# g-benton/Volt

Hardware: AMD Instinct MI355X
Metric: mll_grad_steps_per_s (higher is better)
Workload: dtype f32; 1 GPU; MLL+grad step, N=4096, batch=64 series per GPU, Volatility kernel + EWMA(k=25) mean; series_total=64, parallelism=series-sharded x1, collective=none

## Files before the change

### include/volt_hip_tune.h

```cpp
#ifndef VOLT_HIP_TUNE_H
#define VOLT_HIP_TUNE_H

#include <stddef.h>
#include <stdint.h>

#ifdef __cplusplus
extern "C" {
#endif

int volt_profile_step_f32(const float* K, int64_t ldk, int64_t bsk, const float* resid, const float* sigma2,
                          float* out, float* alpha, void* workspace, int* info, int B, int N, int groups, void* stream,
                          float* ms_sum_host , float* ms_union_host , int* launches_host ,
                          float* per_launch_host );

int volt_tune_update_f32(float* A, const float* Winv, int* info, int B, int Np, int k, int var, int reps, void* stream);
int volt_sched_describe(int B, int n, int has_y, int k, int G, int S, float frac, int* items, int max_items, float* loads);
int volt_tune_diag_f32(float* A, float* Winv, int* info, int B, int Np, int k, long long* stamps, void* stream);

int volt_tune_diag_f64(double* A, double* Winv, int* info, int B, int Np, int k, long long* stamps, void* stream);

int volt_tune_small_stamps(long long* stamps);

int volt_long_describe(int n, int first, int emin, int* items, int max_items, int* nslabs, int* ncnt);

int volt_batch_describe(int B, int n, int has_y, int order, int* items, int max_items);
int volt_tune_batch_stamps(long long* stamps);
int volt_batch64_describe(int B, int n, int has_y, int* items, int max_items);
int volt_tune_batch64_stamps(long long* stamps);
int volt_topology_describe(int* out);

#ifdef __cplusplus
}
#endif
#endif
```

### volt_amd/_lib.py

```python
from __future__ import annotations

import ctypes as C
import os

import torch

from .build import LIB, build_lib, source_hash, sources_present

_lib = None
ABI_VERSION = 5
WANT_GRAD, WS_INITIALISED, REFINE_ALPHA = 1, 2, 4

_i32, _i64, _f32, _f64, _ptr, _sz = C.c_int, C.c_int64, C.c_float, C.c_double, C.c_void_p, C.c_size_t

_SIGS = {
    "volt_abi_version": (C.c_int, []),
    "volt_source_hash": (C.c_char_p, []),
    "volt_padded_n": (C.c_int, [_i32]),
    "volt_cumtrapz_f32": (C.c_int, [_ptr, _i64, _ptr, _i64, _ptr, _i32, _i32, _i32, _ptr]),
    "volt_cumtrapz_f64": (C.c_int, [_ptr, _i64, _ptr, _i64, _ptr, _i32, _i32, _i32, _ptr]),
    "volt_fill_f32": (C.c_int, [_ptr, _ptr, _i32, _i32, _i64, _i64, _ptr]),
    "volt_fill_f64": (C.c_int, [_ptr, _ptr, _i32, _i32, _i64, _i64, _ptr]),
    "volt_ewma_f32": (C.c_int, [_ptr, _i64, _ptr, _i32, _ptr, _i32, _i32, _ptr]),
    "volt_prepare_f32": (C.c_int, [_ptr, _i64, _i64, _ptr, _f32, _ptr, _i32, _i32, _ptr]),
    "volt_potrf_f32": (C.c_int, [_ptr, _ptr, _ptr, _i32, _i32, _ptr]),
    "volt_potrf_workspace_bytes": (C.c_size_t, [_i32, _i32]),
    "volt_potrf_workspace_init_f32": (C.c_int, [_ptr, C.c_size_t, _i32, _i32, _ptr]),
    "volt_potrf_ws_f32": (C.c_int, [_ptr, _ptr, _ptr, _i32, _i32, _ptr, C.c_size_t, _i32, _ptr]),
    "volt_potrf_k_f32": (C.c_int, [_ptr, _i64, _i64, _ptr, C.c_float, _ptr, _ptr, _ptr, _i32, _i32, _ptr, C.c_size_t, _i32, _ptr]),
    "volt_prepare_f64": (C.c_int, [_ptr, _i64, _i64, _ptr, _f64, _ptr, _i32, _i32, _ptr]),
    "volt_potrf_f64": (C.c_int, [_ptr, _ptr, _ptr, _i32, _i32, _ptr]),
    "volt_potrf_workspace_bytes_f64": (C.c_size_t, [_i32, _i32]),
    "volt_potrf_ws_f64": (C.c_int, [_ptr, _ptr, _ptr, _i32, _i32, _ptr, C.c_size_t, _ptr]),
    "volt_potrf_k_f64": (C.c_int, [_ptr, _i64, _i64, _ptr, C.c_double, _ptr, _ptr, _ptr, _i32, _i32, _ptr, C.c_size_t, _ptr]),
    "volt_trsv_lower_f64": (C.c_int, [_ptr, _ptr, _ptr, _ptr, _ptr, _i32, _i32, _ptr]),
    "volt_trsv_lower_t_f64": (C.c_int, [_ptr, _ptr, _ptr, _ptr, _ptr, _i32, _i32, _ptr]),
    "volt_trsv_lower_f32": (C.c_int, [_ptr, _ptr, _ptr, _ptr, _ptr, _i32, _i32, _ptr]),
    "volt_trsv_lower_t_f32": (C.c_int, [_ptr, _ptr, _ptr, _ptr, _ptr, _i32, _i32, _ptr]),
    "volt_trtri_f32": (C.c_int, [_ptr, _ptr, _ptr, _i32, _i32, _ptr]),
    "volt_trtri_f64": (C.c_int, [_ptr, _ptr, _ptr, _i32, _i32, _ptr]),
    "volt_trtri_workspace_bytes_f64": (C.c_size_t, [_i32, _i32]),
    "volt_trtri_ws_f64": (C.c_int, [_ptr, _ptr, _ptr, _i32, _i32, _ptr, C.c_size_t, _ptr]),
    "volt_mll_workspace_bytes_f64": (_sz, [_i32, _i32, _i32]),
    "volt_mll_step_f64": (C.c_int, [_ptr, _i64, _i64, _ptr, _ptr, _f64, _ptr, _ptr, _ptr, _ptr, _i32, _i32, _i32, _ptr]),
    "volt_rollout_scratch_bytes": (_sz, [_i32, _i32, _i32]),
    "volt_rollout_bordered_f32": (C.c_int, [_ptr] * 16 + [_i32] * 6 + [_f32] * 3 + [_ptr]),
    "volt_adam_step_f32": (C.c_int, [_ptr, _i32, C.c_longlong, _ptr, C.c_float, C.c_float, C.c_float, C.c_float, _ptr, _ptr]),
    "volt_mll_workspace_bytes": (_sz, [_i32, _i32, _i32]),
    "volt_mll_workspace_init_f32": (C.c_int, [_ptr, _i32, _i32, _i32, _ptr]),
    "volt_mll_step_f32": (C.c_int, [_ptr, _i64, _i64, _ptr, _ptr, _f32, _ptr, _ptr, _ptr, _ptr, _i32, _i32, _i32, _ptr]),
    "volt_mll_grad_k_f32": (C.c_int, [_ptr, _ptr, _ptr, _ptr, _i32, _i32, _ptr]),
    "volt_rollout_shared_f32": (C.c_int, [_ptr] * 8 + [_i32] * 5 + [_f32, _ptr]),
    "volt_gemm_nt_f32": (C.c_int, [_ptr, _i64, _i64, _i32, _ptr, _i64, _i64, _i32, _ptr, _i64, _i64, _i32, _f32, _f32,
                                   _i32, _i32, _i32, _i32, _ptr]),
    "volt_gpcv_workspace_bytes": (_sz, [_i32, _i32, _i32]),
    "volt_gpcv_step_f32": (C.c_int, [_ptr, _i64, _i64, _f32] + [_ptr] * 6 + [_i32, _f32, _f32, _f32, _f32] + [_ptr] * 7
                           + [_i32, _i32, _i32, _ptr]),
    "volt_gpcv_cv_workspace_bytes": (_sz, [_i32, _i32, _i32, _i32]),
    "volt_gpcv_cv_step_f32": (C.c_int, [_ptr, _i64, _i64, _f32] + [_ptr] * 5 + [_i32, _ptr, _ptr, _i32, _f32, _f32, _f32, _f32]
                              + [_ptr] * 8 + [_i32, _i32, _i32, _ptr]),
    "volt_gpcv_mt_workspace_bytes": (_sz, [_i32, _i32, _i32]),
    "volt_gpcv_mt_step_f32": (C.c_int, [_ptr, _i64, _f32] + [_ptr] * 9 + [_i32, _f32, _f32, _f32, _f32] + [_ptr] * 10
                              + [_i32, _i32, _i32, _ptr]),
    "volt_syev_small_f64": (C.c_int, [_ptr, _i64, _ptr, _ptr, _ptr, _i32, _i32, _ptr]),
    "volt_kron_state_bytes": (_sz, [_i32]),
    "volt_kron_prologue_f32": (C.c_int, [_ptr] * 7 + [_i64] + [_ptr] * 4 + [_i32, _i32, _ptr]),
    "volt_kron_prologue_f64": (C.c_int, [_ptr] * 7 + [_i64] + [_ptr] * 4 + [_i32, _i32, _ptr]),
    "volt_kron_epilogue_f32": (C.c_int, [_ptr] * 11 + [_i32, _i32, _ptr]),
    "volt_kron_epilogue_f64": (C.c_int, [_ptr] * 11 + [_i32, _i32, _ptr]),
}

_TUNE_SIGS = {
    "volt_profile_step_f32": (C.c_int, [_ptr, _i64, _i64, _ptr, _ptr, _ptr, _ptr, _ptr, _ptr, _i32, _i32, _i32, _ptr, _ptr, _ptr,
                                        _ptr, _ptr]),
    "volt_tune_update_f32": (C.c_int, [_ptr, _ptr, _ptr, _i32, _i32, _i32, _i32, _i32, _ptr]),
    "volt_sched_describe": (C.c_int, [_i32, _i32, _i32, _i32, _i32, _i32, C.c_float, _ptr, _i32, _ptr]),
    "volt_tune_diag_f32": (C.c_int, [_ptr, _ptr, _ptr, _i32, _i32, _i32, _ptr, _ptr]),
    "volt_tune_diag_f64": (C.c_int, [_ptr, _ptr, _ptr, _i32, _i32, _i32, _ptr, _ptr]),
    "volt_tune_small_stamps": (C.c_int, [_ptr]),
    "volt_long_describe": (C.c_int, [_i32, _i32, _i32, _ptr, _i32, _ptr, _ptr]),
    "volt_batch_describe": (C.c_int, [_i32, _i32, _i32, _i32, _ptr, _i32]),
    "volt_tune_batch_stamps": (C.c_int, [_ptr]),
    "volt_batch64_describe": (C.c_int, [_i32, _i32, _i32, _ptr, _i32]),
    "volt_tune_batch64_stamps": (C.c_int, [_ptr]),
    "volt_topology_describe": (C.c_int, [_ptr]),
}

EXPORTS = tuple(_SIGS)
TUNE_EXPORTS = tuple(_TUNE_SIGS)


class VoltHipError(RuntimeError):
    pass


class VoltHipWarning(RuntimeWarning):
    """The library recovered from an internal condition (e.g. re-ran a step on the launch-per-column schedule)."""


INFO_INTERNAL_MAX = -(2 ** 31) + 255


def _embedded_hash(path):
    handle = C.CDLL(path)
    fn = handle.volt_source_hash
    fn.restype = C.c_char_p
    return handle, fn().decode()


def lib() -> C.CDLL:
    global _lib
    if _lib is None:
        handle = None
        if os.path.exists(LIB):
            try:
                handle, built = _embedded_hash(LIB)
            except (OSError, AttributeError):
                handle = None
            if handle is not None and sources_present() and built != source_hash():
                import _ctypes
                _ctypes.dlclose(handle._handle)
                handle = None
        if handle is None:
            try:
                build_lib(force=os.path.exists(LIB), verbose=False)
            except Exception as e:
                raise VoltHipError(
                    f"{LIB} is missing or stale and could not be built ({e}): run `python -m volt_amd.build` "
                    "(hipcc, gfx950). volt_amd has no CPU fallback.") from e
            handle, built = _embedded_hash(LIB)
            if built != source_hash():
                raise VoltHipError(f"{LIB} was built from other sources ({built} != {source_hash()}): "
                                   "run `python -m volt_amd.build --force`")
        for name, (res, args) in {**_SIGS, **_TUNE_SIGS}.items():
            fn = getattr(handle, name)
            fn.restype, fn.argtypes = res, args
        if handle.volt_abi_version() != ABI_VERSION:
            raise VoltHipError("libvolt_hip.so ABI version mismatch: rebuild")
        _lib = handle
    return _lib


def check(rc: int, what: str) -> None:
    if rc == 0:
        return
    if rc < 0:
        raise VoltHipError(f"{what}: invalid argument #{-rc}")
    raise VoltHipError(f"{what}: HIP error {rc}")


def stream_ptr() -> int:
    return torch.cuda.current_stream().cuda_stream
```

### volt_amd/csrc/batch_step.hip

```cpp
#include "common.h"
#include "tiles.h"
#include "host.h"
#include "batch_sched.h"
#include "../../include/volt_hip.h"
#include "../../include/volt_hip_tune.h"
#include <algorithm>
#include <array>
#include <map>
#include <mutex>
#include <string.h>
#include <vector>

namespace volt {

__global__ void batch_begin_kernel(float* __restrict__ Winv, int nflags, int* __restrict__ info, int ninfo,
                                   int* __restrict__ prog, int nprog) {
    const int i = blockIdx.x * blockDim.x + threadIdx.x;
    if (i < nflags) reinterpret_cast<int*>(Winv)[(int64_t)i * TS * TS] = 0;
    if (i < ninfo) info[i] = 0;
    for (int c = i; c < nprog; c += gridDim.x * blockDim.x) prog[c] = 0;
}

constexpr int AUX_WT = AUX_SC1;

__device__ __forceinline__ void diag0_image(const KSource& src, int b, float* smem) {
    const float add = (src.sigma2 ? src.sigma2[b] : 0.f) + src.jitter;
    const float* Kb = src.K + (int64_t)b * src.bsk;
    const int N = src.N;
#pragma unroll 1
    for (int e0 = threadIdx.x; e0 < TS * TS; e0 += 16 * NT) {
        float v[16];
#pragma unroll
        for (int u = 0; u < 16; ++u) {
            const int e = e0 + u * NT, r = e >> 7, c = e & 127;
            v[u] = Kb[(int64_t)(r < N ? r : N - 1) * src.ldk + (c < N ? c : N - 1)];
        }
#pragma unroll
        for (int u = 0; u < 16; ++u) {
            const int e = e0 + u * NT, r = e >> 7, c = e & 127;
            float x = (r < N && c < N) ? v[u] : 0.f;
            if (r == c) x = (r < N) ? x + add : 1.f;
            smem[r * DT + c] = (c <= r) ? x : 0.f;
        }
    }
}

__device__ __forceinline__ void alpha_item(const float* __restrict__ Y, const TriReduce& red, float* __restrict__ z,
                                           float* __restrict__ apart, int Np, int b, int c, int chunk) {
    const int n = Np / TS, lane = threadIdx.x & 63, wave = threadIdx.x >> 6, l31 = lane & 31, h = lane >> 5;
    f32x4 zc = {0.f, 0.f, 0.f, 0.f};
    {
        const float* zp = red.zpart + (int64_t)b * n * Np + c * TS + 4 * l31;
        int jb = 0;
        for (; jb + 8 <= c + 1; jb += 8) {
            f32x4 v[8];
#pragma unroll
            for (int u = 0; u < 8; ++u) v[u] = *reinterpret_cast<const f32x4*>(zp + (int64_t)(jb + u) * Np);
#pragma unroll
            for (int u = 0; u < 8; ++u)
#pragma unroll
                for (int e = 0; e < 4; ++e) zc[e] += v[u][e];
        }
        for (; jb <= c; ++jb) {
            const f32x4 v = *reinterpret_cast<const f32x4*>(zp + (int64_t)jb * Np);
#pragma unroll
            for (int e = 0; e < 4; ++e) zc[e] += v[e];
        }
    }
    if (chunk == 0 && wave == 0 && h == 0) *reinterpret_cast<f32x4*>(z + (int64_t)b * Np + c * TS + 4 * l31) = zc;
    const float* Yc = Y + (int64_t)b * Np * Np + c * TS + 4 * l31 + (int64_t)h * Np;
    float* dst = apart + ((int64_t)b * n + c) * Np;
    const int r0 = chunk * BATCH_ALPHA_ROWS;
    const int r1 = (r0 + BATCH_ALPHA_ROWS < (c + 1) * TS) ? r0 + BATCH_ALPHA_ROWS : (c + 1) * TS;
    for (int r = r0 + 32 * wave; r < r1; r += 128) {
        f32x4 y[16];
#pragma unroll
        for (int u = 0; u < 16; ++u) y[u] = *reinterpret_cast<const f32x4*>(Yc + (int64_t)(r + 2 * u) * Np);
#pragma unroll
        for (int u = 0; u < 16; ++u) {
            float lo, hi;
            rowpair_dot(y[u], zc, lo, hi);
            if (lane == 0) {
                dst[r + 2 * u] = lo;
                dst[r + 2 * u + 1] = hi;
            }
        }
    }
}

static long long* g_batch_stamps = nullptr;

struct BatchArgs {
    float* A; float* Winv; float* Y; int* info;
    int Np, B;
    KSource src;
    TriReduce red;
    const int4* tab;
    int* prog;
    int pstride;
    float* zvec; float* apart;
    long long* stamps;
};

static __shared__ __attribute__((aligned(16))) float g_smem[2 * STAGE_FLOATS];
static __shared__ float g_srv[TS];
static __shared__ int g_piece;
static __shared__ int g_ahead[2];
static __shared__ int4 g_desc;

template <bool FROMK, bool LOCAL>
__device__ __forceinline__ void batch_piece(const BatchArgs a, const int w, const bool ahead, const int par, BatchPull& pull,
                                            int* qw, int per_queue) {
    float* const smem = g_smem;
    float* const srv = g_srv;
    float* const A = a.A; float* const Winv = a.Winv; float* const Y = a.Y; int* const info = a.info;
    const int Np = a.Np;
    const KSource& src = a.src;
    const TriReduce& red = a.red;
    long long* const stamps = a.stamps;
    const int n = Np / TS;
    int4 d = ahead ? g_desc : a.tab[BATCH_HDR + w];
    d.x = __builtin_amdgcn_readfirstlane(d.x);
    d.y = __builtin_amdgcn_readfirstlane(d.y);
    d.z = __builtin_amdgcn_readfirstlane(d.z);
    if (stamps && threadIdx.x == 0) stamps[(int64_t)w * 8 + 5] = __builtin_amdgcn_s_memrealtime();
    const int kind = d.x & 7, b = d.x >> 3;
    int* rowp = a.prog + (int64_t)b * a.pstride;
    int* tcol = rowp + n;
    int* la = tcol + n;
    int* info_b = info + b;
    const bool usek = FROMK && src.K != nullptr;

    if (kind == BK_DIAG) {
        const int k = d.y;
        __builtin_amdgcn_s_setprio(3);
        if (k == 0) {
            if (usek) {
                diag0_image(src, b, smem);
                diag_body<false, false, LOCAL>(A, Winv, info, Np, 0, b, smem, nullptr, true);
            } else {
                diag_body<false, false, LOCAL>(A, Winv, info, Np, 0, b, smem, nullptr, false);
            }
            return;
        }
        batch_wait<LOCAL>(rowp + k, k, k >= 2 ? la + k : nullptr, 1, info_b);
        if (stamps && threadIdx.x == 0) stamps[(int64_t)w * 8 + 3] = __builtin_amdgcn_s_memrealtime();
        if (k >= 2) update_body<FROMK>(A, Np, k, k, k - 1, k, false, b, src, smem, true);
        else update_body<FROMK>(A, Np, 1, 1, 0, 1, true, b, src, smem, true);
        if (stamps && threadIdx.x == 0) stamps[(int64_t)w * 8 + 4] = __builtin_amdgcn_s_memrealtime();
        diag_body<false, false, LOCAL>(A, Winv, info, Np, k, b, smem, nullptr, true);
        return;
    }
    if (kind == BK_LOOKAHEAD) {
        const int k = d.y;
        Chase ch;
        ch.p0 = ch.p1 = rowp + k + 1;
        bool ok = true;
        update_body<FROMK, 0, true, LOCAL>(A, Np, k + 1, k + 1, 0, k, true, b, src, smem, false, &ch, &ok);
        if (!ok && (threadIdx.x & 63) == 0) report_timeout(info_b);
        publish_release<LOCAL>(la + k + 1, 1);
        return;
    }
    if (kind == BK_TRTRI_DIAG) {
        const int i = d.y;
        batch_wait<LOCAL>(reinterpret_cast<const int*>(Winv + ((int64_t)b * n + i) * TS * TS), 1, nullptr, 0, info_b);
        trtri_diag_body(Winv, Y, Np, i, b, red, smem);
        publish_release<LOCAL>(tcol + i, 1);
        return;
    }
    if (kind == BK_ALPHA) {
        const int c = d.y;
        if (threadIdx.x < 64) {
            bool ok = true;
            for (int j = 0; j <= c; ++j) ok = wait_word<AtLeast>(tcol + j, c - j + 1) && ok;
            if (!ok && threadIdx.x == 0) report_timeout(info_b);
            acquire_unless_local<LOCAL>();
        }
        __syncthreads();
        alpha_item(Y, red, a.zvec, a.apart, Np, b, c, d.z);
        return;
    }
    TriJob jb;
    int* word;
    int val;
    if (kind == BK_PANEL) {
        const int i = d.y, k = d.z;
        jb = panel_job<FROMK>(A, Winv, Np, i, k, b, src);
        jb.t.ch.p0 = rowp + k;
        jb.t.ch.p1 = rowp + i;
        word = rowp + i;
        val = k + 1;
    } else {
        const int i = d.y, j = d.z;
        jb = trtri_job(A, Winv, Y, Np, i, j, b);
        if (red.rpad && threadIdx.x < TS) srv[threadIdx.x] = red.rpad[(int64_t)b * Np + j * TS + threadIdx.x];
        jb.t.flag = reinterpret_cast<const int*>(jb.t.W);
        jb.t.ch.p0 = rowp + i;
        jb.t.ch.base0 = j;
        jb.t.ch.p1 = tcol + j;
        word = tcol + j;
        val = i - j + 1;
    }
    f32x16 T[4], O[4];
    ChasePre pre = {0, 0};
    if (jb.t.n1 > 0) pre = chase_issue(jb.t.ch);
    job_t0(jb, T);
    if (stamps && threadIdx.x == 0) stamps[(int64_t)w * 8 + 3] = __builtin_amdgcn_s_memrealtime();
    const bool ok = tri_tile_run<true, LOCAL>(jb.t, T, O, smem, &pre);
#ifndef VOLT_NO_EPILOGUE_PRIO
    __builtin_amdgcn_s_setprio(3);
#endif
    if (stamps && threadIdx.x == 0) stamps[(int64_t)w * 8 + 4] = __builtin_amdgcn_s_memrealtime();
    if (!ok && (threadIdx.x & 63) == 0) report_timeout(info_b);
    int t_next = -1;
    if (threadIdx.x == 0 && pull.q >= 0) t_next = __hip_atomic_fetch_add(qw + 32 * pull.q, 1, __ATOMIC_RELAXED, __HIP_MEMORY_SCOPE_AGENT);
    if (jb.i >= 0 && red.rpad) trtri_reduce<!LOCAL>(O, Np, jb.i, jb.j, jb.b, red, smem + TS * WLD, srv);
    if (stamps && threadIdx.x == 0) stamps[(int64_t)w * 8 + 6] = __builtin_amdgcn_s_memrealtime();
    tri_store_lds<LOCAL ? 0 : AUX_WT>(O, jb.out, Np, smem);
    if (stamps && threadIdx.x == 0) stamps[(int64_t)w * 8 + 7] = __builtin_amdgcn_s_memrealtime();
    int4 d_next = {0, 0, 0, 0};
    int w_next = -1;
    if (threadIdx.x == 0 && pull.q >= 0) {
        if (t_next < per_queue) {
            w_next = LOCAL ? 8 * t_next + pull.q : t_next;
            d_next = a.tab[BATCH_HDR + w_next];
        } else {
            pull.q = -1;
        }
    }
    publish_wt<LOCAL>(word, val);
    if (threadIdx.x == 0 && w_next >= 0) {
        g_ahead[par ^ 1] = 1;
        g_piece = w_next;
        g_desc = d_next;
    }
}

template <bool FROMK, bool LOCAL>
__global__ __launch_bounds__(256, 2) void batch_step_kernel(BatchArgs a, int check, int npieces, int xskew, int xdrop) {
    {
        const int4 h0 = a.tab[0];
        if (h0.x != BATCH_MAGIC || h0.y != a.B || h0.z != a.Np / TS || h0.w != check) {
            if (blockIdx.x == 0)
                for (int b = threadIdx.x; b < a.B; b += NT) a.info[b] = INFO_BAD_WORKSPACE;
            return;
        }
    }
    int* const qw = a.prog + (int64_t)a.B * a.pstride;
    const int hw = hw_xcc_id();
    if (LOCAL && ((xdrop >> hw) & 1)) return;
    const int xcc = (hw + xskew) & 7;
    const int per_queue = LOCAL ? npieces / 8 : npieces;
    BatchPull pull;
    int w, ahead = 0, par = -1;
    if (xdrop & 0x40000000) {
        w = xskew | (int)0x80000000;
        goto piece;
    }
pull_next:
    __syncthreads();
    if (threadIdx.x == 0 && !(par >= 0 && g_ahead[par])) g_piece = batch_next_piece<LOCAL>(pull, qw, xcc, per_queue);
    __syncthreads();
    w = g_piece;
    ahead = par >= 0 ? g_ahead[par] : 0;
    par = par < 0 ? 0 : par;
    if (threadIdx.x == 0) g_ahead[par ^ 1] = 0;
piece:
    w = __builtin_amdgcn_readfirstlane(w);
    if (w < 0) return;
    __builtin_amdgcn_s_setprio(0);
    if (a.stamps && threadIdx.x == 0) {
        a.stamps[(int64_t)w * 8] = __builtin_amdgcn_s_memrealtime();
        a.stamps[(int64_t)w * 8 + 2] = ((long long)hw << 32) | (unsigned)__builtin_amdgcn_s_getreg((16 - 1) << 11 | 0 << 6 | 4);
    }
    par = __builtin_amdgcn_readfirstlane(par < 0 ? 0 : par);
    batch_piece<FROMK, LOCAL>(a, w, __builtin_amdgcn_readfirstlane(ahead) != 0, par, pull, qw, per_queue);
    par ^= 1;
    if (a.stamps && threadIdx.x == 0) a.stamps[(int64_t)w * 8 + 1] = __builtin_amdgcn_s_memrealtime();
    goto pull_next;
}

}

using namespace volt;

bool volt_internal_batch_applies(int B, int n, int has_y) {
    const Tunables& tn = tunables();
    if (tn.batch <= 0 || B < 1 || n < 2 || B > 65535) return false;
    if (tn.batch >= 2) return true;
    if (has_y) {
        if (n >= 20) return B >= 2;
        if (n >= 16) return B >= 4;
        if (n >= 10) return B >= 6;
        if (n >= 8) return B >= 20;
        return false;
    }
    if (n >= 28) return B >= 2;
    if (n >= 20) return B >= 3;
    if (n >= 10) return B >= 8;
    if (n >= 8) return B >= 24;
    return false;
}

bool volt_internal_batch_first() { return tunables().batch >= 3; }

static int batch_lad(int B) {
    int lad = tunables().batch_lad;
    while (lad > 0 && 2 * lad * B > 128) --lad;
    return lad;
}

static size_t batch_table_bytes(int B, int n, bool has_y) {
    return al256((size_t)(BATCH_HDR + batch_count(B, n, has_y)) * sizeof(BatchItem));
}
static size_t batch_prog_bytes(int B, int n) {
    return al256(((size_t)B * batch_pstride(n) + BATCH_QWORDS) * sizeof(int));
}

size_t volt_internal_batch_bytes(int B, int n, int has_y) {
    if (!volt_internal_batch_applies(B, n, has_y)) return 0;
    return batch_table_bytes(B, n, has_y != 0) + batch_prog_bytes(B, n);
}

static int batch_order_for(int B, int n) {
    const int forced = tunables().batch_order;
    if (forced >= 0) return forced;
    return (B >= 48 && n >= 28 && (B & 7) == 0) ? 54 : 0;
}

static int batch_check_word(int B, int n, bool has_y) {
    const uint32_t w = (uint32_t)BATCH_MAGIC ^ ((uint32_t)B * 0x01000193u) ^ ((uint32_t)n << 20) ^ (has_y ? 0x40000000u : 0u) ^
                       ((uint32_t)batch_order_for(B, n) * 2654435761u) ^ ((uint32_t)batch_lad(B) << 16);
    return (int)w;
}

struct BatchTable {
    int4* items = nullptr;
    size_t bytes = 0;
};
static const BatchTable* get_batch_table(int B, int n, bool has_y) {
    static std::mutex mu;
    static std::map<std::array<int, 4>, BatchTable*> cache;
    const int order = batch_order_for(B, n);
    const std::array<int, 4> key{B, n, has_y ? 1 : 0, order * 16 + batch_lad(B)};
    std::lock_guard<std::mutex> lock(mu);
    auto it = cache.find(key);
    if (it != cache.end()) return it->second;
    std::vector<BatchItem> items;
    batch_build(B, n, has_y, order, items, batch_lad(B));
    BatchTable* bt = new BatchTable;
    static_assert(sizeof(BatchItem) == sizeof(int4), "items are read as int4");
    bt->bytes = (BATCH_HDR + items.size()) * sizeof(BatchItem);
    if ((int64_t)items.size() != batch_count(B, n, has_y) ||
        hipHostMalloc((void**)&bt->items, bt->bytes, hipHostMallocDefault) != hipSuccess) {
        (void)hipGetLastError();
        delete bt;
        bt = nullptr;
    } else {
        memset(bt->items, 0, BATCH_HDR * sizeof(BatchItem));
        bt->items[0] = int4{BATCH_MAGIC, B, n, batch_check_word(B, n, has_y)};
        for (BatchItem& it : items) it.pad = batch_check_word(B, n, has_y);
        memcpy(bt->items + BATCH_HDR, items.data(), items.size() * sizeof(BatchItem));
    }
    cache[key] = bt;
    return bt;
}

int volt_internal_batch_install(Region state, int B, int n, int has_y, void* stream) {
    if (!state.p || state.bytes < volt_internal_batch_bytes(B, n, has_y) || !volt_internal_batch_applies(B, n, has_y)) return 0;
    const BatchTable* bt = get_batch_table(B, n, has_y != 0);
    if (!bt) return (int)hipErrorOutOfMemory;
    hipError_t e = hipMemcpyAsync(state.p, bt->items, bt->bytes, hipMemcpyHostToDevice, (hipStream_t)stream);
    return e != hipSuccess ? (int)e : 0;
}

int volt_internal_batch_step(const StepMats& m, const KSource& src, const TriReduce& red_in, const StepTail& t, Region state,
                             hipEvent_t e0, hipEvent_t e1) {
    const int B = m.B, Np = volt_padded_n(m.N), n = Np / TS;
    const bool has_y = m.Y != nullptr;
    if (!state.p || !volt_internal_batch_applies(B, n, has_y) || state.bytes < volt_internal_batch_bytes(B, n, has_y)) return 0;
    if (has_y && (!t.z || !t.apart)) return 0;
    hipStream_t s = m.stream;
    const int4* tab = reinterpret_cast<const int4*>(state.p);
    int* prog = reinterpret_cast<int*>(reinterpret_cast<char*>(state.p) + batch_table_bytes(B, n, has_y));
    const int pstride = batch_pstride(n), nprog = B * pstride + BATCH_QWORDS, nflags = B * n;
    hipLaunchKernelGGL(batch_begin_kernel, dim3(begin_grid(std::max(nflags, B), nprog)), dim3(256), 0, s, m.Winv, nflags, m.info, B, prog, nprog);
    const int check = batch_check_word(B, n, has_y);
    const bool local = batch_local_handoffs(B);
    const TriReduce red{has_y ? red_in.rpad : nullptr, red_in.zpart, red_in.frob, m.N};
    const int64_t npieces = batch_count(B, n, has_y);
    const int spread = tunables().batch_spread + (n < 32 ? 9 * (32 - n) * tunables().cus / 256 : 0);
    const unsigned pad = (int64_t)B * (n + 1) <= spread ? 16 * 1024 : 0;
    const int64_t slots = (int64_t)tunables().cus * (pad ? 1 : 2) * std::max(1, tunables().batch_pullers);
    const unsigned grid = (unsigned)std::min<int64_t>(npieces, tunables().batch_pullers > 0 ? slots : npieces);
    const BatchArgs args{m.A, m.Winv, m.Y, m.info, Np, B, src, red, tab, prog, pstride, t.z, t.apart, g_batch_stamps};
    const int xskew = tunables().batch_xskew, xdrop = tunables().batch_xdrop;
    if (e0 && hipEventRecord(e0, s) != hipSuccess) return (int)hipGetLastError();
#define VOLT_BATCH_LAUNCH(FK, LC) \
    hipLaunchKernelGGL((batch_step_kernel<FK, LC>), dim3(grid), dim3(256), pad, s, args, check, (int)npieces, xskew, xdrop)
    if (src.K && local) VOLT_BATCH_LAUNCH(true, true);
    else if (src.K) VOLT_BATCH_LAUNCH(true, false);
    else if (local) VOLT_BATCH_LAUNCH(false, true);
    else VOLT_BATCH_LAUNCH(false, false);
#undef VOLT_BATCH_LAUNCH
    if (e1 && hipEventRecord(e1, s) != hipSuccess) return (int)hipGetLastError();
    hipError_t e = hipGetLastError();
    return e != hipSuccess ? (int)e : 1;
}

extern "C" {

int volt_topology_describe(int* out) {
    if (!out) return -1;
    const Tunables& tn = tunables();
    out[0] = tn.cus;
    out[1] = tn.xccs;
    out[2] = tn.sched_g;
    out[3] = tn.plain_spread;
    out[4] = tn.split_spread;
    out[5] = tn.group_gate;
    out[6] = (tn.small_nmax > 0 ? 1 : 0) | (tn.long_on ? 2 : 0) | (tn.batch > 0 ? 4 : 0);
    return 0;
}

int volt_tune_batch_stamps(long long* stamps) {
    g_batch_stamps = stamps;
    return 0;
}

int volt_batch_describe(int B, int n, int has_y, int order, int* items, int max_items) {
    if (order == -1) order = 1000 + batch_order_for(B, n);
    if (B < 1 || n < 1 || order < 0 || (order > 15 && order < 1000) || order > 1255) return -1;
    std::vector<BatchItem> it;
    if (order >= 1000) batch_build(B, n, has_y != 0, order - 1000, it, 0);
    else batch_build(B, n, has_y != 0, order & 1, it, order >> 1);
    if ((int64_t)it.size() != batch_count(B, n, has_y != 0)) return -1;
    if (items) {
        if ((int)it.size() > max_items) return -2;
        memcpy(items, it.data(), it.size() * sizeof(BatchItem));
    }
    return (int)it.size();
}

}
```

### volt_amd/csrc/chol.hip

```cpp
#include "common.h"
#include "tiles.h"
#include "host.h"
#include "sched.h"
#include "long_sched.h"
#include "../../include/volt_hip.h"
#include "../../include/volt_hip_tune.h"
#include <algorithm>
#include <array>
#include <map>
#include <mutex>
#include <stdlib.h>
#include <string.h>
#include <utility>
#include <vector>

namespace volt {

__global__ __launch_bounds__(256) void prepare_kernel(const float* __restrict__ K, int64_t ldk, int64_t bsk,
                                                      const float* __restrict__ sigma2, float jitter,
                                                      float* __restrict__ A, int N, int Np, int col0_only) {
    int t = blockIdx.x;
    int ti, tj;
    if (col0_only) {
        ti = t;
        tj = 0;
    } else {
        ti = (int)((sqrtf(8.f * (float)t + 1.f) - 1.f) * 0.5f);
        while ((ti + 1) * (ti + 2) / 2 <= t) ++ti;
        while (ti * (ti + 1) / 2 > t) --ti;
        tj = t - ti * (ti + 1) / 2;
    }
    const int b = blockIdx.y;
    const float add = (sigma2 ? sigma2[b] : 0.f) + jitter;
    const float* Kb = K + (int64_t)b * bsk;
    float* Ab = A + (int64_t)b * Np * Np;
    const int cq = (threadIdx.x & 31) * 4;
    const int r0 = threadIdx.x >> 5;
    const bool vec_ok = ((ldk & 3) == 0) && ((bsk & 3) == 0) && (((uintptr_t)K & 15) == 0);
#pragma unroll 4
    for (int rr = r0; rr < TS; rr += 8) {
        const int i = ti * TS + rr;
        const int j = tj * TS + cq;
        f32x4 v;
        if (i < N && j + 3 < N && vec_ok) {
            v = *reinterpret_cast<const f32x4*>(Kb + (int64_t)i * ldk + j);
        } else {
#pragma unroll
            for (int c = 0; c < 4; ++c) v[c] = (i < N && j + c < N) ? Kb[(int64_t)i * ldk + j + c] : 0.f;
        }
#pragma unroll
        for (int c = 0; c < 4; ++c)
            if (i == j + c) v[c] = (i < N) ? v[c] + add : 1.f;
        *reinterpret_cast<f32x4*>(Ab + (int64_t)i * Np + j) = v;
    }
}

template <bool FROMK>
__global__ __launch_bounds__(256, 2) void factor_step_kernel(float* __restrict__ A, float* __restrict__ Winv,
                                                            float* __restrict__ Y, int* __restrict__ info, int Np,
                                                            int k_upd, int i_tri, int B, KSource src, TriReduce red) {
    __shared__ __attribute__((aligned(16))) float smem[2 * STAGE_FLOATS];
    static_assert(DIAG_LDS_FLOATS <= 2 * STAGE_FLOATS, "diag block must fit the staging area");
    static_assert(TS * WLD + TS <= 2 * STAGE_FLOATS, "W image + reduction scratch must fit");
    const int n = Np / TS;
    int w = blockIdx.x;
    TriJob jb;
    bool have = false;
    if (k_upd >= 0) {
        const int k = k_upd;
        if (w < B) {
            if (k >= 2) update_body<FROMK>(A, Np, k, k, k - 1, k, false, w, src, smem, true);
            else if (k == 1) update_body<FROMK>(A, Np, 1, 1, 0, 1, true, w, src, smem, true);
            diag_body(A, Winv, info, Np, k, w, smem, nullptr, k > 0);
            return;
        }
        w -= B;
        const int npre = (k >= 1 && k + 1 < n) ? B : 0;
        if (w < npre) {
            update_body<FROMK>(A, Np, k + 1, k + 1, 0, k, true, w, src, smem);
            return;
        }
        w -= npre;
        const int npan = (n - k - 1) * B;
        if (w < npan) {
            int t, b;
            decode_tile_batch(w, n - k - 1, B, t, b);
            jb = panel_job<FROMK>(A, Winv, Np, k + 1 + t, k, b, src);
            have = true;
        }
        w -= npan;
    }
    if (!have) {
        int j, b;
        decode_tile_batch(w, i_tri + 1, B, j, b);
        if (j == i_tri) {
            trtri_diag_body(Winv, Y, Np, i_tri, b, red, smem);
            return;
        }
        jb = trtri_job(A, Winv, Y, Np, i_tri, j, b);
    }
    f32x16 T[4], O[4];
    if (jb.c0 && jb.row_ok && jb.vec_ok) {
#pragma unroll
        for (int tm = 0; tm < 4; ++tm)
#pragma unroll
            for (int g = 0; g < 4; ++g) {
                const f32x4 v = *reinterpret_cast<const f32x4*>(jb.c0 + 32 * tm + 8 * g);
#pragma unroll
                for (int e = 0; e < 4; ++e) T[tm][4 * g + e] = -v[e];
            }
    } else if (jb.c0 && jb.row_ok) {
#pragma unroll
        for (int tm = 0; tm < 4; ++tm)
#pragma unroll
            for (int q = 0; q < 16; ++q) T[tm][q] = -jb.c0[32 * tm + 8 * (q >> 2) + (q & 3)];
    } else {
        zero_acc(T);
    }
    const bool ok = tri_tile_run(jb.t, T, O, smem);
    if (threadIdx.x == 0 && !ok) report_timeout(info + jb.b);
    tri_store(O, jb.out, Np);
    if (jb.i >= 0 && red.rpad) trtri_reduce(O, Np, jb.i, jb.j, jb.b, red, smem);
}

constexpr int VOLT_SPLITK_SLABS = 64;
struct SplitK {
    float* slab;
    int* count;
    int S;
    int L;
    int cap;
    int4* tab = nullptr;
    size_t tab_bytes = 0;
};

__device__ __forceinline__ void slab_sum(f32x16 (&acc)[4], const float* __restrict__ slabs, int nsl) {
    zero_acc(acc);
    for (int sidx = 0; sidx < nsl; ++sidx) {
        const f32x4* in = reinterpret_cast<const f32x4*>(slabs + (int64_t)sidx * TS * TS);
#pragma unroll
        for (int t4 = 0; t4 < 4; ++t4)
#pragma unroll
            for (int g = 0; g < 4; ++g) {
                const f32x4 v = in[(t4 * 4 + g) * NT + threadIdx.x];
#pragma unroll
                for (int e = 0; e < 4; ++e) acc[t4][4 * g + e] += v[e];
            }
    }
}
__device__ __forceinline__ bool splitk_arrive(int* counter, int nsl) {
    __shared__ int s_last;
    asm volatile("s_waitcnt vmcnt(0)" ::: "memory");
    __syncthreads();
    if (threadIdx.x == 0) {
        const int old = __hip_atomic_fetch_add(counter, 1, __ATOMIC_RELAXED, __HIP_MEMORY_SCOPE_AGENT);
        s_last = (old == nsl - 1);
        if (s_last) __builtin_amdgcn_fence(__ATOMIC_ACQUIRE, "agent");
    }
    __syncthreads();
    return s_last != 0;
}

template <bool FROMK>
__device__ __forceinline__ void lookahead_slice(float* __restrict__ A, int Np, int k, int b, int sl, int nsl, int b0, int b1,
                                                const KSource& src, float* __restrict__ slabs, int* __restrict__ counter,
                                                float* smem) {
    float* Ab = A + (int64_t)b * Np * Np;
    const int lane = threadIdx.x & 63, wave = threadIdx.x >> 6, wr = wave >> 1, wc = wave & 1;
    f32x16 acc[4];
    zero_acc(acc);
    gemm_nt_128<0>(Ab + (int64_t)(k + 1) * TS * Np + (int64_t)b0 * TS, Np, Ab + (int64_t)(k + 1) * TS * Np + (int64_t)b0 * TS, Np,
                   (b1 - b0) * (TS / BK), acc, smem);
    if (nsl > 1) {
        slab_dump(acc, slabs + (int64_t)sl * TS * TS);
        if (!splitk_arrive(counter, nsl)) return;
        slab_sum(acc, slabs, nsl);
    }
    const bool usek = FROMK && src.K != nullptr;
    const float add = usek ? ((src.sigma2 ? src.sigma2[b] : 0.f) + src.jitter) : 0.f;
    const float* Kb = usek ? src.K + (int64_t)b * src.bsk : nullptr;
    float* C = Ab + (int64_t)(k + 1) * TS * Np + (int64_t)(k + 1) * TS;
#pragma unroll
    for (int tm = 0; tm < 2; ++tm)
#pragma unroll
        for (int tn = 0; tn < 2; ++tn)
#pragma unroll
            for (int q = 0; q < 16; ++q) {
                const int r = wr * 64 + tm * 32 + accrow(q, lane);
                const int c = wc * 64 + tn * 32 + (lane & 31);
                C[(int64_t)r * Np + c] = input_elem(src, Kb, add, Ab, Np, usek, (k + 1) * TS + r, (k + 1) * TS + c)
                                         - acc[tm * 2 + tn][q];
            }
}

template <bool FUSE>
__device__ __forceinline__ void tri_slice(TriJob& jb, int sl, int nsl, int b0, int b1, float* __restrict__ slabs,
                                          int* __restrict__ counter, int* __restrict__ info, const TriReduce& red, int Np,
                                          float* smem) {
    f32x16 T[4], O[4];
    if (sl == 0 && jb.c0 && jb.row_ok && jb.vec_ok) {
#pragma unroll
        for (int tm = 0; tm < 4; ++tm)
#pragma unroll
            for (int g = 0; g < 4; ++g) {
                const f32x4 v = *reinterpret_cast<const f32x4*>(jb.c0 + 32 * tm + 8 * g);
#pragma unroll
                for (int e = 0; e < 4; ++e) T[tm][4 * g + e] = -v[e];
            }
    } else if (sl == 0 && jb.c0 && jb.row_ok) {
#pragma unroll
        for (int tm = 0; tm < 4; ++tm)
#pragma unroll
            for (int q = 0; q < 16; ++q) T[tm][q] = -jb.c0[32 * tm + 8 * (q >> 2) + (q & 3)];
    } else {
        zero_acc(T);
    }
    if (!FUSE || nsl > 1) {
        gemm_nt_128<1>(jb.t.X + (int64_t)b0 * TS, jb.t.ldx, jb.t.Z + (int64_t)b0 * TS, jb.t.ldz, (b1 - b0) * (TS / BK), T, smem);
        if (nsl > 1) {
            slab_dump(T, slabs + (int64_t)sl * TS * TS);
            if (!splitk_arrive(counter, nsl)) return;
            slab_sum(T, slabs, nsl);
        }
        jb.t.n1 = 0;
    }
    const bool ok = tri_tile_run(jb.t, T, O, smem);
    if (threadIdx.x == 0 && !ok) report_timeout(info + jb.b);
    tri_store(O, jb.out, Np);
    if (jb.i >= 0 && red.rpad) trtri_reduce(O, Np, jb.i, jb.j, jb.b, red, smem);
}

template <bool FROMK>
__global__ __launch_bounds__(256, 2) void factor_step_split_kernel(float* __restrict__ A, float* __restrict__ Winv,
                                                                  float* __restrict__ Y, int* __restrict__ info, int Np,
                                                                  int k_upd, int i_tri, int B, KSource src, TriReduce red,
                                                                  SplitK sk) {
    __shared__ __attribute__((aligned(16))) float smem[2 * STAGE_FLOATS];
    const int n = Np / TS, S = sk.S;
    int w = blockIdx.x;
    const int k = k_upd;
    if (k < n && w < B) {
        if (k >= 2) update_body<FROMK>(A, Np, k, k, k - 1, k, false, w, src, smem, true);
        else if (k == 1) update_body<FROMK>(A, Np, 1, 1, 0, 1, true, w, src, smem, true);
        diag_body(A, Winv, info, Np, k, w, smem, nullptr, k > 0);
        return;
    }
    if (k < n) w -= B;
    int* count = sk.count + (int64_t)k * B * (n + 1);
    const int npre = (k >= 1 && k + 1 < n) ? B : 0;
    if (w < npre * S) {
        const int b = w / S, sl = w % S;
        const int kb = k;
        int nsl = (kb + sk.L - 1) / sk.L;
        nsl = nsl < 1 ? 1 : (nsl > S ? S : nsl);
        if (sl >= nsl) return;
        lookahead_slice<FROMK>(A, Np, k, b, sl, nsl, sl * kb / nsl, (sl + 1) * kb / nsl, src,
                               sk.slab + (int64_t)b * S * TS * TS, count + b, smem);
        return;
    }
    w -= npre * S;
    TriJob jb;
    int tile, kb;
    const int npan = (k < n) ? (n - k - 1) * B : 0;
    const int sl = w % S;
    int wt = w / S;
    if (wt < npan) {
        int t, b;
        decode_tile_batch(wt, n - k - 1, B, t, b);
        jb = panel_job<FROMK>(A, Winv, Np, k + 1 + t, k, b, src);
        tile = B + wt;
        kb = k;
    } else {
        wt -= npan;
        int j, b;
        decode_tile_batch(wt, i_tri + 1, B, j, b);
        if (j == i_tri) {
            if (sl == 0) trtri_diag_body(Winv, Y, Np, i_tri, b, red, smem);
            return;
        }
        jb = trtri_job(A, Winv, Y, Np, i_tri, j, b);
        tile = B + npan + wt;
        kb = i_tri - j;
    }
    int nsl = (kb + sk.L - 1) / sk.L;
    nsl = nsl < 1 ? 1 : (nsl > S ? S : nsl);
    if (sl >= nsl) return;
    tri_slice<false>(jb, sl, nsl, sl * kb / nsl, (sl + 1) * kb / nsl, sk.slab + (int64_t)tile * S * TS * TS, count + tile,
                     info, red, Np, smem);
}

template <bool FROMK>
__global__ __launch_bounds__(256, 1) void factor_step_sched_kernel(float* __restrict__ A, float* __restrict__ Winv,
                                                                  float* __restrict__ Y, int* __restrict__ info, int Np,
                                                                  int k, int i_tri, int B, KSource src, TriReduce red,
                                                                  SplitK sk, const int4* __restrict__ items, int4 key0,
                                                                  int4 key1) {
    __shared__ __attribute__((aligned(16))) float smem[2 * STAGE_FLOATS];
    const int n = Np / TS, S = sk.S;
    {
        const int4 h0 = sk.tab[0], h1 = sk.tab[1];
        if (h0.x != key0.x || h0.y != key0.y || h0.z != key0.z || h0.w != key0.w || h1.x != key1.x || h1.y != key1.y ||
            h1.z != key1.z || h1.w != key1.w) {
            if (blockIdx.x == 0)
                for (int b = threadIdx.x; b < B; b += NT) info[b] = INFO_BAD_WORKSPACE;
            return;
        }
    }
    int* count = sk.count + (int64_t)k * B * (n + 1);
    const int4 d = items[blockIdx.x];
    const int kind = d.x & 7, b = d.x >> 3;
    const int sl = d.z & 255, nsl = (d.z >> 8) & 255, tile = d.z >> 16;
    const int b0 = d.w & 0xffff, b1 = d.w >> 16;
    float* slabs = sk.slab + (int64_t)tile * S * TS * TS;
    if (kind == 0) {
        if (k >= 2) update_body<FROMK>(A, Np, k, k, k - 1, k, false, b, src, smem, true);
        else if (k == 1) update_body<FROMK>(A, Np, 1, 1, 0, 1, true, b, src, smem, true);
        diag_body(A, Winv, info, Np, k, b, smem, nullptr, k > 0);
    } else if (kind == 4) {
        trtri_diag_body(Winv, Y, Np, i_tri, b, red, smem);
    } else if (kind == 1) {
        lookahead_slice<FROMK>(A, Np, k, b, sl, nsl, b0, b1, src, slabs, count + tile, smem);
    } else {
        TriJob jb = kind == 2 ? panel_job<FROMK>(A, Winv, Np, d.y, k, b, src) : trtri_job(A, Winv, Y, Np, i_tri, d.y, b);
        tri_slice<true>(jb, sl, nsl, b0, b1, slabs, count + tile, info, red, Np, smem);
    }
}

__global__ __launch_bounds__(256, 2) void tune_diag_kernel(float* __restrict__ A, float* __restrict__ Winv,
                                                          int* __restrict__ info, int Np, int k, long long* stamps) {
    __shared__ __attribute__((aligned(16))) float smem[2 * STAGE_FLOATS];
    diag_body<true>(A, Winv, info, Np, k, blockIdx.x, smem, stamps + 32 * blockIdx.x);
}

__global__ void begin_factor_kernel(float* __restrict__ Winv, int nflags, int* __restrict__ info, int ninfo,
                                    int* __restrict__ count, int ncount) {
    const int i = blockIdx.x * blockDim.x + threadIdx.x;
    if (i < nflags) reinterpret_cast<int*>(Winv)[(int64_t)i * TS * TS] = 0;
    if (i < ninfo) info[i] = 0;
    for (int c = i; c < ncount; c += gridDim.x * blockDim.x) count[c] = 0;
}

__global__ __launch_bounds__(256, 2) void tune_update_kernel(float* __restrict__ A, const float* __restrict__ Winv,
                                                            int* __restrict__ info, int Np, int k, int B, KSource src) {
    __shared__ __attribute__((aligned(16))) float smem[2 * STAGE_FLOATS];
    int t, b;
    decode_tile_batch(Np / TS - k - 1, B, t, b);
    const TriJob jb = panel_job<false>(A, Winv, Np, k + 1 + t, k, b, src);
    f32x16 T[4], O[4];
#pragma unroll
    for (int tm = 0; tm < 4; ++tm)
#pragma unroll
        for (int g = 0; g < 4; ++g) {
            const f32x4 v = *reinterpret_cast<const f32x4*>(jb.c0 + 32 * tm + 8 * g);
#pragma unroll
            for (int e = 0; e < 4; ++e) T[tm][4 * g + e] = -v[e];
        }
    const bool ok = tri_tile_run(jb.t, T, O, smem);
    if (threadIdx.x == 0 && !ok) report_timeout(info + jb.b);
    tri_store(O, jb.out, Np);
}
template <int ABL>
__global__ __launch_bounds__(256, 2) void tune_update_sq_kernel(float* __restrict__ A, int Np, int k, int B, KSource src) {
    __shared__ __attribute__((aligned(16))) float smem[2 * STAGE_FLOATS];
    int t, b;
    decode_tile_batch(Np / TS - k - 1, B, t, b);
    update_body<false, ABL>(A, Np, k + 1 + t, k, 0, k, true, b, src, smem);
}
__global__ void tune_empty_kernel(float* A) { if (A == nullptr) A[0] = 0.f; }

}

using namespace volt;

static Tunables read_env(Tunables t) {
    auto geti = [](const char* name, int& v) { if (const char* e = getenv(name)) v = atoi(e); };
        geti("VOLT_GROUPS", t.groups);
        geti("VOLT_SPLITK_TARGET", t.splitk_target);
        geti("VOLT_SPLITK_MINL", t.splitk_minl);
        geti("VOLT_SPLITK_MAXS", t.splitk_maxs);
        geti("VOLT_SPLITK_GROUPS", t.splitk_groups);
        geti("VOLT_SPLITK_MAXB", t.splitk_maxb);
        geti("VOLT_SCHED", t.sched);
        geti("VOLT_SCHED_MINB", t.sched_minb);
        geti("VOLT_SCHED_MAXB", t.sched_maxb);
        geti("VOLT_SCHED_MAXB_POTRF", t.sched_maxb_potrf);
        geti("VOLT_SCHED_G", t.sched_g);
        geti("VOLT_SCHED_S", t.sched_s);
        geti("VOLT_SCHED_GROUPS", t.sched_groups);
        geti("VOLT_SCHED_KMIN", t.sched_kmin);
        geti("VOLT_SMALL_NMAX", t.small_nmax);
        geti("VOLT_SMALL_MAXWG", t.small_maxwg);
        geti("VOLT_SMALL_PAD_MAXB", t.small_pad_maxb);
        geti("VOLT_SMALL_MAXB", t.small_maxb);
        geti("VOLT_SMALL_MAXB2", t.small_maxb2);
        geti("VOLT_LONG", t.long_on);
        geti("VOLT_LONG_FIRST", t.long_first);
        geti("VOLT_LONG_EMIN", t.long_emin);
        geti("VOLT_LONG_PAD", t.long_pad);
        geti("VOLT_LONG_NMIN", t.long_nmin);
        geti("VOLT_LONG_XCD", t.long_xcd);
        geti("VOLT_LONG_SPLIT", t.long_split);
        geti("VOLT_PLAIN_SPREAD", t.plain_spread);
        geti("VOLT_SPLIT_SPREAD", t.split_spread);
        geti("VOLT_BATCH", t.batch);
        geti("VOLT_BATCH_ORDER", t.batch_order);
        geti("VOLT_BATCH_LOCAL", t.batch_local);
        geti("VOLT_BATCH_SPREAD", t.batch_spread);
        geti("VOLT_BATCH_LAD", t.batch_lad);
        geti("VOLT_BATCH_PULLERS", t.batch_pullers);
        geti("VOLT_ROLLOUT_LANE", t.rollout_lane);
        geti("VOLT_LONG_PULLERS", t.long_pullers);
        geti("VOLT_BATCH_XSKEW", t.batch_xskew);
        geti("VOLT_BATCH_XDROP", t.batch_xdrop);
        geti("VOLT_BATCH64", t.batch64);
        geti("VOLT_BATCH64_MAX", t.batch64_max);
        geti("VOLT_BATCH64_MAX_STEP", t.batch64_max_step);
        geti("VOLT_F64_LOOKAHEAD", t.f64_lookahead);
        geti("VOLT_F64_TRTRI_LOOKAHEAD", t.f64_trtri_lookahead);
        geti("VOLT_F64_SPREAD", t.f64_spread);
        geti("VOLT_F64_SPLIT_TARGET", t.f64_split_target);
        if (const char* e = getenv("VOLT_SCHED_FRAC")) t.sched_frac = (float)atof(e);
        geti("VOLT_FAKE_CUS", t.cus);
        geti("VOLT_FAKE_XCCS", t.xccs);
    return t;
}

static void apply_topology(Tunables& t, bool faked) {
    if (!faked) {
        int dev = 0, cus = 0, xccs = 0;
        if (hipGetDevice(&dev) == hipSuccess &&
            hipDeviceGetAttribute(&cus, hipDeviceAttributeMultiprocessorCount, dev) == hipSuccess && cus > 0) {
            t.cus = cus;
            if (hipDeviceGetAttribute(&xccs, hipDeviceAttributeNumberOfXccs, dev) == hipSuccess && xccs > 0) t.xccs = xccs;
        } else {
            (void)hipGetLastError();
        }
    }
    if (t.cus == 256 && t.xccs == 8) return;
    const double f = t.cus / 256.0;
    auto scale = [f](int v, int lo) { const int r = (int)(v * f + 0.5); return r < lo ? lo : r; };
    t.sched_g = scale(t.sched_g, 8);
    t.plain_spread = scale(t.plain_spread, 8);
    t.split_spread = scale(t.split_spread, 16);
    t.splitk_target = scale(t.splitk_target, 16);
    t.group_gate = scale(t.group_gate, 16);
    t.batch_spread = scale(t.batch_spread, 8);
    t.small_nmax = 0;
    t.long_on = 0;
    t.batch = 0;
    t.batch64 = 0;
}

const Tunables& tunables() {
    static const Tunables tn = [] {
        const char* tune0 = getenv("VOLT_TUNE");
        const bool tuning = tune0 && atoi(tune0) != 0;
        const bool faked = tuning && (getenv("VOLT_FAKE_CUS") || getenv("VOLT_FAKE_XCCS"));
        Tunables t = [&] {
            Tunables t;
            if (!tuning) return t;
            return read_env(t);
        }();
        apply_topology(t, faked);
        return t;
    }();
    return tn;
}
struct LaunchTimer {
    hipEvent_t base = nullptr;
    std::vector<hipEvent_t> ev;
    std::vector<int> cls;
    hipError_t err = hipSuccess;
    void note(hipError_t e) { if (err == hipSuccess && e != hipSuccess) err = e; }
    void start(hipStream_t s) {
        note(hipEventCreate(&base));
        note(hipEventRecord(base, s));
    }
    void begin(int c, hipStream_t s) {
        hipEvent_t e = nullptr;
        note(hipEventCreate(&e));
        note(hipEventRecord(e, s));
        ev.push_back(e);
        cls.push_back(c);
    }
    void end(hipStream_t s) {
        hipEvent_t e = nullptr;
        note(hipEventCreate(&e));
        note(hipEventRecord(e, s));
        ev.push_back(e);
    }
    void collect(float* ms_sum, float* ms_union, int* n_by_class, int nclass, float* per_launch = nullptr) {
        std::vector<std::vector<std::pair<float, float>>> iv(nclass);
        for (int c = 0; c < nclass; ++c) { ms_sum[c] = ms_union[c] = 0.f; n_by_class[c] = 0; }
        for (size_t i = 0; i < cls.size(); ++i) {
            float t0 = 0.f, t1 = 0.f;
            note(hipEventElapsedTime(&t0, base, ev[2 * i]));
            note(hipEventElapsedTime(&t1, base, ev[2 * i + 1]));
            ms_sum[cls[i]] += t1 - t0;
            n_by_class[cls[i]] += 1;
            if (per_launch) per_launch[i] = t1 - t0;
            iv[cls[i]].push_back({t0, t1});
        }
        for (int c = 0; c < nclass; ++c) {
            std::sort(iv[c].begin(), iv[c].end());
            float lo = 0.f, hi = -1.f;
            for (auto& x : iv[c]) {
                if (hi < lo || x.first > hi) {
                    if (hi >= lo) ms_union[c] += hi - lo;
                    lo = x.first;
                    hi = x.second;
                } else if (x.second > hi) {
                    hi = x.second;
                }
            }
            if (hi >= lo) ms_union[c] += hi - lo;
        }
        for (auto e : ev) (void)hipEventDestroy(e);
        if (base) (void)hipEventDestroy(base);
        ev.clear();
        cls.clear();
    }
};

struct FactorOpts {
    KSource src;
    float* Y;
    TriReduce red;
    SplitK sk;
    const struct SchedDev* sched = nullptr;
};

constexpr int SCHED_HDR = 16;
struct SchedDev {
    int4* items = nullptr;
    size_t bytes = 0;
    int4 key[2];
    std::vector<int> item_off;
    int S = 0;
    int pad_lds = 0;
    int kmin = 0;
};

static const SchedDev* get_sched(int B, int n, bool has_y, const SchedParams& p, hipStream_t s) {
    static std::mutex mu;
    static std::map<std::array<int, 8>, SchedDev*> cache;
    int dev = 0;
    if (hipGetDevice(&dev) != hipSuccess) return nullptr;
    const std::array<int, 8> key{dev, B, n, has_y ? 1 : 0, p.G, p.S, (int)(p.frac * 1000.f), p.min_len};
    std::lock_guard<std::mutex> lock(mu);
    auto it = cache.find(key);
    if (it != cache.end()) return it->second;
    hipStreamCaptureStatus cap = hipStreamCaptureStatusNone;
    if (hipStreamIsCapturing(s, &cap) != hipSuccess || cap != hipStreamCaptureStatusNone) return nullptr;
    std::vector<SchedItem> items;
    SchedDev* sd = new SchedDev;
    sd->S = p.S;
    sd->pad_lds = 16 * 1024;
    const int kmin_env = tunables().sched_kmin;
    sd->kmin = kmin_env >= 0 ? kmin_env : !has_y ? (B * (256 / p.G) >= 48 ? 20 : 12) : (p.G < 256 ? 16 : B <= 4 ? 12 : B <= 7 ? 16 : 20);
    const int launches = has_y ? n + 1 : n;
    for (int k = 0; k < launches; ++k) {
        sd->item_off.push_back((int)items.size());
        sched_build_launch(B, n, has_y, k, p, items);
    }
    sd->item_off.push_back((int)items.size());
    static_assert(sizeof(SchedItem) == sizeof(int4), "items are read as int4");
    sd->bytes = (SCHED_HDR + items.size()) * sizeof(SchedItem);
    sd->key[0] = int4{0x564f4c54, B, n, has_y ? 1 : 0};
    sd->key[1] = int4{p.G, p.S, (int)(p.frac * 1000.f), p.min_len};
    if (hipHostMalloc((void**)&sd->items, sd->bytes, hipHostMallocDefault) != hipSuccess) {
        (void)hipGetLastError();
        delete sd;
        sd = nullptr;
    } else {
        memset(sd->items, 0, SCHED_HDR * sizeof(SchedItem));
        sd->items[0] = sd->key[0];
        sd->items[1] = sd->key[1];
        memcpy(sd->items + SCHED_HDR, items.data(), items.size() * sizeof(SchedItem));
    }
    cache[key] = sd;
    return sd;
}

static bool sched_choice(int B, int n, bool has_y, int cap, int& Gs, SchedParams& sp) {
    const Tunables& tn = tunables();
    if (!tn.sched || cap < 1 || B < tn.sched_minb || B > (has_y ? tn.sched_maxb : tn.sched_maxb_potrf)) return false;
    Gs = (tn.sched_groups > 1 && B >= 10 && B % tn.sched_groups == 0) ? tn.sched_groups : 1;
    sp = SchedParams();
    sp.G = tn.sched_g / Gs;
    sp.S = std::max(1, std::min(tn.sched_s, cap / B));
    sp.frac = tn.sched_frac;
    (void)n;
    return true;
}

static int sched_install(void* tab, size_t tab_bytes, int B, int n, bool has_y, int cap, hipStream_t s) {
    int Gs = 1;
    SchedParams sp;
    if (!tab || !sched_choice(B, n, has_y, cap, Gs, sp)) return 0;
    const SchedDev* sd = get_sched(B / Gs, n, has_y, sp, s);
    if (!sd || sd->bytes > tab_bytes) return 0;
    hipError_t e = hipMemcpyAsync(tab, sd->items, sd->bytes, hipMemcpyHostToDevice, s);
    return e != hipSuccess ? (int)e : 0;
}

struct Group {
    float* A;
    float* Winv;
    int* info;
    FactorOpts o;
    int B;
    hipStream_t s;
};

static void enqueue_step(const Group& g, int Np, int k, LaunchTimer* tm) {
    const int n = Np / TS, B = g.B;
    const TriReduce nored{nullptr, nullptr, nullptr, 0};
    const int itri = (g.o.Y && k > 0) ? k - 1 : -1;
    const int npre = (k >= 1 && k + 1 < n) ? B : 0;
    const int grid = B + npre + (n - k - 1) * B + (itri >= 0 ? (itri + 1) * B : 0);
    if (g.o.sched && k >= g.o.sched->kmin) {
        const SchedDev& sd = *g.o.sched;
        SplitK sk = g.o.sk;
        sk.S = sd.S;
        sk.L = 1;
        for (int kk = k; kk <= (k + 1 == n && g.o.Y ? n : k); ++kk) {
            const int it = kk < n ? itri : n - 1;
            if (tm) tm->begin(kk < n ? 0 : 1, g.s);
            const int cnt = sd.item_off[kk + 1] - sd.item_off[kk];
            if (g.o.src.K && kk < n)
                hipLaunchKernelGGL(factor_step_sched_kernel<true>, dim3(cnt), dim3(256), sd.pad_lds, g.s, g.A, g.Winv, g.o.Y,
                                   g.info, Np, kk, it, B, g.o.src, g.o.Y ? g.o.red : nored, sk, g.o.sk.tab + SCHED_HDR + sd.item_off[kk], sd.key[0],
                                   sd.key[1]);
            else
                hipLaunchKernelGGL(factor_step_sched_kernel<false>, dim3(cnt), dim3(256), sd.pad_lds, g.s, g.A, g.Winv, g.o.Y,
                                   g.info, Np, kk, it, B, g.o.src, g.o.Y ? g.o.red : nored, sk, g.o.sk.tab + SCHED_HDR + sd.item_off[kk], sd.key[0],
                                   sd.key[1]);
            if (tm) tm->end(g.s);
        }
        return;
    }
    if (!g.o.sched && g.o.sk.slab && g.o.sk.S > 1) {
        const int kk = k < n ? k : n - 1;
        const double blocks = (double)B * ((double)(n - kk - 1) * kk + 0.5 * kk * (kk - 1) + kk);
        int L = (int)(blocks / (double)g.o.sk.S + 0.999);
        const int minl = tunables().splitk_minl;
        if (L < minl) L = minl;
        int S = (kk + L - 1) / L;
        if (S < 1) S = 1;
        const int maxs = tunables().splitk_maxs;
        if (S > maxs) S = maxs;
        if (S * B > g.o.sk.cap) S = g.o.sk.cap / B;
        if (S < 1) S = 1;
        SplitK sk = g.o.sk;
        sk.S = S;
        sk.L = L;
        const int gs = B + S * (npre + (n - k - 1) * B + (itri >= 0 ? (itri + 1) * B : 0));
        if (tm) tm->begin(0, g.s);
        const int split_spread = tunables().split_spread;
        const unsigned spad = gs <= split_spread ? 16 * 1024 : 0;
        if (g.o.src.K)
            hipLaunchKernelGGL(factor_step_split_kernel<true>, dim3(gs), dim3(256), spad, g.s, g.A, g.Winv, g.o.Y, g.info, Np,
                               k, itri, B, g.o.src, g.o.Y ? g.o.red : nored, sk);
        else
            hipLaunchKernelGGL(factor_step_split_kernel<false>, dim3(gs), dim3(256), spad, g.s, g.A, g.Winv, g.o.Y, g.info, Np,
                               k, itri, B, g.o.src, g.o.Y ? g.o.red : nored, sk);
        if (tm) tm->end(g.s);
        if (k + 1 == n && g.o.Y) {
            if (tm) tm->begin(1, g.s);
            hipLaunchKernelGGL(factor_step_split_kernel<false>, dim3(S * n * B), dim3(256), S * n * B <= split_spread ? 16 * 1024 : 0, g.s, g.A, g.Winv, g.o.Y,
                               g.info, Np, n, n - 1, B, g.o.src, g.o.red, sk);
            if (tm) tm->end(g.s);
        }
        return;
    }
    if (tm) tm->begin(0, g.s);
    const unsigned pad = grid <= tunables().plain_spread ? 16 * 1024 : 0;
    if (g.o.src.K)
        hipLaunchKernelGGL(factor_step_kernel<true>, dim3(grid), dim3(256), pad, g.s, g.A, g.Winv, g.o.Y, g.info, Np, k,
                           itri, B, g.o.src, g.o.Y ? g.o.red : nored);
    else
        hipLaunchKernelGGL(factor_step_kernel<false>, dim3(grid), dim3(256), pad, g.s, g.A, g.Winv, g.o.Y, g.info, Np, k,
                           itri, B, g.o.src, g.o.Y ? g.o.red : nored);
    if (tm) tm->end(g.s);
    if (k + 1 == n && g.o.Y) {
        if (tm) tm->begin(1, g.s);
        hipLaunchKernelGGL(factor_step_kernel<false>, dim3(n * B), dim3(256), 0, g.s, g.A, g.Winv, g.o.Y, g.info, Np,
                           -1, n - 1, B, g.o.src, g.o.red);
        if (tm) tm->end(g.s);
    }
}

static int begin_factor(float* Winv, int* info, int B, int n, hipStream_t s, int* sk_count = nullptr) {
    const int nflags = B * n, ncount = sk_count ? (n + 1) * (n + 1) * B : 0;
    hipLaunchKernelGGL(begin_factor_kernel, dim3(begin_grid(std::max(nflags, B), ncount)), dim3(256), 0, s, Winv, nflags, info, B, sk_count, ncount);
    return 0;
}

constexpr int MAX_GROUPS = 8;
struct StreamPool {
    hipStream_t aux[MAX_GROUPS - 1];
    hipEvent_t fork, join[MAX_GROUPS - 1], extra[5];
    std::mutex mu;
    int want_groups = 2;
    bool ok = false;
};
static StreamPool* stream_pool() {
    static StreamPool pools[16];
    static std::once_flag once[16];
    int dev = 0;
    if (hipGetDevice(&dev) != hipSuccess || dev < 0 || dev >= 16) return nullptr;
    std::call_once(once[dev], [dev]() {
        StreamPool& p = pools[dev];
        bool ok = hipEventCreateWithFlags(&p.fork, hipEventDisableTiming) == hipSuccess;
        for (int i = 0; i < MAX_GROUPS - 1; ++i) {
            ok = ok && hipStreamCreateWithFlags(&p.aux[i], hipStreamNonBlocking) == hipSuccess;
            ok = ok && hipEventCreateWithFlags(&p.join[i], hipEventDisableTiming) == hipSuccess;
        }
        for (int i = 0; i < 5; ++i) ok = ok && hipEventCreateWithFlags(&p.extra[i], hipEventDisableTiming) == hipSuccess;
        p.want_groups = tunables().groups;
        if (p.want_groups < 1) p.want_groups = 1;
        if (p.want_groups > MAX_GROUPS) p.want_groups = MAX_GROUPS;
        p.ok = ok;
    });
    return pools[dev].ok ? &pools[dev] : nullptr;
}

bool volt_internal_aux(VoltAux* out) {
    StreamPool* p = stream_pool();
    if (!p) return false;
    *out = VoltAux{p->aux[0], p->aux[1], p->aux[2], p->aux[3], p->fork,
                   {p->join[0], p->join[1], p->join[2], p->join[3], p->join[4], p->join[5], p->join[6], p->extra[0],
                    p->extra[1], p->extra[2], p->extra[3], p->extra[4]}, &p->mu};
    return true;
}

static int pick_groups(const StreamPool* pool, int B, int force) {
    int want = force > 0 ? force : (pool ? pool->want_groups : 1);
    if (want > MAX_GROUPS) want = MAX_GROUPS;
    while (want > 1 && (B % want != 0 || B / want < 8)) want >>= 1;
    return want;
}

#define VOLT_TRY(call)                              \
    do {                                            \
        hipError_t e__ = (call);                    \
        if (e__ != hipSuccess) return (int)e__;     \
    } while (0)

static int run_factor_groups(float* A, float* Winv, int* info, int B, int Np, hipStream_t s, const FactorOpts& o,
                             volt_group_post_fn post = nullptr, void* post_ctx = nullptr, LaunchTimer* tm = nullptr,
                             int force_groups = 0) {
    const int n = Np / TS;
    StreamPool* pool = stream_pool();
    int G = pool ? pick_groups(pool, B, force_groups) : 1;
    if (force_groups == 0 && (int64_t)B * (n + 1) < tunables().group_gate) G = 1;
    hipStreamCaptureStatus cap_status = hipStreamCaptureStatusNone;
    const bool capturing = hipStreamIsCapturing(s, &cap_status) == hipSuccess && cap_status != hipStreamCaptureStatusNone;
    if (capturing && force_groups == 0) G = 1;
    const Tunables& tn = tunables();
    const int target = tn.splitk_target, split_groups = tn.splitk_groups, split_maxb = tn.splitk_maxb;
    const bool can_split = o.sk.slab && o.sk.count && force_groups == 0 && target > 1;
    FactorOpts o1 = o;
    o1.sk.S = 1;
    if (can_split && B < 8) {
        G = 1;
        o1.sk.S = target;
    }
    if (can_split && !capturing && B >= 10 && B < split_maxb && pool && split_groups > 1 && B % split_groups == 0) {
        G = split_groups;
        o1.sk.S = target / G;
    }
    if (can_split) {
        int Gs = 1;
        SchedParams sp;
        const SchedDev* sd = nullptr;
        if (o.sk.tab && sched_choice(B, n, o.Y != nullptr, o.sk.cap, Gs, sp) && (Gs == 1 || (pool && !capturing)))
            sd = get_sched(B / Gs, n, o.Y != nullptr, sp, s);
        if (sd && sd->bytes <= o.sk.tab_bytes && n > sd->kmin + (B < 8 ? 7 : 1)) {
            G = Gs;
            o1.sk.S = 2;
            o1.sched = sd;
        }
    }
    int rc = begin_factor(Winv, info, B, n, s, o1.sk.S > 1 ? o1.sk.count : nullptr);
    if (rc) return rc;
    std::unique_lock<std::mutex> lock;
    if (pool && G > 1) lock = std::unique_lock<std::mutex>(pool->mu);
    if (pool && G > 1) VOLT_TRY(hipEventRecord(pool->fork, s));
    if (tm) tm->start(s);
    if (G == 1) {
        const Group g{A, Winv, info, o1, B, s};
        for (int k = 0; k < n; ++k) enqueue_step(g, Np, k, tm);
        if (post) post(post_ctx, 0, B, s);
        VOLT_LAUNCH_CHECK();
        return tm && tm->err != hipSuccess ? (int)tm->err : 0;
    }
    const int Bg = B / G;
    const int64_t mat = (int64_t)Np * Np;
    Group grp[MAX_GROUPS];
    for (int g = 0; g < G; ++g) {
        FactorOpts og = o1;
        const int b0 = g * Bg;
        if (og.sk.S > 1) {
            og.sk.slab += (int64_t)g * (o.sk.cap / G) * (n + 1) * TS * TS;
            og.sk.count += (int64_t)g * (n + 1) * (n + 1) * Bg;
            og.sk.cap = o.sk.cap / G;
        }
        if (og.src.K) {
            og.src.K += (int64_t)b0 * og.src.bsk;
            if (og.src.sigma2) og.src.sigma2 += b0;
        }
        if (og.Y) og.Y += b0 * mat;
        if (og.red.rpad) {
            og.red.rpad += (int64_t)b0 * Np;
            og.red.zpart += (int64_t)b0 * n * Np;
            og.red.frob += (int64_t)b0 * (n * (n + 1) / 2);
        }
        grp[g] = Group{A + b0 * mat, Winv + (int64_t)b0 * n * TS * TS, info + b0, og, Bg, g == 0 ? s : pool->aux[g - 1]};
        if (g > 0) VOLT_TRY(hipStreamWaitEvent(grp[g].s, pool->fork, 0));
    }
    for (int k = 0; k < n; ++k)
        for (int g = 0; g < G; ++g) enqueue_step(grp[g], Np, k, tm);
    if (post)
        for (int g = 0; g < G; ++g) post(post_ctx, g * Bg, Bg, grp[g].s);
    int first_err = 0;
    for (int g = 1; g < G; ++g) {
        hipError_t e = hipEventRecord(pool->join[g - 1], grp[g].s);
        if (e == hipSuccess) e = hipStreamWaitEvent(s, pool->join[g - 1], 0);
        if (e != hipSuccess) {
            (void)hipStreamSynchronize(grp[g].s);
            if (!first_err) first_err = (int)e;
        }
    }
    if (first_err) return first_err;
    VOLT_LAUNCH_CHECK();
    return tm && tm->err != hipSuccess ? (int)tm->err : 0;
}

static int run_trtri(const float* A, const float* Winv, float* Y, int B, int Np, hipStream_t s, LaunchTimer* tm) {
    const int n = Np / TS;
    const TriReduce nored{nullptr, nullptr, nullptr, 0};
    for (int i = 0; i < n; ++i) {
        if (tm) tm->begin(1, s);
        hipLaunchKernelGGL(factor_step_kernel<false>, dim3((i + 1) * B), dim3(256), 0, s, const_cast<float*>(A),
                           const_cast<float*>(Winv), Y, nullptr, Np, -1, i, B, KSource{nullptr, 0, 0, nullptr, 0.f, 0},
                           nored);
        if (tm) tm->end(s);
    }
    VOLT_LAUNCH_CHECK();
    return 0;
}

size_t volt_internal_sched_bytes(int B, int n) {
    if (B < 3 || B > 64 || n < 8) return 0;
    return al256(((size_t)(n + 1) * B * (1 + 4 * (size_t)(n + 1)) + SCHED_HDR) * sizeof(SchedItem));
}

int volt_internal_sched_install(Region tab, int B, int n, int has_y, int cap, void* stream) {
    return sched_install(tab.p, tab.bytes, B, n, has_y != 0, cap, (hipStream_t)stream);
}

static FactorOpts factor_from_k(const StepMats& m, const KSource& src, const TriReduce& red, const SplitScratch& sk) {
    const int Np = volt_padded_n(m.N);
    hipLaunchKernelGGL(prepare_kernel, dim3(Np / TS, m.B), dim3(256), 0, m.stream, src.K, src.ldk, src.bsk, src.sigma2, src.jitter,
                       m.A, m.N, Np, 1);
    return FactorOpts{src, m.Y, red, SplitK{sk.slab, sk.count, 1, 1, sk.rows, (int4*)sk.tab.p, sk.tab.bytes}};
}

int volt_internal_factor(const StepMats& m, const KSource& src, const TriReduce& red, const SplitScratch& sk,
                         volt_group_post_fn post, void* post_ctx) {
    const FactorOpts o = factor_from_k(m, src, red, sk);
    return run_factor_groups(m.A, m.Winv, m.info, m.B, volt_padded_n(m.N), m.stream, o, post, post_ctx);
}

int volt_internal_profile(const StepMats& m, const KSource& src, const TriReduce& red, const SplitScratch& sk, int groups,
                          volt_group_post_fn post, void* post_ctx, const ProfileOut& out) {
    if (groups < 0 || groups > MAX_GROUPS) return -11;
    const FactorOpts o = factor_from_k(m, src, red, sk);
    LaunchTimer tm;
    const int rc = run_factor_groups(m.A, m.Winv, m.info, m.B, volt_padded_n(m.N), m.stream, o, post, post_ctx, &tm, groups);
    hipError_t e = hipStreamSynchronize(m.stream);
    tm.collect(out.ms_sum, out.ms_union, out.launches, 2, out.per_launch);
    if (rc) return rc;
    if (e != hipSuccess) return (int)e;
    return tm.err != hipSuccess ? (int)tm.err : 0;
}

extern "C" {

int volt_prepare_f32(const float* K, int64_t ldk, int64_t bsk, const float* sigma2, float jitter, float* A, int B,
                     int N, void* stream) {
    if (!K) return -1;
    if (ldk < N) return -2;
    if (!A) return -6;
    if (B < 0 || B > 65535) return -7;
    if (N < 1) return -8;
    if (B == 0) return 0;
    const int Np = volt_padded_n(N), n = Np / TS;
    hipLaunchKernelGGL(prepare_kernel, dim3(n * (n + 1) / 2, B), dim3(256), 0, (hipStream_t)stream, K, ldk, bsk,
                       sigma2, jitter, A, N, Np, 0);
    VOLT_LAUNCH_CHECK();
    return 0;
}

int volt_tune_update_f32(float* A, const float* Winv, int* info, int B, int Np, int k, int var, int reps, void* stream) {
    if (!A) return -1;
    if (!Winv) return -2;
    if (!info) return -3;
    if (B < 1) return -4;
    if (Np < TS || Np % TS) return -5;
    const int n = Np / TS;
    if (k < 1 || k + 1 >= n) return -6;
    if (var < 0 || var > 5) return -7;
    hipStream_t s = (hipStream_t)stream;
    const KSource none{nullptr, 0, 0, nullptr, 0.f, 0};
    for (int r = 0; r < reps; ++r) {
        if (var == 0) hipLaunchKernelGGL(tune_update_kernel, dim3((n - k - 1) * B), dim3(256), 0, s, A, Winv, info, Np, k, B, none);
        else if (var == 1) hipLaunchKernelGGL(tune_update_sq_kernel<0>, dim3((n - k - 1) * B), dim3(256), 0, s, A, Np, k, B, none);
        else if (var == 2) hipLaunchKernelGGL(tune_update_sq_kernel<1>, dim3((n - k - 1) * B), dim3(256), 0, s, A, Np, k, B, none);
        else if (var == 3) hipLaunchKernelGGL(tune_update_sq_kernel<2>, dim3((n - k - 1) * B), dim3(256), 0, s, A, Np, k, B, none);
        else if (var == 4) hipLaunchKernelGGL(tune_update_sq_kernel<3>, dim3((n - k - 1) * B), dim3(256), 0, s, A, Np, k, B, none);
        else hipLaunchKernelGGL(tune_empty_kernel, dim3((n - k - 1) * B), dim3(256), 0, s, A);
    }
    VOLT_LAUNCH_CHECK();
    return 0;
}

int volt_sched_describe(int B, int n, int has_y, int k, int G, int S, float frac, int* items, int max_items, float* loads) {
    if (B < 1 || n < 1 || k < 0 || k > n || (k == n && !has_y) || G < 1 || S < 1) return -1;
    SchedParams p;
    p.G = G;
    p.S = S;
    if (frac > 0.f) p.frac = frac;
    std::vector<SchedItem> it;
    std::vector<float> ld;
    sched_build_launch(B, n, has_y != 0, k, p, it, &ld);
    if ((int)it.size() > max_items) return -2;
    if (items) memcpy(items, it.data(), it.size() * sizeof(SchedItem));
    if (loads) memcpy(loads, ld.data(), ld.size() * sizeof(float));
    return (int)it.size();
}



int volt_tune_diag_f32(float* A, float* Winv, int* info, int B, int Np, int k, long long* stamps, void* stream) {
    if (!A) return -1;
    if (!Winv) return -2;
    if (!info) return -3;
    if (B < 1) return -4;
    if (Np < TS || Np % TS) return -5;
    if (k < 0 || k >= Np / TS) return -6;
    if (!stamps) return -7;
    hipLaunchKernelGGL(tune_diag_kernel, dim3(B), dim3(256), 0, (hipStream_t)stream, A, Winv, info, Np, k, stamps);
    VOLT_LAUNCH_CHECK();
    return 0;
}

static int potrf_ws_rows(int B) { return B < 32 ? VOLT_SPLITK_SLABS : (B <= 64 ? 2 * VOLT_SPLITK_SLABS : 0); }

struct PotrfWs {
    SplitScratch sk;
    Region batch;
    size_t bytes;
};
static PotrfWs carve_potrf(void* ws, int B, int Np) {
    const size_t n = (size_t)Np / TS;
    size_t off = 0;
    auto take = [&](size_t bytes) {
        void* p = ws && bytes ? reinterpret_cast<char*>(ws) + off : nullptr;
        off += bytes;
        return Region{p, bytes};
    };
    PotrfWs w;
    w.sk.rows = n < 3 ? 0 : potrf_ws_rows(B);
    w.sk.slab = reinterpret_cast<float*>(take(w.sk.rows ? al256((size_t)w.sk.rows * (n + 1) * TS * TS * sizeof(float)) : 0).p);
    w.sk.count = reinterpret_cast<int*>(take(w.sk.rows ? al256((n + 1) * (n + 1) * B * sizeof(int)) : 0).p);
    w.sk.tab = take(w.sk.rows ? volt_internal_sched_bytes(B, (int)n) : 0);
    w.batch = take(volt_internal_batch_bytes(B, (int)n, 0));
    w.bytes = off;
    return w;
}

size_t volt_potrf_workspace_bytes(int B, int Np) {
    if (B < 1 || Np < TS || Np % TS) return 0;
    return carve_potrf(nullptr, B, Np).bytes;
}

int volt_potrf_workspace_init_f32(void* ws, size_t ws_bytes, int B, int Np, void* stream) {
    if (B < 1) return -3;
    if (Np < TS || Np % TS) return -4;
    if (!volt_potrf_workspace_bytes(B, Np)) return 0;
    if (!ws || ((uintptr_t)ws & 255)) return -1;
    const PotrfWs w = carve_potrf(ws, B, Np);
    if (ws_bytes < w.bytes) return -2;
    if (w.batch.p) {
        const int rc = volt_internal_batch_install(w.batch, B, Np / TS, 0, stream);
        if (rc) return rc;
    }
    if (!w.sk.tab.p) return 0;
    return sched_install(w.sk.tab.p, w.sk.tab.bytes, B, Np / TS, false, w.sk.rows, (hipStream_t)stream);
}

static int potrf_with_scratch(const KSource& src, const StepMats& m, void* ws, size_t ws_bytes, int ws_flags, int err) {
    const int Np = volt_padded_n(m.N);
    const bool ready = (ws_flags & VOLT_WS_INITIALISED) != 0;
    SplitScratch sk{nullptr, nullptr, 0, {}};
    if (ws) {
        if (((uintptr_t)ws & 255) != 0) return err;
        const PotrfWs w = carve_potrf(ws, m.B, Np);
        if (ws_bytes < w.bytes) return err - 1;
        if (w.batch.p && ready) {
            KSource bsrc = src;
            bsrc.N = m.N;
            const int rc = volt_internal_batch_step(m, bsrc, TriReduce{nullptr, nullptr, nullptr, 0}, StepTail{}, w.batch);
            if (rc == 1) return 0;
            if (rc) return rc > 0 ? rc : err - 2;
        }
        sk = w.sk;
        if (!ready) sk.tab.p = nullptr;
    }
    if (src.K) return volt_internal_factor(m, src, TriReduce{nullptr, nullptr, nullptr, 0}, sk, nullptr, nullptr);
    const FactorOpts o{src, nullptr, TriReduce{nullptr, nullptr, nullptr, 0}, SplitK{sk.slab, sk.count, 1, 1, sk.rows, (int4*)sk.tab.p, sk.tab.bytes}};
    return run_factor_groups(m.A, m.Winv, m.info, m.B, Np, m.stream, o);
}

int volt_potrf_ws_f32(float* A, float* Winv, int* info, int B, int Np, void* ws, size_t ws_bytes, int ws_flags, void* stream) {
    if (!A) return -1;
    if (!Winv) return -2;
    if (!info) return -3;
    if (B < 0) return -4;
    if (Np < TS || Np % TS) return -5;
    if (B == 0) return 0;
    return potrf_with_scratch(KSource{nullptr, 0, 0, nullptr, 0.f, 0}, StepMats{A, Winv, nullptr, info, B, Np, (hipStream_t)stream}, ws,
                              ws_bytes, ws_flags, -6);
}

int volt_potrf_f32(float* A, float* Winv, int* info, int B, int Np, void* stream) {
    return volt_potrf_ws_f32(A, Winv, info, B, Np, nullptr, 0, 0, stream);
}

int volt_potrf_k_f32(const float* K, int64_t ldk, int64_t bsk, const float* sigma2, float jitter, float* A, float* Winv,
                     int* info, int B, int N, void* ws, size_t ws_bytes, int ws_flags, void* stream) {
    if (!K) return -1;
    if (ldk < N) return -2;
    if (!A) return -6;
    if (!Winv) return -7;
    if (!info) return -8;
    if (B < 0 || B > 65535) return -9;
    if (N < 1) return -10;
    if (B == 0) return 0;
    return potrf_with_scratch(KSource{K, ldk, bsk, sigma2, jitter, N}, StepMats{A, Winv, nullptr, info, B, N, (hipStream_t)stream}, ws,
                              ws_bytes, ws_flags, -11);
}

int volt_trtri_f32(const float* A, const float* Winv, float* Y, int B, int Np, void* stream) {
    if (!A) return -1;
    if (!Winv) return -2;
    if (!Y) return -3;
    if (B < 0) return -4;
    if (Np < TS || Np % TS) return -5;
    if (B == 0) return 0;
    return run_trtri(A, Winv, Y, B, Np, (hipStream_t)stream, nullptr);
}

}
```

### volt_amd/csrc/common.h

```cpp
#pragma once
#include <hip/hip_runtime.h>
#include <stdint.h>
#include "handoff.h"

#define VOLT_ABI_VERSION 5

namespace volt {

constexpr int TS = 128;
constexpr int BK = 32;
constexpr int SLD = BK + 4;
constexpr int NT = 256;
constexpr int STAGE_FLOATS = 2 * TS * SLD;
constexpr int GEMM_LDS_BYTES = 2 * STAGE_FLOATS * 4;

typedef float f32x4 __attribute__((ext_vector_type(4)));
typedef float f32x16 __attribute__((ext_vector_type(16)));

#define VOLT_LAUNCH_CHECK()                                   \
    do {                                                      \
        hipError_t e__ = hipGetLastError();                   \
        if (e__ != hipSuccess) return (int)e__;               \
    } while (0)

__device__ __forceinline__ int accrow(int q, int lane) { return (q & 3) + 8 * (q >> 2) + 4 * (lane >> 5); }

__device__ __forceinline__ void decode_tile_batch(int w, int ntiles, int nbatch, int& tile, int& batch) {
    if ((nbatch & 7) == 0) {
        const int xcd = w & 7, slot = w >> 3;
        batch = (slot / ntiles) * 8 + xcd;
        tile = slot % ntiles;
    } else {
        batch = w / ntiles;
        tile = w % ntiles;
    }
}

__device__ __forceinline__ void decode_tile_batch(int ntiles, int nbatch, int& tile, int& batch) {
    decode_tile_batch((int)blockIdx.x, ntiles, nbatch, tile, batch);
}

struct StageRegs {
    f32x4 a[4], b[4];
};

__device__ __forceinline__ void stage_load(StageRegs& s, const float* __restrict__ A, int64_t lda,
                                           const float* __restrict__ B, int64_t ldb, int k0) {
    const int t = threadIdx.x;
    const int row = t >> 3, cq = (t & 7) * 4;
#pragma unroll
    for (int p = 0; p < 4; ++p) {
        s.a[p] = *reinterpret_cast<const f32x4*>(A + (int64_t)(row + 32 * p) * lda + k0 + cq);
        s.b[p] = *reinterpret_cast<const f32x4*>(B + (int64_t)(row + 32 * p) * ldb + k0 + cq);
    }
}

__device__ __forceinline__ void stage_store(const StageRegs& s, float* __restrict__ buf) {
    const int t = threadIdx.x;
    const int row = t >> 3, cq = (t & 7) * 4;
    float* sA = buf;
    float* sB = buf + TS * SLD;
#pragma unroll
    for (int p = 0; p < 4; ++p) {
        *reinterpret_cast<f32x4*>(sA + (row + 32 * p) * SLD + cq) = s.a[p];
        *reinterpret_cast<f32x4*>(sB + (row + 32 * p) * SLD + cq) = s.b[p];
    }
}

struct StageAddr {
    __amdgpu_buffer_rsrc_t ra, rb;
    int va[4], vb[4];
};

__device__ __forceinline__ StageAddr stage_addr(const float* A, int64_t lda, const float* B, int64_t ldb) {
    StageAddr sa;
    sa.ra = __builtin_amdgcn_make_buffer_rsrc((void*)A, 0, 0x7fffffff, 0x00020000);
    sa.rb = __builtin_amdgcn_make_buffer_rsrc((void*)B, 0, 0x7fffffff, 0x00020000);
    const int t = threadIdx.x;
    const int row = t >> 3, cq = (t & 7) * 4;
#pragma unroll
    for (int p = 0; p < 4; ++p) {
        sa.va[p] = (int)(((int64_t)(row + 32 * p) * lda + cq) * 4);
        sa.vb[p] = (int)(((int64_t)(row + 32 * p) * ldb + cq) * 4);
    }
    return sa;
}

__device__ __forceinline__ void stage_load_buf(StageRegs& s, const StageAddr& sa, int k0) {
    const int so = __builtin_amdgcn_readfirstlane(k0 * 4);
#pragma unroll
    for (int p = 0; p < 4; ++p) {
        s.a[p] = __builtin_bit_cast(f32x4, __builtin_amdgcn_raw_buffer_load_b128(sa.ra, sa.va[p], so, 0));
        s.b[p] = __builtin_bit_cast(f32x4, __builtin_amdgcn_raw_buffer_load_b128(sa.rb, sa.vb[p], so, 0));
    }
}

__device__ __forceinline__ void zero_acc(f32x16 (&acc)[4]) {
#pragma unroll
    for (int i = 0; i < 4; ++i)
#pragma unroll
        for (int q = 0; q < 16; ++q) acc[i][q] = 0.f;
}

template <int WL> struct Frag;
template <> struct Frag<0> { f32x4 a0, a1, b0, b1; };
template <> struct Frag<1> { f32x4 a[4], b0; };

template <int WL>
__device__ __forceinline__ void frag_load(Frag<WL>& f, const float* __restrict__ buf, int kk) {
    const int lane = threadIdx.x & 63, wave = threadIdx.x >> 6;
    const int l31 = lane & 31, lh = lane >> 5;
    const float* sA = buf;
    const float* sB = buf + TS * SLD;
    const int ko = kk * 8 + 4 * lh;
    if constexpr (WL == 0) {
        const int wr = wave >> 1, wc = wave & 1;
        f.a0 = *reinterpret_cast<const f32x4*>(sA + (wr * 64 + l31) * SLD + ko);
        f.b0 = *reinterpret_cast<const f32x4*>(sB + (wc * 64 + l31) * SLD + ko);
        f.b1 = *reinterpret_cast<const f32x4*>(sB + (wc * 64 + 32 + l31) * SLD + ko);
        f.a1 = *reinterpret_cast<const f32x4*>(sA + (wr * 64 + 32 + l31) * SLD + ko);
    } else {
        f.b0 = *reinterpret_cast<const f32x4*>(sB + (wave * 32 + l31) * SLD + ko);
#pragma unroll
        for (int tm = 0; tm < 4; ++tm) f.a[tm] = *reinterpret_cast<const f32x4*>(sA + (tm * 32 + l31) * SLD + ko);
    }
}

template <int WL>
__device__ __forceinline__ void frag_mma_m(const Frag<WL>& f, int m, f32x16 (&acc)[4]) {
    if constexpr (WL == 0) {
        acc[0] = __builtin_amdgcn_mfma_f32_32x32x2f32(f.a0[m], f.b0[m], acc[0], 0, 0, 0);
        acc[1] = __builtin_amdgcn_mfma_f32_32x32x2f32(f.a0[m], f.b1[m], acc[1], 0, 0, 0);
        acc[2] = __builtin_amdgcn_mfma_f32_32x32x2f32(f.a1[m], f.b0[m], acc[2], 0, 0, 0);
        acc[3] = __builtin_amdgcn_mfma_f32_32x32x2f32(f.a1[m], f.b1[m], acc[3], 0, 0, 0);
    } else {
#pragma unroll
        for (int tm = 0; tm < 4; ++tm)
            acc[tm] = __builtin_amdgcn_mfma_f32_32x32x2f32(f.a[tm][m], f.b0[m], acc[tm], 0, 0, 0);
    }
}
template <int WL>
__device__ __forceinline__ void frag_mma(const Frag<WL>& f, f32x16 (&acc)[4]) {
#pragma unroll
    for (int m = 0; m < 4; ++m) frag_mma_m<WL>(f, m, acc);
}

constexpr int SEG_CHUNKS = 4;
__device__ __forceinline__ f32x16 zero16c() {
    f32x16 z;
#pragma unroll
    for (int q = 0; q < 16; ++q) z[q] = 0.f;
    return z;
}
#define VOLT_SB() __builtin_amdgcn_sched_barrier(0)
template <int WL>
__device__ __forceinline__ f32x16 frag_mma_one(const Frag<WL>& f, int m, int t, const f32x16& c) {
    if constexpr (WL == 0) {
        const float a = (t & 2) ? f.a1[m] : f.a0[m], b = (t & 1) ? f.b1[m] : f.b0[m];
        return __builtin_amdgcn_mfma_f32_32x32x2f32(a, b, c, 0, 0, 0);
    } else {
        return __builtin_amdgcn_mfma_f32_32x32x2f32(f.a[t][m], f.b0[m], c, 0, 0, 0);
    }
}
template <int WL>
__device__ __forceinline__ void seg_first_group(const Frag<WL>& f, f32x16 (&P)[4], f32x16 (&T)[4]) {
    const f32x16 z = zero16c();
    P[0] = frag_mma_one<WL>(f, 0, 0, z);
    VOLT_SB();
    T[3] += P[3];
    VOLT_SB();
    P[1] = frag_mma_one<WL>(f, 0, 1, z);
    P[2] = frag_mma_one<WL>(f, 0, 2, z);
    P[3] = frag_mma_one<WL>(f, 0, 3, z);
#pragma unroll
    for (int m = 1; m < 4; ++m) frag_mma_m<WL>(f, m, P);
}
template <int WL>
__device__ __forceinline__ void seg_last_group(const Frag<WL>& f, f32x16 (&P)[4], f32x16 (&T)[4]) {
#pragma unroll
    for (int m = 0; m < 3; ++m) frag_mma_m<WL>(f, m, P);
    P[0] = frag_mma_one<WL>(f, 3, 0, P[0]);
    P[1] = frag_mma_one<WL>(f, 3, 1, P[1]);
    VOLT_SB();
    T[0] += P[0];
    VOLT_SB();
    P[2] = frag_mma_one<WL>(f, 3, 2, P[2]);
    VOLT_SB();
    T[1] += P[1];
    VOLT_SB();
    P[3] = frag_mma_one<WL>(f, 3, 3, P[3]);
    VOLT_SB();
    T[2] += P[2];
    VOLT_SB();
}
enum SegRole { SEG_MID = 0, SEG_FIRST = 1, SEG_LAST = 2 };


__device__ __forceinline__ void stage_store_piece(const StageRegs& s, float* __restrict__ buf, int p) {
    const int t = threadIdx.x;
    const int row = t >> 3, cq = (t & 7) * 4;
    *reinterpret_cast<f32x4*>(buf + (row + 32 * p) * SLD + cq) = s.a[p];
    *reinterpret_cast<f32x4*>(buf + TS * SLD + (row + 32 * p) * SLD + cq) = s.b[p];
}
__device__ __forceinline__ void stage_load_piece(StageRegs& s, const StageAddr& sa, int so, int p) {
    s.a[p] = __builtin_bit_cast(f32x4, __builtin_amdgcn_raw_buffer_load_b128(sa.ra, sa.va[p], so, 0));
    s.b[p] = __builtin_bit_cast(f32x4, __builtin_amdgcn_raw_buffer_load_b128(sa.rb, sa.vb[p], so, 0));
}

template <int WL, bool MORE, bool ST, bool LD, int ROLE = SEG_MID>
__device__ __forceinline__ void chunk_run(const float* cur, float* nxt, Frag<WL>& F0, Frag<WL>& F1, f32x16 (&acc)[4],
                                         f32x16 (&run)[4], StageRegs& s, const StageAddr& sa, int k_ld) {
    frag_load<WL>(F1, cur, 1);
    VOLT_SB();
    if constexpr (ROLE == SEG_FIRST) seg_first_group<WL>(F0, acc, run);
    else frag_mma<WL>(F0, acc);
    VOLT_SB();
    frag_load<WL>(F0, cur, 2);
    VOLT_SB();
#pragma unroll
    for (int m = 0; m < 4; ++m) {
        frag_mma_m<WL>(F1, m, acc);
        if constexpr (ST) stage_store_piece(s, nxt, m);
        VOLT_SB();
    }
    frag_load<WL>(F1, cur, 3);
    VOLT_SB();
    const int so = __builtin_amdgcn_readfirstlane(k_ld * 4);
#pragma unroll
    for (int m = 0; m < 4; ++m) {
        frag_mma_m<WL>(F0, m, acc);
        if constexpr (LD) stage_load_piece(s, sa, so, m);
        VOLT_SB();
    }
    __syncthreads();
    if constexpr (MORE) frag_load<WL>(F0, nxt, 0);
    VOLT_SB();
    if constexpr (ROLE == SEG_LAST) seg_last_group<WL>(F1, acc, run);
    else frag_mma<WL>(F1, acc);
    VOLT_SB();
}

template <int WL, bool CHASE = false, bool LOCALP = false>
__device__ __forceinline__ void gemm_nt_128(const float* __restrict__ A, int64_t lda, const float* __restrict__ B,
                                               int64_t ldb, int nchunks, f32x16 (&acc)[4], float* smem,
                                               const Chase* ch = nullptr, bool* ch_ok = nullptr) {
    if (nchunks <= 0) return;
    int ready = 0;
    if constexpr (CHASE) ready = chase_wait<LOCALP>(*ch, 1, *ch_ok);
    StageRegs s0, s1;
    const StageAddr sa = stage_addr(A, lda, B, ldb);
    stage_load_buf(s0, sa, 0);
    stage_store(s0, smem);
    stage_load_buf(s0, sa, BK);
    stage_load_buf(s1, sa, 2 * BK);
    __syncthreads();
    Frag<WL> F0, F1;
    frag_load<WL>(F0, smem, 0);
    float* b0 = smem;
    float* b1 = smem + STAGE_FLOATS;
    f32x16 P[4];
    P[3] = zero16c();
    int c = 0;
    for (; c + SEG_CHUNKS < nchunks; c += SEG_CHUNKS) {
        if constexpr (CHASE) {
            const int need = (c >> 2) + 2;
            if (ready < need) ready = chase_wait<LOCALP>(*ch, need, *ch_ok);
        }
        chunk_run<WL, true, true, true, SEG_FIRST>(b0, b1, F0, F1, P, acc, s0, sa, (c + 3) * BK);
        chunk_run<WL, true, true, true>(b1, b0, F0, F1, P, acc, s1, sa, (c + 4) * BK);
        chunk_run<WL, true, true, true>(b0, b1, F0, F1, P, acc, s0, sa, (c + 5) * BK);
        chunk_run<WL, true, true, true, SEG_LAST>(b1, b0, F0, F1, P, acc, s1, sa, (c + 6) * BK);
    }
    chunk_run<WL, true, true, true, SEG_FIRST>(b0, b1, F0, F1, P, acc, s0, sa, (c + 3) * BK);
    chunk_run<WL, true, true, false>(b1, b0, F0, F1, P, acc, s1, sa, 0);
    chunk_run<WL, true, true, false>(b0, b1, F0, F1, P, acc, s0, sa, 0);
    chunk_run<WL, false, false, false, SEG_LAST>(b1, b0, F0, F1, P, acc, s1, sa, 0);
    acc[3] += P[3];
    __syncthreads();
}

struct TriTile {
    const float* X;  int64_t ldx;
    const float* Z;  int64_t ldz;
    int n1;
    const float* W;
    const int* flag;
    int want;
    Chase ch;
};

#ifndef VOLT_Z_AUX
#define VOLT_Z_AUX 2
#endif
struct TriSrc {
    __amdgpu_buffer_rsrc_t ra, rb, rw;
    int va, vb, vw;
    int pa, pb;
    int n1, nall;
};

template <int KIND = -1>
__device__ __forceinline__ void tri_load_piece(StageRegs& s, const TriSrc& ts, int c, int p) {
    if constexpr (KIND == 0) return;
    if (KIND == 1 || (KIND < 0 && c < ts.n1)) {
        const int sa = __builtin_amdgcn_readfirstlane(c * BK * 4 + p * ts.pa);
        const int sb = __builtin_amdgcn_readfirstlane(c * BK * 4 + p * ts.pb);
        s.a[p] = __builtin_bit_cast(f32x4, __builtin_amdgcn_raw_buffer_load_b128(ts.ra, ts.va, sa, 0));
        s.b[p] = __builtin_bit_cast(f32x4, __builtin_amdgcn_raw_buffer_load_b128(ts.rb, ts.vb, sb, VOLT_Z_AUX));
    } else {
        const int so = __builtin_amdgcn_readfirstlane((c - ts.n1) * BK * 4 + p * (32 * TS * 4));
        s.b[p] = __builtin_bit_cast(f32x4, __builtin_amdgcn_raw_buffer_load_b128(ts.rw, ts.vw, so, 0));
    }
}
template <int KIND = -1>
__device__ __forceinline__ void tri_store_piece(const StageRegs& s, float* __restrict__ buf, const TriSrc& ts, int c, int p) {
    if constexpr (KIND == 0) return;
    const int t = threadIdx.x;
    const int row = t >> 3, cq = (t & 7) * 4;
    if (KIND == 1 || (KIND < 0 && c < ts.n1)) *reinterpret_cast<f32x4*>(buf + (row + 32 * p) * SLD + cq) = s.a[p];
    *reinterpret_cast<f32x4*>(buf + TS * SLD + (row + 32 * p) * SLD + cq) = s.b[p];
}

template <bool MORE, int STK, int LDK, int ROLE = SEG_MID>
__device__ __forceinline__ void tri_chunk_p1(const float* cur, float* nxt, int c, Frag<1>& F0, Frag<1>& F1,
                                             f32x16 (&P)[4], f32x16 (&T)[4], StageRegs& s, const TriSrc& ts) {
    frag_load<1>(F1, cur, 1);
    VOLT_SB();
    if constexpr (ROLE == SEG_FIRST) seg_first_group<1>(F0, P, T);
    else frag_mma<1>(F0, P);
    VOLT_SB();
    frag_load<1>(F0, cur, 2);
    VOLT_SB();
#pragma unroll
    for (int m = 0; m < 4; ++m) {
        frag_mma_m<1>(F1, m, P);
        tri_store_piece<STK>(s, nxt, ts, c + 1, m);
        VOLT_SB();
    }
    frag_load<1>(F1, cur, 3);
    VOLT_SB();
#pragma unroll
    for (int m = 0; m < 4; ++m) {
        frag_mma_m<1>(F0, m, P);
        tri_load_piece<LDK>(s, ts, c + 3, m);
        VOLT_SB();
    }
    __syncthreads();
    if constexpr (MORE) frag_load<1>(F0, nxt, 0);
    VOLT_SB();
    if constexpr (ROLE == SEG_LAST) seg_last_group<1>(F1, P, T);
    else frag_mma<1>(F1, P);
    VOLT_SB();
}

struct FragW { f32x4 w[4]; };
__device__ __forceinline__ void fragw_load(FragW& f, const float* __restrict__ buf, int tp, int g) {
    const int lane = threadIdx.x & 63, l31 = lane & 31, lh = lane >> 5;
    const float* sB = buf + TS * SLD;
#pragma unroll
    for (int rb = 0; rb < 4; ++rb)
        if (rb >= tp) f.w[rb] = *reinterpret_cast<const f32x4*>(sB + (rb * 32 + l31) * SLD + 8 * g + 4 * lh);
}
__device__ __forceinline__ void fragw_mma_m(const FragW& f, const f32x16& Ttp, int tp, int g, int m, f32x16 (&O)[4]) {
    const float a = Ttp[4 * g + m];
#pragma unroll
    for (int rb = 0; rb < 4; ++rb)
        if (rb >= tp) O[rb] = __builtin_amdgcn_mfma_f32_32x32x2f32(a, f.w[rb][m], O[rb], 0, 0, 0);
}

template <int TP>
__device__ __forceinline__ void tri_chunk_p2(const float* cur, float* nxt, f32x16 (&T)[4], f32x16 (&O)[4],
                                             StageRegs& s, const TriSrc& ts) {
    const int c = ts.n1 + TP;
    FragW G0, G1;
    fragw_load(G0, cur, TP, 0);
    fragw_load(G1, cur, TP, 1);
    VOLT_SB();
#pragma unroll
    for (int m = 0; m < 4; ++m) fragw_mma_m(G0, T[TP], TP, 0, m, O);
    VOLT_SB();
    fragw_load(G0, cur, TP, 2);
    VOLT_SB();
#pragma unroll
    for (int m = 0; m < 4; ++m) {
        fragw_mma_m(G1, T[TP], TP, 1, m, O);
        if (TP < 3) tri_store_piece<2>(s, nxt, ts, c + 1, m);
        VOLT_SB();
    }
    fragw_load(G1, cur, TP, 3);
    VOLT_SB();
#pragma unroll
    for (int m = 0; m < 4; ++m) {
        fragw_mma_m(G0, T[TP], TP, 2, m, O);
        if (TP == 0) tri_load_piece<2>(s, ts, c + 3, m);
        VOLT_SB();
    }
    __syncthreads();
#pragma unroll
    for (int m = 0; m < 4; ++m) fragw_mma_m(G1, T[TP], TP, 3, m, O);
    VOLT_SB();
}

template <bool CHASE = false, bool LOCALP = false>
__device__ __forceinline__ bool tri_tile_run(const TriTile& t, f32x16 (&T)[4], f32x16 (&O)[4], float* smem,
                                             const ChasePre* pre = nullptr) {
    const int tid = threadIdx.x;
    const int srow = tid >> 3, scq = (tid & 7) * 4;
    TriSrc ts;
    ts.ra = __builtin_amdgcn_make_buffer_rsrc((void*)t.X, 0, 0x7fffffff, 0x00020000);
    ts.rb = __builtin_amdgcn_make_buffer_rsrc((void*)t.Z, 0, 0x7fffffff, 0x00020000);
    ts.rw = __builtin_amdgcn_make_buffer_rsrc((void*)t.W, 0, TS * TS * 4, 0x00020000);
    ts.va = (int)(((int64_t)srow * t.ldx + scq) * 4);
    ts.vb = (int)(((int64_t)srow * t.ldz + scq) * 4);
    ts.vw = (srow * TS + scq) * 4;
    ts.pa = (int)(32 * t.ldx * 4);
    ts.pb = (int)(32 * t.ldz * 4);
    ts.n1 = t.n1;
    ts.nall = t.n1 + 4;
    bool ok = true;
    int ready = 0;
    if constexpr (CHASE) {
        if (t.n1 > 0) ready = pre ? chase_wait_pre<LOCALP>(t.ch, *pre, 1, ok) : chase_wait<LOCALP>(t.ch, 1, ok);
    }
    if (t.flag && t.n1 == 0) {
        ok = flag_wait_one_lane<LOCALP>(t.flag, t.want);
        __syncthreads();
    }
    StageRegs s0, s1;
    float* b0 = smem;
    float* b1 = smem + STAGE_FLOATS;
#pragma unroll
    for (int p = 0; p < 4; ++p) tri_load_piece(s0, ts, 0, p);
#pragma unroll
    for (int p = 0; p < 4; ++p) tri_store_piece(s0, b0, ts, 0, p);
#pragma unroll
    for (int p = 0; p < 4; ++p) tri_load_piece(s0, ts, 1, p);
#pragma unroll
    for (int p = 0; p < 4; ++p) tri_load_piece(s1, ts, 2, p);
    __syncthreads();
    int c = 0;
    if (t.n1 > 0) {
        Frag<1> F0, F1;
        frag_load<1>(F0, b0, 0);
        O[3] = zero16c();
        for (; c + SEG_CHUNKS < t.n1; c += SEG_CHUNKS) {
            if constexpr (CHASE) {
                const int need = (c >> 2) + 2;
                if (ready < need) ready = chase_wait<LOCALP>(t.ch, need, ok);
            }
            tri_chunk_p1<true, 1, 1, SEG_FIRST>(b0, b1, c, F0, F1, O, T, s0, ts);
            tri_chunk_p1<true, 1, 1>(b1, b0, c + 1, F0, F1, O, T, s1, ts);
            tri_chunk_p1<true, 1, 1>(b0, b1, c + 2, F0, F1, O, T, s0, ts);
            tri_chunk_p1<true, 1, 1, SEG_LAST>(b1, b0, c + 3, F0, F1, O, T, s1, ts);
        }
        if (t.flag) ok = flag_wait_one_lane<LOCALP>(t.flag, t.want) && ok;
        tri_chunk_p1<true, 1, 1, SEG_FIRST>(b0, b1, c, F0, F1, O, T, s0, ts);
        tri_chunk_p1<true, 1, 2>(b1, b0, c + 1, F0, F1, O, T, s1, ts);
        tri_chunk_p1<true, 1, 2>(b0, b1, c + 2, F0, F1, O, T, s0, ts);
        tri_chunk_p1<false, 2, 2, SEG_LAST>(b1, b0, c + 3, F0, F1, O, T, s1, ts);
        c += SEG_CHUNKS;
        T[3] += O[3];
    }
    zero_acc(O);
    tri_chunk_p2<0>(b0, b1, T, O, s0, ts);
    tri_chunk_p2<1>(b1, b0, T, O, s1, ts);
    tri_chunk_p2<2>(b0, b1, T, O, s0, ts);
    tri_chunk_p2<3>(b1, b0, T, O, s1, ts);
    __syncthreads();
    return ok;
}

__device__ __forceinline__ void tri_phase1_only(const TriTile& t, f32x16 (&T)[4], float* smem) {
    const int tid = threadIdx.x;
    const int srow = tid >> 3, scq = (tid & 7) * 4;
    TriSrc ts;
    ts.ra = __builtin_amdgcn_make_buffer_rsrc((void*)t.X, 0, 0x7fffffff, 0x00020000);
    ts.rb = __builtin_amdgcn_make_buffer_rsrc((void*)t.Z, 0, 0x7fffffff, 0x00020000);
    ts.rw = ts.ra;
    ts.va = (int)(((int64_t)srow * t.ldx + scq) * 4);
    ts.vb = (int)(((int64_t)srow * t.ldz + scq) * 4);
    ts.vw = 0;
    ts.pa = (int)(32 * t.ldx * 4);
    ts.pb = (int)(32 * t.ldz * 4);
    ts.n1 = t.n1;
    ts.nall = t.n1;
    StageRegs s0, s1;
    float* b0 = smem;
    float* b1 = smem + STAGE_FLOATS;
#pragma unroll
    for (int p = 0; p < 4; ++p) tri_load_piece(s0, ts, 0, p);
#pragma unroll
    for (int p = 0; p < 4; ++p) tri_store_piece(s0, b0, ts, 0, p);
#pragma unroll
    for (int p = 0; p < 4; ++p) tri_load_piece(s0, ts, 1, p);
#pragma unroll
    for (int p = 0; p < 4; ++p) tri_load_piece(s1, ts, 2, p);
    __syncthreads();
    Frag<1> F0, F1;
    frag_load<1>(F0, b0, 0);
    int c = 0;
    f32x16 P[4];
    P[3] = zero16c();
    for (; c + SEG_CHUNKS < t.n1; c += SEG_CHUNKS) {
        tri_chunk_p1<true, 1, 1, SEG_FIRST>(b0, b1, c, F0, F1, P, T, s0, ts);
        tri_chunk_p1<true, 1, 1>(b1, b0, c + 1, F0, F1, P, T, s1, ts);
        tri_chunk_p1<true, 1, 1>(b0, b1, c + 2, F0, F1, P, T, s0, ts);
        tri_chunk_p1<true, 1, 1, SEG_LAST>(b1, b0, c + 3, F0, F1, P, T, s1, ts);
    }
    tri_chunk_p1<true, 1, 1, SEG_FIRST>(b0, b1, c, F0, F1, P, T, s0, ts);
    tri_chunk_p1<true, 1, 0>(b1, b0, c + 1, F0, F1, P, T, s1, ts);
    tri_chunk_p1<true, 1, 0>(b0, b1, c + 2, F0, F1, P, T, s0, ts);
    tri_chunk_p1<false, 0, 0, SEG_LAST>(b1, b0, c + 3, F0, F1, P, T, s1, ts);
    T[3] += P[3];
    __syncthreads();
}

template <int CTRL>
__device__ __forceinline__ float dpp_add(float x) {
    return x + __int_as_float(__builtin_amdgcn_update_dpp(0, __float_as_int(x), CTRL, 0xf, 0xf, true));
}
__device__ __forceinline__ float wave_sum_f(float x) {
    x = dpp_add<0xB1>(x);
    x = dpp_add<0x4E>(x);
    x = dpp_add<0x141>(x);
    x = dpp_add<0x140>(x);
    const int xi = __float_as_int(x);
    const float r0 = __int_as_float(__builtin_amdgcn_readlane(xi, 0));
    const float r1 = __int_as_float(__builtin_amdgcn_readlane(xi, 16));
    const float r2 = __int_as_float(__builtin_amdgcn_readlane(xi, 32));
    const float r3 = __int_as_float(__builtin_amdgcn_readlane(xi, 48));
    return (r0 + r1) + (r2 + r3);
}

__device__ __forceinline__ void rowpair_dot(const f32x4& y, const f32x4& z, float& lo, float& hi) {
    float p = __builtin_fmaf(y[0], z[0], y[1] * z[1]) + __builtin_fmaf(y[2], z[2], y[3] * z[3]);
    p = dpp_add<0xB1>(p);
    p = dpp_add<0x4E>(p);
    p = dpp_add<0x141>(p);
    p = dpp_add<0x140>(p);
    const int pi = __float_as_int(p);
    lo = __int_as_float(__builtin_amdgcn_readlane(pi, 0)) + __int_as_float(__builtin_amdgcn_readlane(pi, 16));
    hi = __int_as_float(__builtin_amdgcn_readlane(pi, 32)) + __int_as_float(__builtin_amdgcn_readlane(pi, 48));
}

__device__ __forceinline__ double log_pivot_product(const float (&dg)[16], int nvalid_mask) {
    double prod = 1.0;
    bool ok = true;
#pragma unroll
    for (int u = 0; u < 16; ++u)
        if ((nvalid_mask >> u) & 1) {
            ok = ok && (dg[u] > 0.f);
            prod *= (double)dg[u];
        }
    if (!ok) return __builtin_nan("");
    if (prod > 1e-280 && prod < 1e280) return log(prod);
    double s = 0.0;
#pragma unroll 1
    for (int u = 0; u < 16; ++u)
        if ((nvalid_mask >> u) & 1) s += log((double)dg[u]);
    return s;
}

}
```

### volt_amd/csrc/host.h

```cpp
#pragma once
#include <hip/hip_runtime.h>
#include <stddef.h>
#include <stdint.h>
#include <mutex>

struct Tunables {
    int groups = 2;
    int splitk_target = 512, splitk_minl = 2, splitk_maxs = 8, splitk_groups = 2, splitk_maxb = 22;
    int sched = 1, sched_minb = 3, sched_maxb = 31, sched_maxb_potrf = 64;
    int sched_g = 256, sched_s = 4, sched_groups = 2, sched_kmin = -1;
    float sched_frac = 0.6f;
    int small_nmax = 8, small_maxwg = 1150;
    int plain_spread = 320, split_spread = 700;
    int long_split = 1;
    int long_xcd = 0;
    int long_on = 1, long_first = 0, long_emin = 1, long_pad = 1, long_nmin = 2;
    int small_maxb = 40, small_maxb2 = 64;
    int small_pad_maxb = 40;
    int cus = 256, xccs = 8;
    int group_gate = 700;
    int batch = 1;
    int batch_order = -1;
    int batch_lad = 0;
    int batch_spread = 400;
    int batch64 = 1;
    int batch64_max = 3300;
    int batch64_max_step = 2500;
    int batch_local = 1;
    int batch_pullers = 1;
    int long_pullers = 1;
    int rollout_lane = 1;
    int batch_xskew = 0, batch_xdrop = 0;
    int f64_lookahead = -1;
    int f64_trtri_lookahead = -1;
    int f64_spread = 512;
    int f64_split_target = 512;
};
const Tunables& tunables();

namespace volt {

inline size_t al256(size_t x) { return (x + 255) & ~(size_t)255; }

struct KSource {
    const float* K;
    int64_t ldk, bsk;
    const float* sigma2;
    float jitter;
    int N;
};
struct KSource64 {
    const double* K;
    int64_t ldk, bsk;
    const double* sigma2;
    double jitter;
    int N;
};
struct TriReduce {
    const float* rpad;
    float* zpart;
    float* frob;
    int N;
};

struct StepMats {
    float *A, *Winv, *Y;
    int* info;
    int B, N;
    hipStream_t stream;
};
struct StepMats64 {
    double *A, *Winv, *Y;
    int* info;
    int B, Np;
    hipStream_t stream;
};
struct StepTail {
    const float* resid;
    float *rpad, *z, *apad, *apart, *out, *alpha;
};
struct Region {
    void* p = nullptr;
    size_t bytes = 0;
};
struct SplitScratch {
    float* slab;
    int* count;
    int rows;
    Region tab;
};
struct ProfileOut {
    float *ms_sum, *ms_union;
    int* launches;
    float* per_launch;
};

inline bool batch_local_handoffs(int B) { return (B & 7) == 0 && tunables().batch_local != 0 && tunables().xccs == 8; }
inline int begin_grid(int direct, int strided) {
    int blocks = ((direct > strided ? direct : strided) + 255) / 256;
    if (blocks > 256) blocks = 256;
    if (blocks * 256 < direct) blocks = (direct + 255) / 256;
    return blocks;
}

}

typedef void (*volt_group_post_fn)(void* ctx, int b0, int Bg, hipStream_t s);
struct VoltAux {
    hipStream_t aux, aux2, aux3, aux4;
    hipEvent_t fork, ev[12];
    std::mutex* mu;
};
bool volt_internal_aux(VoltAux* out);
size_t volt_internal_sched_bytes(int B, int n);
int volt_internal_sched_install(volt::Region tab, int B, int n, int has_y, int cap, void* stream);
int volt_internal_factor(const volt::StepMats& m, const volt::KSource& src, const volt::TriReduce& red, const volt::SplitScratch& sk,
                         volt_group_post_fn post, void* post_ctx);
int volt_internal_profile(const volt::StepMats& m, const volt::KSource& src, const volt::TriReduce& red, const volt::SplitScratch& sk,
                          int groups, volt_group_post_fn post, void* post_ctx, const volt::ProfileOut& out);
size_t volt_internal_small_bytes(int B, int n);
int volt_internal_small_install(volt::Region state, int B, int n, void* stream);
int volt_internal_small_step(const volt::StepMats& m, const volt::KSource& src, const volt::TriReduce& red, const volt::StepTail& t,
                             volt::Region state);
size_t volt_internal_long_bytes(int B, int n);
size_t volt_internal_long_slab_floats(int B, int n);
int volt_internal_long_install(volt::Region state, int B, int n, void* stream);
int volt_internal_long_step(const volt::StepMats& m, const volt::KSource& src, const volt::TriReduce& red, const volt::StepTail& t,
                            float* eslab, volt::Region state);
bool volt_internal_batch_applies(int B, int n, int has_y);
size_t volt_internal_batch_bytes(int B, int n, int has_y);
bool volt_internal_batch_first();
int volt_internal_batch_install(volt::Region state, int B, int n, int has_y, void* stream);
int volt_internal_batch_step(const volt::StepMats& m, const volt::KSource& src, const volt::TriReduce& red, const volt::StepTail& t,
                             volt::Region state, hipEvent_t e0 = nullptr, hipEvent_t e1 = nullptr);
int volt_internal_factor_f64(const volt::StepMats64& m, volt::Region state = {});
bool volt_internal_batch64_applies(int B, int n, int has_y);
size_t volt_internal_batch64_bytes(int B, int n, int has_y);
int volt_internal_batch64_step(const volt::StepMats64& m, volt::Region state, const volt::KSource64* ksrc = nullptr);
size_t volt_internal_batch64_trtri_bytes(int B, int n);
int volt_internal_batch64_trtri(const double* A, const double* Winv, double* Y, int B, int Np, volt::Region state, void* stream);
const float* volt_internal_mll_y(void* workspace, int B, int N);
```

### volt_amd/csrc/mll.hip

```cpp
#include "common.h"
#include "host.h"
#include "../../include/volt_hip.h"
#include "../../include/volt_hip_tune.h"
#include <math.h>

namespace volt {

__global__ void pad_resid_kernel(const float* __restrict__ resid, float* __restrict__ rpad, int N, int Np) {
    const int b = blockIdx.y;
    const int i = blockIdx.x * blockDim.x + threadIdx.x;
    if (i < Np) rpad[(int64_t)b * Np + i] = (i < N) ? resid[(int64_t)b * N + i] : 0.f;
}

__global__ void sum_zpart_kernel(const float* __restrict__ zpart, float* __restrict__ z, int Np) {
    const int n = Np / TS;
    const int b = blockIdx.y;
    const int c = blockIdx.x * blockDim.x + threadIdx.x;
    if (c >= Np) return;
    const int cb = c / TS;
    float a = 0.f;
    for (int jb = 0; jb <= cb; ++jb) a += zpart[((int64_t)b * n + jb) * Np + c];
    z[(int64_t)b * Np + c] = a;
}

__global__ __launch_bounds__(256) void y_times_z_kernel(const float* __restrict__ Y, const float* __restrict__ z,
                                                        float* __restrict__ alpha, int Np, int B) {
    int rb, b;
    decode_tile_batch(Np / 16, B, rb, b);
    const int lane = threadIdx.x & 63, wave = threadIdx.x >> 6, l31 = lane & 31, h = lane >> 5;
    const int j0 = rb * 16 + wave * 4;
    const float* Yb = Y + (int64_t)b * Np * Np;
    const float* zb = z + (int64_t)b * Np;
    const int n = Np / TS;
    float acc[4] = {0.f, 0.f, 0.f, 0.f};
    const float* y0 = Yb + (int64_t)(j0 + h) * Np + 4 * l31;
    const float* y1 = Yb + (int64_t)(j0 + 2 + h) * Np + 4 * l31;
    for (int c = j0 / TS; c < n; ++c) {
        const f32x4 zv = *reinterpret_cast<const f32x4*>(zb + c * TS + 4 * l31);
        const f32x4 ya = *reinterpret_cast<const f32x4*>(y0 + c * TS);
        const f32x4 yb = *reinterpret_cast<const f32x4*>(y1 + c * TS);
        float lo, hi;
        rowpair_dot(ya, zv, lo, hi);
        acc[0] += lo;
        acc[1] += hi;
        rowpair_dot(yb, zv, lo, hi);
        acc[2] += lo;
        acc[3] += hi;
    }
    if (lane == 0) {
#pragma unroll
        for (int r = 0; r < 4; ++r) alpha[(int64_t)b * Np + j0 + r] = acc[r];
    }
}

__global__ __launch_bounds__(256) void alpha_sum_kernel(const float* __restrict__ apart, float* __restrict__ alpha_pad, int N,
                                                        int Np) {
    const int n = Np / TS, b = blockIdx.y;
    const int i = blockIdx.x * 256 + threadIdx.x;
    if (i >= Np) return;
    float al = 0.f;
    if (i < N)
        for (int c = i / TS; c < n; ++c) al += apart[((int64_t)b * n + c) * Np + i];
    alpha_pad[(int64_t)b * Np + i] = al;
}

__global__ __launch_bounds__(256) void mll_scalars_kernel(const float* __restrict__ A, const float* __restrict__ z,
                                                          const float* __restrict__ alpha_pad,
                                                          const float* __restrict__ frob, const float* __restrict__ sigma2,
                                                          float jitter, float* __restrict__ out,
                                                          float* __restrict__ alpha_out, int N, int Np, int want_grad) {
    __shared__ double red[256];
    const int b = blockIdx.x, tid = threadIdx.x;
    const int n = Np / TS;
    const float* Ab = A + (int64_t)b * Np * Np;
    auto block_sum = [&](double v) -> double {
        red[tid] = v;
        __syncthreads();
        for (int s = 128; s > 0; s >>= 1) {
            if (tid < s) red[tid] += red[tid + s];
            __syncthreads();
        }
        const double r = red[0];
        __syncthreads();
        return r;
    };
    double q = 0, ld = 0, aa = 0, tr = 0;
    constexpr int CPT = 16;
    for (int c0 = tid; c0 < Np; c0 += CPT * 256) {
        float al[CPT], dg[CPT], zz[CPT];
#pragma unroll
        for (int u = 0; u < CPT; ++u) {
            const int c = c0 + u * 256, cc = c < N ? c : N - 1;
            dg[u] = Ab[(int64_t)cc * Np + cc];
            zz[u] = z[(int64_t)b * Np + cc];
            al[u] = 0.f;
            if (want_grad) al[u] = alpha_pad[(int64_t)b * Np + cc];
        }
        int valid = 0;
#pragma unroll
        for (int u = 0; u < CPT; ++u) {
            const int c = c0 + u * 256;
            if (c < N) {
                const double zi = zz[u];
                q += zi * zi;
                valid |= 1 << u;
                if (want_grad) {
                    aa += (double)al[u] * al[u];
                    alpha_out[(int64_t)b * N + c] = al[u];
                }
            }
        }
        ld += log_pivot_product(dg, valid);
    }
    if (want_grad) {
        const int nt = n * (n + 1) / 2;
        for (int i = tid; i < nt; i += 256) tr += frob[(int64_t)b * nt + i];
    }
    q = block_sum(q);
    ld = 2.0 * block_sum(ld);
    aa = block_sum(aa);
    tr = block_sum(tr);
    if (tid == 0) {
        const double LOG_2PI = 1.8378770664093453;
        float* o = out + (int64_t)b * 8;
        o[0] = (float)(-0.5 * (q + ld + N * LOG_2PI) / N);
        o[2] = (float)q;
        o[3] = (float)ld;
        o[6] = (sigma2 ? sigma2[b] : 0.f) + jitter;
        o[7] = 0.f;
        if (want_grad) {
            o[1] = (float)(0.5 * (aa - tr) / N);
            o[4] = (float)tr;
            o[5] = (float)aa;
        }
    }
}

__device__ __forceinline__ double wave_sum_d(double x) {
#pragma unroll
    for (int o = 32; o > 0; o >>= 1) x += __shfl_xor(x, o);
    return x;
}
__global__ __launch_bounds__(256) void refine_resid_kernel(const float* __restrict__ K, int64_t ldk, int64_t bsk,
                                                           const float* __restrict__ resid, const float* __restrict__ alpha,
                                                           const float* __restrict__ sigma2, float jitter,
                                                           float* __restrict__ r1pad, int N, int Np) {
    const int b = blockIdx.y;
    const int lane = threadIdx.x & 63, wave = threadIdx.x >> 6;
    const int i = blockIdx.x * 4 + wave;
    if (i >= Np) return;
    if (i >= N) {
        if (lane == 0) r1pad[(int64_t)b * Np + i] = 0.f;
        return;
    }
    const float* Ki = K + (int64_t)b * bsk + (int64_t)i * ldk;
    const float* ab = alpha + (int64_t)b * N;
    double acc = 0.0;
    const bool vec = ((ldk & 3) == 0) && ((bsk & 3) == 0) && (((uintptr_t)K & 15) == 0) && ((N & 3) == 0) && (((uintptr_t)alpha & 15) == 0);
    if (vec) {
        for (int j = lane * 4; j < N; j += 256) {
            const f32x4 kv = *reinterpret_cast<const f32x4*>(Ki + j);
            const f32x4 av = *reinterpret_cast<const f32x4*>(ab + j);
            acc += ((double)kv[0] * av[0] + (double)kv[1] * av[1]) + ((double)kv[2] * av[2] + (double)kv[3] * av[3]);
        }
    } else {
        for (int j = lane; j < N; j += 64) acc += (double)Ki[j] * ab[j];
    }
    acc = wave_sum_d(acc);
    if (lane == 0) {
        const double s = (double)(sigma2 ? sigma2[b] : 0.f) + (double)jitter;
        r1pad[(int64_t)b * Np + i] = (float)((double)resid[(int64_t)b * N + i] - acc - s * (double)ab[i]);
    }
}
__global__ __launch_bounds__(256) void refine_finish_kernel(const float* __restrict__ delta_pad, const float* __restrict__ resid,
                                                            float* __restrict__ alpha, float* __restrict__ out, int N, int Np) {
    __shared__ double red[2][256];
    const int b = blockIdx.x, tid = threadIdx.x;
    double q = 0, aa = 0;
    for (int i = tid; i < N; i += 256) {
        const float an = alpha[(int64_t)b * N + i] + delta_pad[(int64_t)b * Np + i];
        alpha[(int64_t)b * N + i] = an;
        q += (double)resid[(int64_t)b * N + i] * an;
        aa += (double)an * an;
    }
    red[0][tid] = q;
    red[1][tid] = aa;
    __syncthreads();
    for (int s = 128; s > 0; s >>= 1) {
        if (tid < s) { red[0][tid] += red[0][tid + s]; red[1][tid] += red[1][tid + s]; }
        __syncthreads();
    }
    if (tid == 0) {
        const double LOG_2PI = 1.8378770664093453;
        float* o = out + (int64_t)b * 8;
        o[0] = (float)(-0.5 * (red[0][0] + (double)o[3] + N * LOG_2PI) / N);
        o[1] = (float)(0.5 * (red[1][0] - (double)o[4]) / N);
        o[2] = (float)red[0][0];
        o[5] = (float)red[1][0];
        o[7] = 1.f;
    }
}

struct MllWs {
    float *A, *Winv, *Y, *rpad, *z, *scratch, *apad, *zpart, *frob, *apart;
    SplitScratch sk;
    Region small;
    Region lng;
    float* eslab;
    Region batch;
    size_t bytes;
};

static MllWs carve(void* base, int B, int N, int want_grad) {
    const size_t Np = (size_t)volt_padded_n(N), n = Np / TS;
    size_t off = 0;
    auto take = [&](size_t floats) {
        float* p = base ? reinterpret_cast<float*>(reinterpret_cast<char*>(base) + off) : nullptr;
        off += al256(floats * sizeof(float));
        return p;
    };
    MllWs w;
    w.A = take((size_t)B * Np * Np);
    w.Winv = take((size_t)B * n * TS * TS);
    w.rpad = take((size_t)B * Np);
    w.z = take((size_t)B * Np);
    w.scratch = take((size_t)B * Np);
    w.apad = take((size_t)B * Np);
    if (want_grad) {
        w.Y = take((size_t)B * Np * Np);
        w.zpart = take((size_t)B * n * Np);
        w.frob = take((size_t)B * (n * (n + 1) / 2));
    } else {
        w.Y = w.zpart = w.frob = nullptr;
    }
    w.sk.rows = B < 32 ? 64 : (!want_grad && B <= 64 ? 128 : 0);
    w.sk.slab = w.sk.rows ? take((size_t)w.sk.rows * (n + 1) * TS * TS) : nullptr;
    w.sk.count = w.sk.rows ? reinterpret_cast<int*>(take((size_t)(n + 1) * (n + 1) * B)) : nullptr;
    auto region = [&](size_t bytes) { return Region{bytes ? take(bytes / sizeof(float)) : nullptr, bytes}; };
    w.sk.tab = region(w.sk.rows ? volt_internal_sched_bytes(B, (int)n) : 0);
    w.small = region(want_grad ? volt_internal_small_bytes(B, (int)n) : 0);
    w.lng = region(want_grad ? volt_internal_long_bytes(B, (int)n) : 0);
    w.eslab = w.lng.bytes ? take(volt_internal_long_slab_floats(B, (int)n)) : nullptr;
    const size_t batch_bytes = volt_internal_batch_bytes(B, (int)n, want_grad);
    w.apart = (w.small.bytes || w.lng.bytes || (want_grad && batch_bytes)) ? take((size_t)B * n * Np) : nullptr;
    w.batch = region(batch_bytes);
    w.bytes = off;
    return w;
}

}

using namespace volt;

namespace {
struct TailCtx {
    volt::MllWs w;
    const float* sigma2;
    float jitter;
    float* out;
    float* alpha;
    int N, Np, want_grad;
};

void mll_tail(void* vctx, int b0, int Bg, hipStream_t s) {
    const TailCtx& c = *static_cast<const TailCtx*>(vctx);
    const int Np = c.Np, n = Np / TS;
    const int64_t mat = (int64_t)Np * Np;
    float* z = c.w.z + (int64_t)b0 * Np;
    float* apad = c.w.apad + (int64_t)b0 * Np;
    const float* A = c.w.A + b0 * mat;
    if (c.want_grad) {
        const float* Y = c.w.Y + b0 * mat;
        hipLaunchKernelGGL(sum_zpart_kernel, dim3((Np + 255) / 256, Bg), dim3(256), 0, s,
                           c.w.zpart + (int64_t)b0 * n * Np, z, Np);
        hipLaunchKernelGGL(y_times_z_kernel, dim3((Np / 16) * Bg), dim3(256), 0, s, Y, z, apad, Np, Bg);
    } else {
        (void)volt_trsv_lower_f32(A, c.w.Winv + (int64_t)b0 * n * TS * TS, c.w.rpad + (int64_t)b0 * Np, z,
                                  c.w.scratch + (int64_t)b0 * Np, Bg, Np, (void*)s);
    }
    hipLaunchKernelGGL(mll_scalars_kernel, dim3(Bg), dim3(256), 0, s, A, z, apad,
                       c.want_grad ? c.w.frob + (int64_t)b0 * (n * (n + 1) / 2) : nullptr,
                       c.sigma2 ? c.sigma2 + b0 : nullptr, c.jitter, c.out + (int64_t)b0 * 8,
                       c.alpha ? c.alpha + (int64_t)b0 * c.N : nullptr, c.N, Np, c.want_grad);
}
void batch_tail(TailCtx& c, int B, hipStream_t s) {
    if (!c.want_grad) {
        mll_tail(&c, 0, B, s);
        return;
    }
    hipLaunchKernelGGL(alpha_sum_kernel, dim3((c.Np + 255) / 256, B), dim3(256), 0, s, c.w.apart, c.w.apad, c.N, c.Np);
    hipLaunchKernelGGL(mll_scalars_kernel, dim3(B), dim3(256), 0, s, c.w.A, c.w.z, c.w.apad, c.w.frob, c.sigma2, c.jitter, c.out,
                       c.alpha, c.N, c.Np, 1);
}

struct StepArgs {
    StepMats m;
    KSource src;
    TriReduce red;
    StepTail t;
};
StepArgs step_args(const TailCtx& c, const float* K, int64_t ldk, int64_t bsk, const float* resid, int* info, int B, hipStream_t s) {
    const volt::MllWs& w = c.w;
    return {StepMats{w.A, w.Winv, w.Y, info, B, c.N, s}, KSource{K, ldk, bsk, c.sigma2, c.jitter, c.N},
            TriReduce{w.rpad, w.zpart, w.frob, c.N}, StepTail{resid, w.rpad, w.z, w.apad, w.apart, c.out, c.alpha}};
}
void pad_resid(const StepArgs& a, const TailCtx& c) {
    hipLaunchKernelGGL(pad_resid_kernel, dim3((c.Np + 255) / 256, a.m.B), dim3(256), 0, a.m.stream, a.t.resid, a.t.rpad, c.N, c.Np);
}
int try_batch_step(const StepArgs& a, TailCtx& c, hipEvent_t e0 = nullptr, hipEvent_t e1 = nullptr) {
    pad_resid(a, c);
    const int rc = volt_internal_batch_step(a.m, a.src, a.red, a.t, c.w.batch, e0, e1);
    if (rc == 1) batch_tail(c, a.m.B, a.m.stream);
    return rc;
}
}

const float* volt_internal_mll_y(void* workspace, int B, int N) { return carve(workspace, B, N, 1).Y; }

extern "C" {

size_t volt_mll_workspace_bytes(int B, int N, int want_grad) {
    if (B <= 0 || N <= 0) return 0;
    return carve(nullptr, B, N, want_grad).bytes;
}

int volt_mll_workspace_init_f32(void* workspace, int B, int N, int want_grad, void* stream) {
    if (!workspace || ((uintptr_t)workspace & 255)) return -1;
    if (B < 1 || B > 65535) return -2;
    if (N < 1) return -3;
    MllWs w = carve(workspace, B, N, want_grad);
    const int n = volt_padded_n(N) / TS;
    int rc;
    if (w.small.p && (rc = volt_internal_small_install(w.small, B, n, stream))) return rc;
    if (w.lng.p && (rc = volt_internal_long_install(w.lng, B, n, stream))) return rc;
    if (w.batch.p && (rc = volt_internal_batch_install(w.batch, B, n, want_grad, stream))) return rc;
    if (!w.sk.tab.p) return 0;
    return volt_internal_sched_install(w.sk.tab, B, n, want_grad, w.sk.rows, stream);
}

int volt_mll_step_f32(const float* K, int64_t ldk, int64_t bsk, const float* resid, const float* sigma2, float jitter,
                      float* out, float* alpha, int* info, void* workspace, int B, int N, int flags,
                      void* stream) {
    const int want_grad = flags & VOLT_WANT_GRAD;
    const bool ready = (flags & VOLT_WS_INITIALISED) != 0;
    if (!K) return -1;
    if (ldk < N) return -2;
    if (!resid) return -4;
    if (!out) return -7;
    if (want_grad && !alpha) return -8;
    if (!info) return -9;
    if (!workspace || ((uintptr_t)workspace & 255)) return -10;
    if (B < 0 || B > 65535) return -11;
    if (N < 1) return -12;
    if (B == 0) return 0;
    hipStream_t s = (hipStream_t)stream;
    const int Np = volt_padded_n(N);
    TailCtx ctx{carve(workspace, B, N, want_grad), sigma2, jitter, out, alpha, N, Np, want_grad};
    const MllWs& w = ctx.w;
    const StepArgs a = step_args(ctx, K, ldk, bsk, resid, info, B, s);
    int rc = 0;
    if (ready && w.batch.p && volt_internal_batch_first()) rc = try_batch_step(a, ctx);
    if (rc == 0 && ready && want_grad && w.lng.p && w.apart && w.eslab)
        rc = volt_internal_long_step(a.m, a.src, a.red, a.t, w.eslab, w.lng);
    if (rc == 0 && ready && want_grad && w.small.p && w.apart)
        rc = volt_internal_small_step(a.m, a.src, a.red, a.t, w.small);
    if (rc == 0 && ready && w.batch.p) rc = try_batch_step(a, ctx);
    if (rc == 0) {
        pad_resid(a, ctx);
        TriReduce red = a.red;
        if (!want_grad) red.rpad = nullptr;
        SplitScratch sk = w.sk;
        if (!ready) sk.tab.p = nullptr;
        rc = volt_internal_factor(a.m, a.src, red, sk, mll_tail, &ctx);
    } else if (rc == 1) {
        rc = 0;
    }
    if (rc) return rc > 0 ? rc : -1;
    if (want_grad && (flags & VOLT_REFINE_ALPHA)) {
        hipLaunchKernelGGL(refine_resid_kernel, dim3((Np + 3) / 4, B), dim3(256), 0, s, K, ldk, bsk, resid, alpha, sigma2, jitter,
                           w.rpad, N, Np);
        if ((rc = volt_trsv_lower_f32(w.A, w.Winv, w.rpad, w.z, w.scratch, B, Np, stream))) return rc > 0 ? rc : -1;
        if ((rc = volt_trsv_lower_t_f32(w.A, w.Winv, w.z, w.apad, w.scratch, B, Np, stream))) return rc > 0 ? rc : -1;
        hipLaunchKernelGGL(refine_finish_kernel, dim3(B), dim3(256), 0, s, w.apad, resid, alpha, out, N, Np);
    }
    VOLT_LAUNCH_CHECK();
    return 0;
}

int volt_profile_step_f32(const float* K, int64_t ldk, int64_t bsk, const float* resid, const float* sigma2,
                          float* out, float* alpha, void* workspace, int* info, int B, int N, int groups, void* stream,
                          float* ms_sum_host, float* ms_union_host, int* launches_host, float* per_launch_host) {
    if (!K) return -1;
    if (ldk < N) return -2;
    if (!resid) return -4;
    if (!out) return -6;
    if (!alpha) return -7;
    if (!workspace || ((uintptr_t)workspace & 255)) return -8;
    if (!info) return -9;
    if (B < 1 || B > 65535) return -10;
    if (N < 1) return -11;
    if (!ms_sum_host) return -14;
    if (!ms_union_host) return -15;
    if (!launches_host) return -16;
    TailCtx ctx{carve(workspace, B, N, 1), sigma2, 0.f, out, alpha, N, volt_padded_n(N), 1};
    const StepArgs a = step_args(ctx, K, ldk, bsk, resid, info, B, (hipStream_t)stream);
    if (groups == 0 && ctx.w.batch.p) {
        hipEvent_t e0 = nullptr, e1 = nullptr;
        if (hipEventCreate(&e0) != hipSuccess || hipEventCreate(&e1) != hipSuccess) return (int)hipGetLastError();
        int rc = try_batch_step(a, ctx, e0, e1);
        if (rc == 1) {
            hipError_t e = hipStreamSynchronize((hipStream_t)stream);
            float ms = 0.f;
            if (e == hipSuccess) e = hipEventElapsedTime(&ms, e0, e1);
            ms_sum_host[0] = ms_union_host[0] = ms;
            ms_sum_host[1] = ms_union_host[1] = 0.f;
            launches_host[0] = 1;
            launches_host[1] = 0;
            if (per_launch_host) per_launch_host[0] = ms;
            rc = e != hipSuccess ? (int)e : 0;
        } else if (rc == 0) {
            rc = -8;
        }
        (void)hipEventDestroy(e0);
        (void)hipEventDestroy(e1);
        return rc;
    }
    pad_resid(a, ctx);
    return volt_internal_profile(a.m, a.src, a.red, ctx.w.sk, groups, mll_tail, &ctx,
                                 ProfileOut{ms_sum_host, ms_union_host, launches_host, per_launch_host});
}

}
```

### volt_amd/csrc/tiles.h

```cpp
#pragma once
#include "common.h"
#include "host.h"

namespace volt {


__device__ __forceinline__ float input_elem(const KSource& src, const float* Kb, float add, const float* Ab, int Np,
                                            bool usek, int gi, int gj) {
    if (usek) {
        float v = (gi < src.N && gj < src.N) ? Kb[(int64_t)gi * src.ldk + gj] : 0.f;
        if (gi == gj) v = (gi < src.N) ? v + add : 1.f;
        return v;
    }
    return Ab[(int64_t)gi * Np + gj];
}

template <bool FROMK, int ABL = 0, bool CHASE = false, bool LOCALP = false>
__device__ __forceinline__ void update_body(float* __restrict__ A, int Np, int rowblk, int colblk, int kb0, int kb1,
                                            bool fromk, int b, const KSource& src, float* smem,
                                            bool to_image = false, const Chase* ch = nullptr, bool* ch_ok = nullptr) {
    float* Ab = A + (int64_t)b * Np * Np;
    const float* Arows = Ab + (int64_t)rowblk * TS * Np + (int64_t)kb0 * TS;
    const float* Brows = Ab + (int64_t)colblk * TS * Np + (int64_t)kb0 * TS;
    const int lane = threadIdx.x & 63, wave = threadIdx.x >> 6;
    const int wr = wave >> 1, wc = wave & 1;
    float* C = Ab + (int64_t)rowblk * TS * Np + (int64_t)colblk * TS;
    f32x16 acc[4];
    const bool usek = FROMK && fromk;
    const float add = usek ? ((src.sigma2 ? src.sigma2[b] : 0.f) + src.jitter) : 0.f;
    const float* Kb = usek ? src.K + (int64_t)b * src.bsk : nullptr;
#pragma unroll
    for (int tm = 0; tm < 2; ++tm)
#pragma unroll
        for (int tn = 0; tn < 2; ++tn)
#pragma unroll
            for (int q = 0; q < 16; ++q) {
                const int r = wr * 64 + tm * 32 + accrow(q, lane);
                const int c = wc * 64 + tn * 32 + (lane & 31);
                if (ABL & 1) acc[tm * 2 + tn][q] = 0.f;
                else acc[tm * 2 + tn][q] = -input_elem(src, Kb, add, Ab, Np, usek, rowblk * TS + r, colblk * TS + c);
            }
    gemm_nt_128<0, CHASE, LOCALP>(Arows, Np, Brows, Np, (kb1 - kb0) * (TS / BK), acc, smem, ch, ch_ok);
    if (ABL & 2) {
        float sum = 0.f;
#pragma unroll
        for (int t4 = 0; t4 < 4; ++t4)
#pragma unroll
            for (int q = 0; q < 16; ++q) sum += acc[t4][q];
        C[(int64_t)(threadIdx.x >> 1) * Np + (threadIdx.x & 1)] = sum;
        return;
    }
    if (to_image) {
        __syncthreads();
#pragma unroll
        for (int tm = 0; tm < 2; ++tm)
#pragma unroll
            for (int tn = 0; tn < 2; ++tn)
#pragma unroll
                for (int q = 0; q < 16; ++q) {
                    const int r = wr * 64 + tm * 32 + accrow(q, lane);
                    const int c = wc * 64 + tn * 32 + (lane & 31);
                    smem[r * (TS + 1) + c] = (c <= r) ? -acc[tm * 2 + tn][q] : 0.f;
                }
        return;
    }
#pragma unroll
    for (int tm = 0; tm < 2; ++tm)
#pragma unroll
        for (int tn = 0; tn < 2; ++tn)
#pragma unroll
            for (int q = 0; q < 16; ++q) {
                const int r = wr * 64 + tm * 32 + accrow(q, lane);
                const int c = wc * 64 + tn * 32 + (lane & 31);
                C[(int64_t)r * Np + c] = -acc[tm * 2 + tn][q];
            }
}

constexpr int DT = TS + 1;
constexpr int DIAG_LDS_FLOATS = TS * DT;

__device__ __forceinline__ f32x16 mm32_lds_lds(f32x16 acc, const float* __restrict__ A, const float* __restrict__ B) {
    const int lane = threadIdx.x & 63, l31 = lane & 31, lh = lane >> 5;
    float av[16], bv[16];
#pragma unroll
    for (int s2 = 0; s2 < 16; ++s2) {
        const int kk = 2 * s2 + lh;
        av[s2] = A[l31 * DT + kk];
        bv[s2] = B[kk * DT + l31];
    }
    VOLT_SB();
#pragma unroll
    for (int s2 = 0; s2 < 16; ++s2) acc = __builtin_amdgcn_mfma_f32_32x32x2f32(av[s2], bv[s2], acc, 0, 0, 0);
    return acc;
}
__device__ __forceinline__ f32x16 mm32_lds_reg(f32x16 acc, const float* __restrict__ A, const f32x16& Breg) {
    const int lane = threadIdx.x & 63, l31 = lane & 31, lh = lane >> 5;
    float av[16];
#pragma unroll
    for (int q = 0; q < 16; ++q) av[q] = A[l31 * DT + (q & 3) + 8 * (q >> 2) + 4 * lh];
    VOLT_SB();
#pragma unroll
    for (int q = 0; q < 16; ++q) acc = __builtin_amdgcn_mfma_f32_32x32x2f32(av[q], Breg[q], acc, 0, 0, 0);
    return acc;
}

template <bool NEG>
__device__ __forceinline__ f32x16 mm32_nt(f32x16 acc, const float* __restrict__ A, const float* __restrict__ B) {
    const int lane = threadIdx.x & 63, l31 = lane & 31, lh = lane >> 5;
    float av[16], bv[16];
#pragma unroll
    for (int s2 = 0; s2 < 16; ++s2) {
        const int kk = 2 * s2 + lh;
        av[s2] = A[l31 * DT + kk];
        bv[s2] = B[l31 * DT + kk];
    }
    VOLT_SB();
#pragma unroll
    for (int s2 = 0; s2 < 16; ++s2)
        acc = __builtin_amdgcn_mfma_f32_32x32x2f32(NEG ? -av[s2] : av[s2], bv[s2], acc, 0, 0, 0);
    return acc;
}

__device__ __forceinline__ float lane_bcast(float v, int src) {
    return __int_as_float(__builtin_amdgcn_readlane(__float_as_int(v), src));
}

#define VOLT_RL "v_readlane_b32 "
__device__ __forceinline__ void rl_fma3(float& c0, float& c1, float& c2, float b0, float b1, float b2, float s0,
                                        float s1, float s2, int l0, int l1, int l2) {
    float t0, t1, t2;
    asm volatile(VOLT_RL "%3, %9, %12\n\t" VOLT_RL "%4, %10, %13\n\t" VOLT_RL "%5, %11, %14\n\t"
                 "v_fma_f32 %0, -%6, %3, %0\n\tv_fma_f32 %1, -%7, %4, %1\n\tv_fma_f32 %2, -%8, %5, %2"
                 : "+v"(c0), "+v"(c1), "+v"(c2), "=&s"(t0), "=&s"(t1), "=&s"(t2)
                 : "v"(b0), "v"(b1), "v"(b2), "v"(s0), "v"(s1), "v"(s2), "i"(l0), "i"(l1), "i"(l2));
}
__device__ __forceinline__ void rl_fma2(float& c0, float& c1, float b0, float b1, float s0, float s1, int l0, int l1) {
    float t0, t1;
    asm volatile(VOLT_RL "%2, %6, %8\n\t" VOLT_RL "%3, %7, %9\n\ts_nop 0\n\t"
                 "v_fma_f32 %0, -%4, %2, %0\n\tv_fma_f32 %1, -%5, %3, %1"
                 : "+v"(c0), "+v"(c1), "=&s"(t0), "=&s"(t1)
                 : "v"(b0), "v"(b1), "v"(s0), "v"(s1), "i"(l0), "i"(l1));
}
__device__ __forceinline__ void settle(float& v) { asm volatile("s_nop 0" : "+v"(v)); }

__device__ __forceinline__ void rl_fma1(float& c0, float b0, float s0, int l0) {
    float t0;
    asm volatile(VOLT_RL "%1, %3, %4\n\ts_nop 1\n\tv_fma_f32 %0, -%2, %1, %0"
                 : "+v"(c0), "=&s"(t0)
                 : "v"(b0), "v"(s0), "i"(l0));
}

#define VOLT_STAMP(i)                                                                  \
    do {                                                                               \
        if (STAMP && threadIdx.x == 0) stamps[i] = __builtin_amdgcn_s_memtime();       \
    } while (0)

template <int J0, int J1>
__device__ __forceinline__ void pivots16(float (&a)[32], float (&rv)[32], int& npos) {
    settle(a[J0]);
    float d = lane_bcast(a[J0], J0);
    float rinv = __builtin_amdgcn_rsqf(d);
#pragma unroll
    for (int j = J0; j < J1; ++j) {
        npos += (d > 0.f) ? 1 : 0;
        rv[j] = rinv;
        float l = a[j] * rinv;
        settle(l);
        a[j] = l;
        float rnext = 0.f;
        if (j + 1 < J1) {
            rl_fma1(a[j + 1], l, l, j + 1);
            settle(a[j + 1]);
            d = lane_bcast(a[j + 1], j + 1);
            rnext = __builtin_amdgcn_rsqf(d);
        }
        int c = j + 2;
#pragma unroll
        for (; c + 2 < J1; c += 3) rl_fma3(a[c], a[c + 1], a[c + 2], l, l, l, l, l, l, c, c + 1, c + 2);
        if (c + 1 < J1) rl_fma2(a[c], a[c + 1], l, l, l, l, c, c + 1);
        else if (c < J1) rl_fma1(a[c], l, l, c);
        rinv = rnext;
    }
}
template <int R0, int R1>
__device__ __forceinline__ void invert16(const float (&a)[32], const float (&rv)[32], float (&x)[32], int l31) {
#pragma unroll
    for (int r = R0; r < R1; ++r) x[r] = (r == l31) ? 1.f : 0.f;
#pragma unroll
    for (int m = R0; m < R1; ++m) {
        const float xm = x[m] * rv[m];
        x[m] = xm;
        int r = m + 1;
#pragma unroll
        for (; r + 2 < R1; r += 3) rl_fma3(x[r], x[r + 1], x[r + 2], xm, xm, xm, a[m], a[m], a[m], r, r + 1, r + 2);
        if (r + 1 < R1) rl_fma2(x[r], x[r + 1], xm, xm, a[m], a[m], r, r + 1);
        else if (r < R1) rl_fma1(x[r], xm, a[m], r);
    }
}
__device__ __forceinline__ void wave_lds_fence() {
    __builtin_amdgcn_fence(__ATOMIC_RELEASE, "wavefront");
    __builtin_amdgcn_wave_barrier();
    __builtin_amdgcn_fence(__ATOMIC_ACQUIRE, "wavefront");
}

constexpr int PSC = 17;
constexpr int PIVOT_SCRATCH_FLOATS = 2 * 16 * PSC;
static_assert(DIAG_LDS_FLOATS + 3 * PIVOT_SCRATCH_FLOATS <= 2 * STAGE_FLOATS, "pivot scratch must fit behind the image");

template <bool STAMP = false>
__device__ __forceinline__ void pivot_phase(float* __restrict__ sT, int kb, int prow, float (&a)[32], int& npos,
                                            long long* stamps = nullptr) {
    const int lane = threadIdx.x & 63, wave = threadIdx.x >> 6, l31 = lane & 31, l15 = lane & 15, g = lane >> 4;
    const bool panel = prow >= 0;
    const bool prw = panel && lane >= 32;
    const bool low = !prw && l31 >= 16;
    float* Dk = sT + (32 * kb) * DT + 32 * kb;
    float* Rw = prw ? sT + (32 * prow + l31) * DT + 32 * kb : Dk + l31 * DT;
    float* S21 = sT + DIAG_LDS_FLOATS + wave * PIVOT_SCRATCH_FLOATS;
    float* S22 = S21 + 16 * PSC;
    float rv[32];
#pragma unroll
    for (int c = 0; c < 16; ++c) a[c] = Rw[c];
    if (STAMP && kb == 1) VOLT_STAMP(16);
    pivots16<0, 16>(a, rv, npos);
    if (STAMP && kb == 1) VOLT_STAMP(17);
    {
        float* dst = prw ? Rw : S21 + (l31 & 15) * PSC;
        if (prw || low) {
#pragma unroll
            for (int c = 0; c < 16; ++c) dst[c] = a[c];
        }
    }
    wave_lds_fence();
    float v21[4];
#pragma unroll
    for (int s = 0; s < 4; ++s) v21[s] = S21[l15 * PSC + 4 * s + g];
    {
        f32x4 c22;
#pragma unroll
        for (int q = 0; q < 4; ++q) c22[q] = Dk[(16 + 4 * g + q) * DT + 16 + l15];
#pragma unroll
        for (int s = 0; s < 4; ++s) c22 = __builtin_amdgcn_mfma_f32_16x16x4f32(-v21[s], v21[s], c22, 0, 0, 0);
#pragma unroll
        for (int q = 0; q < 4; ++q) S22[(4 * g + q) * PSC + l15] = c22[q];
    }
    if (panel) {
        float* Pk = sT + (32 * prow) * DT + 32 * kb;
#pragma unroll
        for (int t = 0; t < 2; ++t) {
            f32x4 cp;
#pragma unroll
            for (int q = 0; q < 4; ++q) cp[q] = Pk[(16 * t + 4 * g + q) * DT + 16 + l15];
#pragma unroll
            for (int s = 0; s < 4; ++s)
                cp = __builtin_amdgcn_mfma_f32_16x16x4f32(-Pk[(16 * t + l15) * DT + 4 * s + g], v21[s], cp, 0, 0, 0);
#pragma unroll
            for (int q = 0; q < 4; ++q) Pk[(16 * t + 4 * g + q) * DT + 16 + l15] = cp[q];
        }
    }
    wave_lds_fence();
    if (STAMP && kb == 1) VOLT_STAMP(18);
    {
        const float* src = prw ? Rw + 16 : S22 + (l31 & 15) * PSC;
#pragma unroll
        for (int c = 0; c < 16; ++c) {
            const float t = src[c];
            a[16 + c] = (prw || low) ? t : 0.f;
        }
    }
    if (STAMP && kb == 1) VOLT_STAMP(19);
    pivots16<16, 32>(a, rv, npos);
    if (STAMP && kb == 1) VOLT_STAMP(20);
    if (prw) {
#pragma unroll
        for (int c = 16; c < 32; ++c) Rw[c] = a[c];
    }
}

__device__ __forceinline__ __amdgpu_buffer_rsrc_t w_rsrc(float* W) {
    return __builtin_amdgcn_make_buffer_rsrc((void*)W, 0, TS * TS * 4, 0x00020000);
}
template <int AUX = 0>
__device__ __forceinline__ void w_store(__amdgpu_buffer_rsrc_t rs, int voff, int soff, float v) {
    __builtin_amdgcn_raw_buffer_store_b32(__float_as_uint(v), rs, voff, soff, AUX);
}
template <bool SLABS = false>
__device__ __forceinline__ void x_block(float* __restrict__ sT, int kb, __amdgpu_buffer_rsrc_t rs) {
    constexpr int AUX = SLABS ? AUX_SC1 : 0;
    constexpr bool store00 = SLABS;
    const int lane = threadIdx.x & 63, l15 = lane & 15, g = lane >> 4, h = lane >> 5;
    const bool up = (lane & 16) != 0;
    float* Dk = sT + (32 * kb) * DT + 32 * kb;
    const float* Lh = Dk + (16 * h) * DT + 16 * h;
    float v21[4];
#pragma unroll
    for (int s = 0; s < 4; ++s) v21[s] = Dk[(16 + l15) * DT + 4 * s + g];
    float x[16];
#pragma unroll
    for (int r = 0; r < 16; ++r) {
        float acc = (r == l15) ? 1.f : 0.f;
#pragma unroll
        for (int m = 0; m < r; ++m) acc = __builtin_fmaf(-Lh[r * DT + m], x[m], acc);
        const float d = Lh[r * DT + r];
        const float ri = __builtin_amdgcn_rcpf(d);
        x[r] = acc * __builtin_fmaf(__builtin_fmaf(-d, ri, 1.f), ri, ri);
    }
    wave_lds_fence();
    if (!up) {
#pragma unroll
        for (int r = 0; r < 16; ++r) Dk[(16 * h + r) * DT + 16 * h + l15] = x[r];
    }
    wave_lds_fence();
    f32x4 t21 = {0.f, 0.f, 0.f, 0.f}, r21 = {0.f, 0.f, 0.f, 0.f};
#pragma unroll
    for (int s = 0; s < 4; ++s)
        t21 = __builtin_amdgcn_mfma_f32_16x16x4f32(v21[s], Dk[(4 * s + g) * DT + l15], t21, 0, 0, 0);
#pragma unroll
    for (int q = 0; q < 4; ++q)
        r21 = __builtin_amdgcn_mfma_f32_16x16x4f32(Dk[(16 + l15) * DT + 16 + 4 * g + q], t21[q], r21, 0, 0, 0);
    const int wbase = (32 * kb * TS + 32 * kb) * 4;
#pragma unroll
    for (int q = 0; q < 4; ++q) {
        Dk[(16 + 4 * g + q) * DT + l15] = -r21[q];
        w_store<AUX>(rs, wbase + ((16 + 4 * g) * TS + l15) * 4, q * TS * 4, -r21[q]);
    }
    if (!up || h == 0) {
        const int voff = wbase + (up ? 16 + l15 : (16 * h) * TS + 16 * h + l15) * 4;
        if (kb != 0 || lane != 0 || store00) w_store<AUX>(rs, voff, 0, up ? 0.f : x[0]);
#pragma unroll
        for (int r = 1; r < 16; ++r) w_store<AUX>(rs, voff, r * TS * 4, up ? 0.f : x[r]);
    }
}

__device__ __forceinline__ f32x16 zero16() {
    f32x16 z;
#pragma unroll
    for (int q = 0; q < 16; ++q) z[q] = 0.f;
    return z;
}
__device__ __forceinline__ void w_out(__amdgpu_buffer_rsrc_t rs, int i, int j, float* __restrict__ blk, const f32x16& R) {
    const int lane = threadIdx.x & 63;
    const int voff = ((32 * i + 4 * (lane >> 5)) * TS + 32 * j + (lane & 31)) * 4;
#pragma unroll
    for (int q = 0; q < 16; ++q) {
        w_store(rs, voff, ((q & 3) + 8 * (q >> 2)) * TS * 4, -R[q]);
        if (blk) blk[accrow(q, lane) * DT + (lane & 31)] = -R[q];
    }
}

template <bool STAMP = false, bool SLABS = false, bool LOCALPUB = false>
__device__ __forceinline__ void diag_body(float* __restrict__ A, float* __restrict__ Winv, int* __restrict__ info,
                                          int Np, int k, int b, float* smem, long long* stamps = nullptr,
                                          bool loaded = false, int* ready = nullptr, int ready_val = 0,
                                          int* slab = nullptr, int* pre = nullptr) {
    float* sT = smem;
    VOLT_STAMP(0);
    const int n = Np / TS;
    float* D = A + (int64_t)b * Np * Np + (int64_t)k * TS * Np + (int64_t)k * TS;
    float* W = Winv + ((int64_t)b * n + k) * TS * TS;
    const int tid = threadIdx.x;
    const int lane = tid & 63, wave = tid >> 6, l31 = lane & 31;

    if (!loaded) {
        f32x4 v[TS * TS / 4 / NT];
#pragma unroll
        for (int it = 0; it < TS * TS / 4 / NT; ++it) {
            const int e = tid + it * NT, r = e >> 5, c = (e & 31) * 4;
            v[it] = f32x4{0.f, 0.f, 0.f, 0.f};
            if (c <= r) v[it] = *reinterpret_cast<const f32x4*>(D + (int64_t)r * Np + c);
        }
#pragma unroll
        for (int it = 0; it < TS * TS / 4 / NT; ++it) {
            const int e = tid + it * NT, r = e >> 5, c = (e & 31) * 4;
#pragma unroll
            for (int q = 0; q < 4; ++q) sT[r * DT + c + q] = (c + q <= r) ? v[it][q] : 0.f;
        }
    }
    __syncthreads();
    VOLT_STAMP(1);

    auto blk = [&](int i, int j) { return sT + (32 * i) * DT + 32 * j; };
    const __amdgpu_buffer_rsrc_t wrs = w_rsrc(W);
    auto trail = [&](int i, int j, int m) {
        float* C = blk(i, j);
        f32x16 acc;
#pragma unroll
        for (int q = 0; q < 16; ++q) acc[q] = C[accrow(q, lane) * DT + l31];
        acc = mm32_nt<true>(acc, blk(i, m), blk(j, m));
#pragma unroll
        for (int q = 0; q < 16; ++q) C[accrow(q, lane) * DT + l31] = acc[q];
    };
    auto park_l = [&](int kb, const float (&a)[32]) {
        if (lane < 32) {
            float* Dgk = D + (int64_t)(32 * kb + l31) * Np + 32 * kb;
            float* Dk = blk(kb, kb) + l31 * DT;
#pragma unroll
            for (int c4 = 0; c4 < 8; ++c4) {
                f32x4 v;
#pragma unroll
                for (int q = 0; q < 4; ++q) {
                    v[q] = (4 * c4 + q <= l31) ? a[4 * c4 + q] : 0.f;
                    Dk[4 * c4 + q] = v[q];
                }
                *reinterpret_cast<f32x4*>(Dgk + 4 * c4) = v;
            }
        }
    };
    int bad = 0;
#pragma unroll 1
    for (int kb = 0; kb <= 4; ++kb) {
        float a[32];
        f32x16 P = zero16();
        const int npw = kb > 3 ? 0 : (kb == 3 ? 1 : 3 - kb);
        const int xw = kb == 1 ? 2 : (kb == 4 ? 0 : 1);
        if (wave < npw) {
            int npos = 0;
            pivot_phase<STAMP>(sT, kb, kb < 3 ? kb + 1 + wave : -1, a, npos, stamps);
            if (npos != 32 && bad == 0) {
#pragma unroll
                for (int j = 0; j < 32; ++j) {
                    const float ljj = lane_bcast(a[j], j);
                    if (!(ljj > 0.f) && bad == 0) bad = 32 * kb + j + 1;
                }
            }
            if (kb == 3) park_l(3, a);
        } else if (kb >= 1 && wave == xw) {
            x_block<SLABS>(sT, kb - 1, wrs);
            if (SLABS) {
                const int c = kb - 1, row = lane >> 1, c0 = 16 * (lane & 1);
                const __amdgpu_buffer_rsrc_t drs = __builtin_amdgcn_make_buffer_rsrc((void*)D, 0, 0x7fffffff, 0x00020000);
                for (int i = c + 1; i <= 3; ++i) {
                    const float* src = blk(i, c) + row * DT + c0;
                    const int voff = (int)((((int64_t)(32 * i + row)) * Np + 32 * c + c0) * 4);
#pragma unroll
                    for (int q4 = 0; q4 < 4; ++q4) {
                        const f32x4 v = {src[4 * q4], src[4 * q4 + 1], src[4 * q4 + 2], src[4 * q4 + 3]};
                        __builtin_amdgcn_raw_buffer_store_b128(__builtin_bit_cast(u32x4, v), drs, voff, 16 * q4, AUX_SC1);
                    }
                }
                asm volatile("s_waitcnt vmcnt(0)" ::: "memory");
                if (lane == 0) __hip_atomic_store(slab + c, ready_val, __ATOMIC_RELAXED, __HIP_MEMORY_SCOPE_AGENT);
            }
        } else if (kb == 0) {
            if (SLABS && pre && lane == 0) {
                __builtin_amdgcn_fence(__ATOMIC_RELEASE, "agent");
                __hip_atomic_store(pre, ready_val, __ATOMIC_RELAXED, __HIP_MEMORY_SCOPE_AGENT);
            }
            const u32x4 z = {0u, 0u, 0u, 0u};
            const int voff = ((lane >> 3) * TS + 4 * (lane & 7)) * 4;
#pragma unroll
            for (int i = 0; i < 3; ++i)
#pragma unroll
                for (int j = i + 1; j <= 3; ++j)
#pragma unroll
                    for (int it = 0; it < 4; ++it)
                        __builtin_amdgcn_raw_buffer_store_b128(z, wrs, voff, ((32 * i + 8 * it) * TS + 32 * j) * 4, 0);
        } else if (wave == 3 && kb <= 2) {
            for (int i = kb + 1; i <= 3; ++i)
                for (int j = kb + 1; j <= i; ++j) trail(i, j, kb - 1);
        } else if (kb == 3 && wave == 2) {
            f32x16 S = mm32_lds_lds(zero16(), blk(1, 0), blk(0, 0));
            w_out(wrs, 1, 0, blk(0, 1), mm32_lds_reg(zero16(), blk(1, 1), S));
        } else if (kb == 4 && wave == 1) {
            f32x16 S = mm32_lds_lds(zero16(), blk(2, 0), blk(0, 0));
            S = mm32_lds_lds(S, blk(2, 1), blk(0, 1));
            w_out(wrs, 2, 0, blk(0, 2), mm32_lds_reg(zero16(), blk(2, 2), S));
        } else if (kb == 4 && wave == 2) {
            f32x16 S = mm32_lds_lds(zero16(), blk(2, 1), blk(1, 1));
            w_out(wrs, 2, 1, blk(1, 2), mm32_lds_reg(zero16(), blk(2, 2), S));
            P = mm32_lds_lds(P, blk(3, 1), blk(1, 1));
        } else if (kb == 4 && wave == 3) {
            P = mm32_lds_lds(P, blk(3, 0), blk(0, 0));
            P = mm32_lds_lds(P, blk(3, 1), blk(0, 1));
        }
        if (STAMP && kb == 1 && lane == 0) stamps[21 + wave] = __builtin_amdgcn_s_memtime();
        if (STAMP && kb == 3 && lane == 0) stamps[25 + wave] = __builtin_amdgcn_s_memtime();
        __syncthreads();
        VOLT_STAMP(2 + 2 * kb);
        if (kb == 4) {
            if (wave == 3) {
                P = mm32_lds_lds(P, blk(3, 2), blk(0, 2));
                w_out(wrs, 3, 0, nullptr, mm32_lds_reg(zero16(), blk(3, 3), P));
            } else if (wave == 2) {
                P = mm32_lds_lds(P, blk(3, 2), blk(1, 2));
                w_out(wrs, 3, 1, nullptr, mm32_lds_reg(zero16(), blk(3, 3), P));
            } else if (wave == 1) {
                f32x16 S = mm32_lds_lds(zero16(), blk(3, 2), blk(2, 2));
                w_out(wrs, 3, 2, nullptr, mm32_lds_reg(zero16(), blk(3, 3), S));
            }
        }
        if (kb >= 3) continue;
        if (wave == 0) park_l(kb, a);
        if (kb + 1 + wave <= 3) trail(kb + 1 + wave, kb + 1, kb);
        __syncthreads();
        VOLT_STAMP(3 + 2 * kb);
    }
    if (tid == 0 && bad) atomicCAS(info + b, 0, k * TS + bad);
    VOLT_STAMP(11);
    asm volatile("s_waitcnt vmcnt(0)" ::: "memory");
    __syncthreads();
    VOLT_STAMP(12);
    if (tid == 0) {
        const int bits = __float_as_int(sT[0]);
        if constexpr (LOCALPUB) {
            *reinterpret_cast<volatile int*>(W) = bits ? bits : 0x7fc00000;
        } else {
            __builtin_amdgcn_fence(__ATOMIC_RELEASE, "agent");
            __hip_atomic_store(reinterpret_cast<int*>(W), bits ? bits : 0x7fc00000, __ATOMIC_RELAXED, __HIP_MEMORY_SCOPE_AGENT);
        }
        if (ready) __hip_atomic_store(ready, ready_val, __ATOMIC_RELAXED, __HIP_MEMORY_SCOPE_AGENT);
    }
    VOLT_STAMP(13);
    for (int e = tid; e < TS * TS / 4; e += NT) {
        const int r = e >> 5, c = (e & 31) * 4;
        if ((r >> 5) != (c >> 5)) {
            f32x4 v;
#pragma unroll
            for (int q = 0; q < 4; ++q) v[q] = (c < r) ? sT[r * DT + c + q] : 0.f;
            *reinterpret_cast<f32x4*>(D + (int64_t)r * Np + c) = v;
        }
    }
    VOLT_STAMP(14);
}

constexpr int WLD = TS + 4;


#ifndef VOLT_OUT_NT
#define VOLT_OUT_NT 1
#endif
#if VOLT_OUT_NT
#define VOLT_OUT_STORE(p, v) __builtin_nontemporal_store((v), (p))
#else
#define VOLT_OUT_STORE(p, v) (*(p) = (v))
#endif
__device__ __forceinline__ void tri_store(const f32x16 (&O)[4], float* __restrict__ Out, int64_t ldo) {
    const int lane = threadIdx.x & 63, wave = threadIdx.x >> 6, l31 = lane & 31;
#pragma unroll
    for (int rb = 0; rb < 4; ++rb)
#pragma unroll
        for (int q = 0; q < 16; ++q) {
            const int c = wave * 32 + accrow(q, lane);
            const int r = rb * 32 + l31;
            VOLT_OUT_STORE(Out + (int64_t)c * ldo + r, -O[rb][q]);
        }
}

template <int AUX>
__device__ __forceinline__ void tri_store_aux(const f32x16 (&O)[4], float* __restrict__ Out, int64_t ldo) {
    const int lane = threadIdx.x & 63, wave = threadIdx.x >> 6, l31 = lane & 31;
    const __amdgpu_buffer_rsrc_t rs = __builtin_amdgcn_make_buffer_rsrc((void*)Out, 0, 0x7fffffff, 0x00020000);
    const int voff = (int)((((int64_t)(wave * 32 + 4 * (lane >> 5))) * ldo + l31) * 4);
    const int ld4 = (int)(ldo * 4);
#pragma unroll
    for (int rb = 0; rb < 4; ++rb)
#pragma unroll
        for (int q = 0; q < 16; ++q)
            __builtin_amdgcn_raw_buffer_store_b32(__float_as_uint(-O[rb][q]), rs, voff, ((q & 3) + 8 * (q >> 2)) * ld4 + rb * 128, AUX);
}

template <int AUX>
__device__ __forceinline__ void tri_store_lds(const f32x16 (&O)[4], float* __restrict__ Out, int64_t ldo, float* smem) {
    const int lane = threadIdx.x & 63, wave = threadIdx.x >> 6, l31 = lane & 31, lh = lane >> 5;
    float* mine = smem + wave * 32 * WLD;
#pragma unroll
    for (int rb = 0; rb < 4; ++rb)
#pragma unroll
        for (int q = 0; q < 16; ++q) mine[accrow(q, lane) * WLD + rb * 32 + l31] = -O[rb][q];
    wave_lds_fence();
    const __amdgpu_buffer_rsrc_t rs = __builtin_amdgcn_make_buffer_rsrc((void*)Out, 0, 0x7fffffff, 0x00020000);
    const int voff = (int)((((int64_t)(wave * 32 + lh)) * ldo + 4 * l31) * 4);
    const int ld8 = (int)(ldo * 8);
    f32x4 v[16];
#pragma unroll
    for (int it = 0; it < 16; ++it) v[it] = *reinterpret_cast<const f32x4*>(mine + (2 * it + lh) * WLD + 4 * l31);
    asm volatile("s_waitcnt lgkmcnt(0)" ::: "memory");
    VOLT_SB();
#pragma unroll
    for (int it = 0; it < 16; ++it)
        __builtin_amdgcn_raw_buffer_store_b128(__builtin_bit_cast(u32x4, v[it]), rs, voff, it * ld8, AUX);
    VOLT_SB();
    asm volatile("s_waitcnt vmcnt(0)" ::: "memory");
}

__device__ __forceinline__ void trtri_diag_body(const float* __restrict__ Winv, float* __restrict__ Y, int Np, int i,
                                                int b, TriReduce red, float* smem) {
    const int n = Np / TS;
    float* Yb = Y + (int64_t)b * Np * Np;
    const float* W = Winv + ((int64_t)b * n + i) * TS * TS;
    const int tid = threadIdx.x;
    const int tile_id = i * (i + 1) / 2 + i;
    for (int e = tid; e < TS * TS / 4; e += NT) {
        const int r = e >> 5, c = (e & 31) * 4;
        *reinterpret_cast<f32x4*>(smem + r * WLD + c) = *reinterpret_cast<const f32x4*>(W + r * TS + c);
    }
    __syncthreads();
    float* Yd = Yb + (int64_t)i * TS * Np + (int64_t)i * TS;
    for (int e = tid; e < TS * TS; e += NT) {
        const int c = e >> 7, r = e & 127;
        Yd[(int64_t)c * Np + r] = (r >= c) ? smem[r * WLD + c] : 0.f;
    }
    if (red.rpad) {
        float* sred = smem + TS * WLD;
        float* rv = sred + TS;
        if (tid < TS) rv[tid] = red.rpad[(int64_t)b * Np + i * TS + tid];
        __syncthreads();
        float fz = 0.f, ff = 0.f;
        if (tid < TS) {
            for (int c = 0; c <= tid; ++c) {
                const float y = smem[tid * WLD + c];
                fz += y * rv[c];
                if (i * TS + c < red.N) ff += y * y;
            }
            red.zpart[((int64_t)b * n + i) * Np + i * TS + tid] = fz;
            sred[tid] = ff;
        }
        __syncthreads();
        if (tid < 64) {
            const float tot = wave_sum_f(sred[tid] + sred[tid + 64]);
            if (tid == 0) red.frob[(int64_t)b * (n * (n + 1) / 2) + tile_id] = tot;
        }
    }
}

template <bool WT = false>
__device__ __forceinline__ void trtri_reduce(const f32x16 (&O)[4], int Np, int i, int j, int b, TriReduce red,
                                             float* smem, const float* rvs = nullptr) {
    const int n = Np / TS;
    const int tid = threadIdx.x, lane = tid & 63, wave = tid >> 6, l31 = lane & 31, lh = lane >> 5;
    const int tile_id = i * (i + 1) / 2 + j;
    const float* rv = red.rpad + (int64_t)b * Np + j * TS + wave * 32;
    float rvq[16];
    if (rvs) {
#pragma unroll
        for (int q = 0; q < 16; ++q) rvq[q] = rvs[wave * 32 + accrow(q, lane)];
    } else {
#pragma unroll
        for (int q = 0; q < 16; ++q) rvq[q] = rv[accrow(q, lane)];
    }
    float* sz = smem;
    float ff = 0.f;
#pragma unroll
    for (int rb = 0; rb < 4; ++rb) {
        float cz = 0.f;
#pragma unroll
        for (int q = 0; q < 16; ++q) {
            const float y = -O[rb][q];
            cz += y * rvq[q];
            ff += y * y;
        }
        cz += __shfl_xor(cz, 32);
        if (lh == 0) sz[wave * TS + rb * 32 + l31] = cz;
    }
    ff = wave_sum_f(ff);
    if (lane == 0) sz[4 * TS + wave] = ff;
    __syncthreads();
    if (tid < TS) {
        const float zv = (sz[tid] + sz[TS + tid]) + (sz[2 * TS + tid] + sz[3 * TS + tid]);
        float* zp = red.zpart + ((int64_t)b * n + j) * Np + i * TS + tid;
        if (WT) __hip_atomic_store(zp, zv, __ATOMIC_RELAXED, __HIP_MEMORY_SCOPE_AGENT);
        else *zp = zv;
    }
    if (tid == 0)
        red.frob[(int64_t)b * (n * (n + 1) / 2) + tile_id] = (sz[4 * TS] + sz[4 * TS + 1]) + (sz[4 * TS + 2] + sz[4 * TS + 3]);
}


struct TriJob {
    TriTile t;
    const float* c0;
    bool row_ok, vec_ok;
    float* out;
    int i, j, b;
};

template <bool FROMK>
__device__ __forceinline__ TriJob panel_job(float* __restrict__ A, const float* __restrict__ Winv, int Np, int i, int k,
                                            int b, const KSource& src) {
    const int n = Np / TS;
    float* Ab = A + (int64_t)b * Np * Np;
    const int lane = threadIdx.x & 63, wave = threadIdx.x >> 6, l31 = lane & 31, lh = lane >> 5;
    const bool usek = FROMK && src.K != nullptr;
    TriJob jb;
    jb.t.X = Ab + (int64_t)k * TS * Np;
    jb.t.ldx = Np;
    jb.t.Z = Ab + (int64_t)i * TS * Np;
    jb.t.ldz = Np;
    jb.t.n1 = k * (TS / BK);
    jb.t.W = Winv + ((int64_t)b * n + k) * TS * TS;
    jb.t.flag = reinterpret_cast<const int*>(jb.t.W);
    jb.t.want = 0;
    const int gi = i * TS + wave * 32 + l31;
    const int64_t ld = usek ? src.ldk : (int64_t)Np;
    jb.c0 = (usek ? src.K + (int64_t)b * src.bsk : Ab) + (int64_t)gi * ld + k * TS + 4 * lh;
    jb.row_ok = !usek || gi < src.N;
    jb.vec_ok = !usek || (((src.ldk & 3) == 0) && ((src.bsk & 3) == 0) && (((uintptr_t)src.K & 15) == 0));
    jb.out = Ab + (int64_t)i * TS * Np + (int64_t)k * TS;
    jb.i = -1;
    jb.j = 0;
    jb.b = b;
    return jb;
}

__device__ __forceinline__ TriJob trtri_job(const float* __restrict__ A, const float* __restrict__ Winv,
                                            float* __restrict__ Y, int Np, int i, int j, int b) {
    const int n = Np / TS;
    const float* Ab = A + (int64_t)b * Np * Np;
    float* Yb = Y + (int64_t)b * Np * Np;
    TriJob jb;
    jb.t.X = Ab + (int64_t)i * TS * Np + (int64_t)j * TS;
    jb.t.ldx = Np;
    jb.t.Z = Yb + (int64_t)j * TS * Np + (int64_t)j * TS;
    jb.t.ldz = Np;
    jb.t.n1 = (i - j) * (TS / BK);
    jb.t.W = Winv + ((int64_t)b * n + i) * TS * TS;
    jb.t.flag = nullptr;
    jb.t.want = 0;
    jb.c0 = nullptr;
    jb.row_ok = jb.vec_ok = true;
    jb.out = Yb + (int64_t)j * TS * Np + (int64_t)i * TS;
    jb.i = i;
    jb.j = j;
    jb.b = b;
    return jb;
}

__device__ __forceinline__ void slab_dump(const f32x16 (&acc)[4], float* __restrict__ slab) {
    const __amdgpu_buffer_rsrc_t rs = __builtin_amdgcn_make_buffer_rsrc((void*)slab, 0, TS * TS * 4, 0x00020000);
#pragma unroll
    for (int t4 = 0; t4 < 4; ++t4)
#pragma unroll
        for (int g = 0; g < 4; ++g) {
            f32x4 v;
#pragma unroll
            for (int e = 0; e < 4; ++e) v[e] = acc[t4][4 * g + e];
            __builtin_amdgcn_raw_buffer_store_b128(__builtin_bit_cast(u32x4, v), rs, ((t4 * 4 + g) * NT + (int)threadIdx.x) * 16, 0,
                                                   16 );
        }
}
__device__ __forceinline__ void job_t0(const TriJob& jb, f32x16 (&T)[4]) {
    if (jb.c0 && jb.row_ok && jb.vec_ok) {
#pragma unroll
        for (int tm = 0; tm < 4; ++tm)
#pragma unroll
            for (int g = 0; g < 4; ++g) {
                const f32x4 v = *reinterpret_cast<const f32x4*>(jb.c0 + 32 * tm + 8 * g);
#pragma unroll
                for (int e = 0; e < 4; ++e) T[tm][4 * g + e] = -v[e];
            }
    } else if (jb.c0 && jb.row_ok) {
#pragma unroll
        for (int tm = 0; tm < 4; ++tm)
#pragma unroll
            for (int q = 0; q < 16; ++q) T[tm][q] = -jb.c0[32 * tm + 8 * (q >> 2) + (q & 3)];
    } else {
        zero_acc(T);
    }
}

}
```

Baseline: 45.55 steps/s (1 step = MLL+grad over 64 series of N=4096).

## Compute only lower-triangular subtiles in diagonal SYRK updates; add priority knobs

```diff
diff --git a/include/volt_hip_tune.h b/include/volt_hip_tune.h
--- a/include/volt_hip_tune.h
+++ b/include/volt_hip_tune.h
@@ -25,6 +25,7 @@
 
 int volt_batch_describe(int B, int n, int has_y, int order, int* items, int max_items);
 int volt_tune_batch_stamps(long long* stamps);
+int volt_tune_square_update(int on);
 int volt_batch64_describe(int B, int n, int has_y, int* items, int max_items);
 int volt_tune_batch64_stamps(long long* stamps);
 int volt_topology_describe(int* out);
diff --git a/volt_amd/_lib.py b/volt_amd/_lib.py
--- a/volt_amd/_lib.py
+++ b/volt_amd/_lib.py
@@ -81,6 +81,7 @@
     "volt_long_describe": (C.c_int, [_i32, _i32, _i32, _ptr, _i32, _ptr, _ptr]),
     "volt_batch_describe": (C.c_int, [_i32, _i32, _i32, _i32, _ptr, _i32]),
     "volt_tune_batch_stamps": (C.c_int, [_ptr]),
+    "volt_tune_square_update": (C.c_int, [_i32]),
     "volt_batch64_describe": (C.c_int, [_i32, _i32, _i32, _ptr, _i32]),
     "volt_tune_batch64_stamps": (C.c_int, [_ptr]),
     "volt_topology_describe": (C.c_int, [_ptr]),
diff --git a/volt_amd/csrc/batch_step.hip b/volt_amd/csrc/batch_step.hip
--- a/volt_amd/csrc/batch_step.hip
+++ b/volt_amd/csrc/batch_step.hip
@@ -21,6 +21,17 @@
     for (int c = i; c < nprog; c += gridDim.x * blockDim.x) prog[c] = 0;
 }
 
+#ifndef VOLT_PRIO_PROLOGUE
+#define VOLT_PRIO_PROLOGUE 0
+#endif
+#ifndef VOLT_PRIO_TRTRI_DIAG
+#define VOLT_PRIO_TRTRI_DIAG 0
+#endif
+#ifndef VOLT_PRIO_ALPHA
+#define VOLT_PRIO_ALPHA 0
+#endif
+
+constexpr int PRIO_ENTRY = VOLT_PRIO_PROLOGUE ? 3 : 0;
 constexpr int AUX_WT = AUX_SC1;
 
 __device__ __forceinline__ void diag0_image(const KSource& src, int b, float* smem) {
@@ -145,24 +156,26 @@
         }
         batch_wait<LOCAL>(rowp + k, k, k >= 2 ? la + k : nullptr, 1, info_b);
         if (stamps && threadIdx.x == 0) stamps[(int64_t)w * 8 + 3] = __builtin_amdgcn_s_memrealtime();
-        if (k >= 2) update_body<FROMK>(A, Np, k, k, k - 1, k, false, b, src, smem, true);
-        else update_body<FROMK>(A, Np, 1, 1, 0, 1, true, b, src, smem, true);
+        if (k >= 2) update_diag<FROMK>(A, Np, k, k - 1, k, false, b, src, smem, true);
+        else update_diag<FROMK>(A, Np, 1, 0, 1, true, b, src, smem, true);
         if (stamps && threadIdx.x == 0) stamps[(int64_t)w * 8 + 4] = __builtin_amdgcn_s_memrealtime();
         diag_body<false, false, LOCAL>(A, Winv, info, Np, k, b, smem, nullptr, true);
         return;
     }
     if (kind == BK_LOOKAHEAD) {
+        if (PRIO_ENTRY != 0) __builtin_amdgcn_s_setprio(0);
         const int k = d.y;
         Chase ch;
         ch.p0 = ch.p1 = rowp + k + 1;
         bool ok = true;
-        update_body<FROMK, 0, true, LOCAL>(A, Np, k + 1, k + 1, 0, k, true, b, src, smem, false, &ch, &ok);
+        update_diag<FROMK, true, LOCAL>(A, Np, k + 1, 0, k, true, b, src, smem, false, &ch, &ok);
         if (!ok && (threadIdx.x & 63) == 0) report_timeout(info_b);
         publish_release<LOCAL>(la + k + 1, 1);
         return;
     }
     if (kind == BK_TRTRI_DIAG) {
         const int i = d.y;
+        if ((VOLT_PRIO_TRTRI_DIAG ? 3 : 0) != PRIO_ENTRY) __builtin_amdgcn_s_setprio(VOLT_PRIO_TRTRI_DIAG ? 3 : 0);
         batch_wait<LOCAL>(reinterpret_cast<const int*>(Winv + ((int64_t)b * n + i) * TS * TS), 1, nullptr, 0, info_b);
         trtri_diag_body(Winv, Y, Np, i, b, red, smem);
         publish_release<LOCAL>(tcol + i, 1);
@@ -170,6 +183,7 @@
     }
     if (kind == BK_ALPHA) {
         const int c = d.y;
+        if ((VOLT_PRIO_ALPHA ? 3 : 0) != PRIO_ENTRY) __builtin_amdgcn_s_setprio(VOLT_PRIO_ALPHA ? 3 : 0);
         if (threadIdx.x < 64) {
             bool ok = true;
             for (int j = 0; j <= c; ++j) ok = wait_word<AtLeast>(tcol + j, c - j + 1) && ok;
@@ -206,7 +220,7 @@
     if (jb.t.n1 > 0) pre = chase_issue(jb.t.ch);
     job_t0(jb, T);
     if (stamps && threadIdx.x == 0) stamps[(int64_t)w * 8 + 3] = __builtin_amdgcn_s_memrealtime();
-    const bool ok = tri_tile_run<true, LOCAL>(jb.t, T, O, smem, &pre);
+    const bool ok = tri_tile_run<true, LOCAL, VOLT_PRIO_PROLOGUE != 0>(jb.t, T, O, smem, &pre);
 #ifndef VOLT_NO_EPILOGUE_PRIO
     __builtin_amdgcn_s_setprio(3);
 #endif
@@ -268,7 +282,7 @@
 piece:
     w = __builtin_amdgcn_readfirstlane(w);
     if (w < 0) return;
-    __builtin_amdgcn_s_setprio(0);
+    __builtin_amdgcn_s_setprio(PRIO_ENTRY);
     if (a.stamps && threadIdx.x == 0) {
         a.stamps[(int64_t)w * 8] = __builtin_amdgcn_s_memrealtime();
         a.stamps[(int64_t)w * 8 + 2] = ((long long)hw << 32) | (unsigned)__builtin_amdgcn_s_getreg((16 - 1) << 11 | 0 << 6 | 4);
diff --git a/volt_amd/csrc/chol.hip b/volt_amd/csrc/chol.hip
--- a/volt_amd/csrc/chol.hip
+++ b/volt_amd/csrc/chol.hip
@@ -69,15 +69,15 @@
     if (k_upd >= 0) {
         const int k = k_upd;
         if (w < B) {
-            if (k >= 2) update_body<FROMK>(A, Np, k, k, k - 1, k, false, w, src, smem, true);
-            else if (k == 1) update_body<FROMK>(A, Np, 1, 1, 0, 1, true, w, src, smem, true);
+            if (k >= 2) update_diag<FROMK>(A, Np, k, k - 1, k, false, w, src, smem, true);
+            else if (k == 1) update_diag<FROMK>(A, Np, 1, 0, 1, true, w, src, smem, true);
             diag_body(A, Winv, info, Np, k, w, smem, nullptr, k > 0);
             return;
         }
         w -= B;
         const int npre = (k >= 1 && k + 1 < n) ? B : 0;
         if (w < npre) {
-            update_body<FROMK>(A, Np, k + 1, k + 1, 0, k, true, w, src, smem);
+            update_diag<FROMK>(A, Np, k + 1, 0, k, true, w, src, smem);
             return;
         }
         w -= npre;
@@ -240,8 +240,8 @@
     int w = blockIdx.x;
     const int k = k_upd;
     if (k < n && w < B) {
-        if (k >= 2) update_body<FROMK>(A, Np, k, k, k - 1, k, false, w, src, smem, true);
-        else if (k == 1) update_body<FROMK>(A, Np, 1, 1, 0, 1, true, w, src, smem, true);
+        if (k >= 2) update_diag<FROMK>(A, Np, k, k - 1, k, false, w, src, smem, true);
+        else if (k == 1) update_diag<FROMK>(A, Np, 1, 0, 1, true, w, src, smem, true);
         diag_body(A, Winv, info, Np, k, w, smem, nullptr, k > 0);
         return;
     }
@@ -313,8 +313,8 @@
     const int b0 = d.w & 0xffff, b1 = d.w >> 16;
     float* slabs = sk.slab + (int64_t)tile * S * TS * TS;
     if (kind == 0) {
-        if (k >= 2) update_body<FROMK>(A, Np, k, k, k - 1, k, false, b, src, smem, true);
-        else if (k == 1) update_body<FROMK>(A, Np, 1, 1, 0, 1, true, b, src, smem, true);
+        if (k >= 2) update_diag<FROMK>(A, Np, k, k - 1, k, false, b, src, smem, true);
+        else if (k == 1) update_diag<FROMK>(A, Np, 1, 0, 1, true, b, src, smem, true);
         diag_body(A, Winv, info, Np, k, b, smem, nullptr, k > 0);
     } else if (kind == 4) {
         trtri_diag_body(Winv, Y, Np, i_tri, b, red, smem);
@@ -412,6 +412,7 @@
         geti("VOLT_LONG_PULLERS", t.long_pullers);
         geti("VOLT_BATCH_XSKEW", t.batch_xskew);
         geti("VOLT_BATCH_XDROP", t.batch_xdrop);
+        geti("VOLT_SQUARE_UPDATE", t.square_update);
         geti("VOLT_BATCH64", t.batch64);
         geti("VOLT_BATCH64_MAX", t.batch64_max);
         geti("VOLT_BATCH64_MAX_STEP", t.batch64_max_step);
@@ -466,6 +467,13 @@
     }();
     return tn;
 }
+static int g_square_override = -1;
+int volt_internal_square_update() { return (g_square_override >= 0 ? g_square_override : tunables().square_update) != 0; }
+extern "C" int volt_tune_square_update(int on) {
+    g_square_override = on < 0 ? -1 : (on != 0);
+    return 0;
+}
+
 struct LaunchTimer {
     hipEvent_t base = nullptr;
     std::vector<hipEvent_t> ev;
@@ -844,7 +852,7 @@
     for (int i = 0; i < n; ++i) {
         if (tm) tm->begin(1, s);
         hipLaunchKernelGGL(factor_step_kernel<false>, dim3((i + 1) * B), dim3(256), 0, s, const_cast<float*>(A),
-                           const_cast<float*>(Winv), Y, nullptr, Np, -1, i, B, KSource{nullptr, 0, 0, nullptr, 0.f, 0},
+                           const_cast<float*>(Winv), Y, nullptr, Np, -1, i, B, KSource{nullptr, 0, 0, nullptr, 0.f, 0, volt_internal_square_update()},
                            nored);
         if (tm) tm->end(s);
     }
@@ -914,7 +922,7 @@
     if (k < 1 || k + 1 >= n) return -6;
     if (var < 0 || var > 5) return -7;
     hipStream_t s = (hipStream_t)stream;
-    const KSource none{nullptr, 0, 0, nullptr, 0.f, 0};
+    const KSource none{nullptr, 0, 0, nullptr, 0.f, 0, volt_internal_square_update()};
     for (int r = 0; r < reps; ++r) {
         if (var == 0) hipLaunchKernelGGL(tune_update_kernel, dim3((n - k - 1) * B), dim3(256), 0, s, A, Winv, info, Np, k, B, none);
         else if (var == 1) hipLaunchKernelGGL(tune_update_sq_kernel<0>, dim3((n - k - 1) * B), dim3(256), 0, s, A, Np, k, B, none);
@@ -1032,7 +1040,7 @@
     if (B < 0) return -4;
     if (Np < TS || Np % TS) return -5;
     if (B == 0) return 0;
-    return potrf_with_scratch(KSource{nullptr, 0, 0, nullptr, 0.f, 0}, StepMats{A, Winv, nullptr, info, B, Np, (hipStream_t)stream}, ws,
+    return potrf_with_scratch(KSource{nullptr, 0, 0, nullptr, 0.f, 0, volt_internal_square_update()}, StepMats{A, Winv, nullptr, info, B, Np, (hipStream_t)stream}, ws,
                               ws_bytes, ws_flags, -6);
 }
 
@@ -1050,7 +1058,7 @@
     if (B < 0 || B > 65535) return -9;
     if (N < 1) return -10;
     if (B == 0) return 0;
-    return potrf_with_scratch(KSource{K, ldk, bsk, sigma2, jitter, N}, StepMats{A, Winv, nullptr, info, B, N, (hipStream_t)stream}, ws,
+    return potrf_with_scratch(KSource{K, ldk, bsk, sigma2, jitter, N, volt_internal_square_update()}, StepMats{A, Winv, nullptr, info, B, N, (hipStream_t)stream}, ws,
                               ws_bytes, ws_flags, -11);
 }
 
diff --git a/volt_amd/csrc/common.h b/volt_amd/csrc/common.h
--- a/volt_amd/csrc/common.h
+++ b/volt_amd/csrc/common.h
@@ -55,6 +55,7 @@
     }
 }
 
+template <bool SYM = false>
 __device__ __forceinline__ void stage_store(const StageRegs& s, float* __restrict__ buf) {
     const int t = threadIdx.x;
     const int row = t >> 3, cq = (t & 7) * 4;
@@ -63,7 +64,7 @@
 #pragma unroll
     for (int p = 0; p < 4; ++p) {
         *reinterpret_cast<f32x4*>(sA + (row + 32 * p) * SLD + cq) = s.a[p];
-        *reinterpret_cast<f32x4*>(sB + (row + 32 * p) * SLD + cq) = s.b[p];
+        if constexpr (!SYM) *reinterpret_cast<f32x4*>(sB + (row + 32 * p) * SLD + cq) = s.b[p];
     }
 }
 
@@ -86,12 +87,13 @@
     return sa;
 }
 
+template <bool SYM = false>
 __device__ __forceinline__ void stage_load_buf(StageRegs& s, const StageAddr& sa, int k0) {
     const int so = __builtin_amdgcn_readfirstlane(k0 * 4);
 #pragma unroll
     for (int p = 0; p < 4; ++p) {
         s.a[p] = __builtin_bit_cast(f32x4, __builtin_amdgcn_raw_buffer_load_b128(sa.ra, sa.va[p], so, 0));
-        s.b[p] = __builtin_bit_cast(f32x4, __builtin_amdgcn_raw_buffer_load_b128(sa.rb, sa.vb[p], so, 0));
+        if constexpr (!SYM) s.b[p] = __builtin_bit_cast(f32x4, __builtin_amdgcn_raw_buffer_load_b128(sa.rb, sa.vb[p], so, 0));
     }
 }
 
@@ -105,6 +107,16 @@
 template <int WL> struct Frag;
 template <> struct Frag<0> { f32x4 a0, a1, b0, b1; };
 template <> struct Frag<1> { f32x4 a[4], b0; };
+template <> struct Frag<2> { f32x4 a0, a1, b0, b1; };
+
+struct LowerMap {
+    int a0, a1, b0, b1;
+    __device__ __forceinline__ int row(int t) const { return (t & 2) ? a1 : a0; }
+    __device__ __forceinline__ int col(int t) const { return (t & 1) ? b1 : b0; }
+};
+__device__ __forceinline__ LowerMap lower_map(int wave) {
+    return LowerMap{(0x3230 >> (4 * wave)) & 3, (0x3321 >> (4 * wave)) & 3, (0x1200 >> (4 * wave)) & 3, (0x1311 >> (4 * wave)) & 3};
+}
 
 template <int WL>
 __device__ __forceinline__ void frag_load(Frag<WL>& f, const float* __restrict__ buf, int kk) {
@@ -119,6 +131,12 @@
         f.b0 = *reinterpret_cast<const f32x4*>(sB + (wc * 64 + l31) * SLD + ko);
         f.b1 = *reinterpret_cast<const f32x4*>(sB + (wc * 64 + 32 + l31) * SLD + ko);
         f.a1 = *reinterpret_cast<const f32x4*>(sA + (wr * 64 + 32 + l31) * SLD + ko);
+    } else if constexpr (WL == 2) {
+        const LowerMap lm = lower_map(wave);
+        f.a0 = *reinterpret_cast<const f32x4*>(sA + (lm.a0 * 32 + l31) * SLD + ko);
+        f.b0 = *reinterpret_cast<const f32x4*>(sA + (lm.b0 * 32 + l31) * SLD + ko);
+        f.b1 = *reinterpret_cast<const f32x4*>(sA + (lm.b1 * 32 + l31) * SLD + ko);
+        f.a1 = *reinterpret_cast<const f32x4*>(sA + (lm.a1 * 32 + l31) * SLD + ko);
     } else {
         f.b0 = *reinterpret_cast<const f32x4*>(sB + (wave * 32 + l31) * SLD + ko);
 #pragma unroll
@@ -128,7 +146,11 @@
 
 template <int WL>
 __device__ __forceinline__ void frag_mma_m(const Frag<WL>& f, int m, f32x16 (&acc)[4]) {
-    if constexpr (WL == 0) {
+    if constexpr (WL == 2) {
+        acc[0] = __builtin_amdgcn_mfma_f32_32x32x2f32(f.a0[m], f.b0[m], acc[0], 0, 0, 0);
+        acc[2] = __builtin_amdgcn_mfma_f32_32x32x2f32(f.a1[m], f.b0[m], acc[2], 0, 0, 0);
+        acc[3] = __builtin_amdgcn_mfma_f32_32x32x2f32(f.a1[m], f.b1[m], acc[3], 0, 0, 0);
+    } else if constexpr (WL == 0) {
         acc[0] = __builtin_amdgcn_mfma_f32_32x32x2f32(f.a0[m], f.b0[m], acc[0], 0, 0, 0);
         acc[1] = __builtin_amdgcn_mfma_f32_32x32x2f32(f.a0[m], f.b1[m], acc[1], 0, 0, 0);
         acc[2] = __builtin_amdgcn_mfma_f32_32x32x2f32(f.a1[m], f.b0[m], acc[2], 0, 0, 0);
@@ -155,7 +177,7 @@
 #define VOLT_SB() __builtin_amdgcn_sched_barrier(0)
 template <int WL>
 __device__ __forceinline__ f32x16 frag_mma_one(const Frag<WL>& f, int m, int t, const f32x16& c) {
-    if constexpr (WL == 0) {
+    if constexpr (WL == 0 || WL == 2) {
         const float a = (t & 2) ? f.a1[m] : f.a0[m], b = (t & 1) ? f.b1[m] : f.b0[m];
         return __builtin_amdgcn_mfma_f32_32x32x2f32(a, b, c, 0, 0, 0);
     } else {
@@ -169,7 +191,7 @@
     VOLT_SB();
     T[3] += P[3];
     VOLT_SB();
-    P[1] = frag_mma_one<WL>(f, 0, 1, z);
+    if constexpr (WL != 2) P[1] = frag_mma_one<WL>(f, 0, 1, z);
     P[2] = frag_mma_one<WL>(f, 0, 2, z);
     P[3] = frag_mma_one<WL>(f, 0, 3, z);
 #pragma unroll
@@ -180,13 +202,13 @@
 #pragma unroll
     for (int m = 0; m < 3; ++m) frag_mma_m<WL>(f, m, P);
     P[0] = frag_mma_one<WL>(f, 3, 0, P[0]);
-    P[1] = frag_mma_one<WL>(f, 3, 1, P[1]);
+    if constexpr (WL != 2) P[1] = frag_mma_one<WL>(f, 3, 1, P[1]);
     VOLT_SB();
     T[0] += P[0];
     VOLT_SB();
     P[2] = frag_mma_one<WL>(f, 3, 2, P[2]);
     VOLT_SB();
-    T[1] += P[1];
+    if constexpr (WL != 2) T[1] += P[1];
     VOLT_SB();
     P[3] = frag_mma_one<WL>(f, 3, 3, P[3]);
     VOLT_SB();
@@ -196,15 +218,17 @@
 enum SegRole { SEG_MID = 0, SEG_FIRST = 1, SEG_LAST = 2 };
 
 
+template <bool SYM = false>
 __device__ __forceinline__ void stage_store_piece(const StageRegs& s, float* __restrict__ buf, int p) {
     const int t = threadIdx.x;
     const int row = t >> 3, cq = (t & 7) * 4;
     *reinterpret_cast<f32x4*>(buf + (row + 32 * p) * SLD + cq) = s.a[p];
-    *reinterpret_cast<f32x4*>(buf + TS * SLD + (row + 32 * p) * SLD + cq) = s.b[p];
-}
+    if constexpr (!SYM) *reinterpret_cast<f32x4*>(buf + TS * SLD + (row + 32 * p) * SLD + cq) = s.b[p];
+}
+template <bool SYM = false>
 __device__ __forceinline__ void stage_load_piece(StageRegs& s, const StageAddr& sa, int so, int p) {
     s.a[p] = __builtin_bit_cast(f32x4, __builtin_amdgcn_raw_buffer_load_b128(sa.ra, sa.va[p], so, 0));
-    s.b[p] = __builtin_bit_cast(f32x4, __builtin_amdgcn_raw_buffer_load_b128(sa.rb, sa.vb[p], so, 0));
+    if constexpr (!SYM) s.b[p] = __builtin_bit_cast(f32x4, __builtin_amdgcn_raw_buffer_load_b128(sa.rb, sa.vb[p], so, 0));
 }
 
 template <int WL, bool MORE, bool ST, bool LD, int ROLE = SEG_MID>
@@ -220,7 +244,7 @@
 #pragma unroll
     for (int m = 0; m < 4; ++m) {
         frag_mma_m<WL>(F1, m, acc);
-        if constexpr (ST) stage_store_piece(s, nxt, m);
+        if constexpr (ST) stage_store_piece<WL == 2>(s, nxt, m);
         VOLT_SB();
     }
     frag_load<WL>(F1, cur, 3);
@@ -229,7 +253,7 @@
 #pragma unroll
     for (int m = 0; m < 4; ++m) {
         frag_mma_m<WL>(F0, m, acc);
-        if constexpr (LD) stage_load_piece(s, sa, so, m);
+        if constexpr (LD) stage_load_piece<WL == 2>(s, sa, so, m);
         VOLT_SB();
     }
     __syncthreads();
@@ -249,10 +273,10 @@
     if constexpr (CHASE) ready = chase_wait<LOCALP>(*ch, 1, *ch_ok);
     StageRegs s0, s1;
     const StageAddr sa = stage_addr(A, lda, B, ldb);
-    stage_load_buf(s0, sa, 0);
-    stage_store(s0, smem);
-    stage_load_buf(s0, sa, BK);
-    stage_load_buf(s1, sa, 2 * BK);
+    stage_load_buf<WL == 2>(s0, sa, 0);
+    stage_store<WL == 2>(s0, smem);
+    stage_load_buf<WL == 2>(s0, sa, BK);
+    stage_load_buf<WL == 2>(s1, sa, 2 * BK);
     __syncthreads();
     Frag<WL> F0, F1;
     frag_load<WL>(F0, smem, 0);
@@ -401,7 +425,7 @@
     VOLT_SB();
 }
 
-template <bool CHASE = false, bool LOCALP = false>
+template <bool CHASE = false, bool LOCALP = false, bool PRIO0 = false>
 __device__ __forceinline__ bool tri_tile_run(const TriTile& t, f32x16 (&T)[4], f32x16 (&O)[4], float* smem,
                                              const ChasePre* pre = nullptr) {
     const int tid = threadIdx.x;
@@ -438,6 +462,7 @@
 #pragma unroll
     for (int p = 0; p < 4; ++p) tri_load_piece(s1, ts, 2, p);
     __syncthreads();
+    if constexpr (PRIO0) __builtin_amdgcn_s_setprio(0);
     int c = 0;
     if (t.n1 > 0) {
         Frag<1> F0, F1;
diff --git a/volt_amd/csrc/host.h b/volt_amd/csrc/host.h
--- a/volt_amd/csrc/host.h
+++ b/volt_amd/csrc/host.h
@@ -30,6 +30,7 @@
     int batch_pullers = 1;
     int long_pullers = 1;
     int rollout_lane = 1;
+    int square_update = 0;
     int batch_xskew = 0, batch_xdrop = 0;
     int f64_lookahead = -1;
     int f64_trtri_lookahead = -1;
@@ -48,6 +49,7 @@
     const float* sigma2;
     float jitter;
     int N;
+    int square;
 };
 struct KSource64 {
     const double* K;
@@ -112,6 +114,7 @@
     std::mutex* mu;
 };
 bool volt_internal_aux(VoltAux* out);
+int volt_internal_square_update();
 size_t volt_internal_sched_bytes(int B, int n);
 int volt_internal_sched_install(volt::Region tab, int B, int n, int has_y, int cap, void* stream);
 int volt_internal_factor(const volt::StepMats& m, const volt::KSource& src, const volt::TriReduce& red, const volt::SplitScratch& sk,
diff --git a/volt_amd/csrc/mll.hip b/volt_amd/csrc/mll.hip
--- a/volt_amd/csrc/mll.hip
+++ b/volt_amd/csrc/mll.hip
@@ -301,7 +301,7 @@
 };
 StepArgs step_args(const TailCtx& c, const float* K, int64_t ldk, int64_t bsk, const float* resid, int* info, int B, hipStream_t s) {
     const volt::MllWs& w = c.w;
-    return {StepMats{w.A, w.Winv, w.Y, info, B, c.N, s}, KSource{K, ldk, bsk, c.sigma2, c.jitter, c.N},
+    return {StepMats{w.A, w.Winv, w.Y, info, B, c.N, s}, KSource{K, ldk, bsk, c.sigma2, c.jitter, c.N, volt_internal_square_update()},
             TriReduce{w.rpad, w.zpart, w.frob, c.N}, StepTail{resid, w.rpad, w.z, w.apad, w.apart, c.out, c.alpha}};
 }
 void pad_resid(const StepArgs& a, const TailCtx& c) {
diff --git a/volt_amd/csrc/tiles.h b/volt_amd/csrc/tiles.h
--- a/volt_amd/csrc/tiles.h
+++ b/volt_amd/csrc/tiles.h
@@ -15,20 +15,72 @@
     return Ab[(int64_t)gi * Np + gj];
 }
 
-template <bool FROMK, int ABL = 0, bool CHASE = false, bool LOCALP = false>
+template <bool FROMK, int ABL = 0, bool CHASE = false, bool LOCALP = false, bool LOWER = false>
 __device__ __forceinline__ void update_body(float* __restrict__ A, int Np, int rowblk, int colblk, int kb0, int kb1,
                                             bool fromk, int b, const KSource& src, float* smem,
                                             bool to_image = false, const Chase* ch = nullptr, bool* ch_ok = nullptr) {
     float* Ab = A + (int64_t)b * Np * Np;
     const float* Arows = Ab + (int64_t)rowblk * TS * Np + (int64_t)kb0 * TS;
     const float* Brows = Ab + (int64_t)colblk * TS * Np + (int64_t)kb0 * TS;
-    const int lane = threadIdx.x & 63, wave = threadIdx.x >> 6;
-    const int wr = wave >> 1, wc = wave & 1;
+    const int lane = threadIdx.x & 63;
     float* C = Ab + (int64_t)rowblk * TS * Np + (int64_t)colblk * TS;
     f32x16 acc[4];
     const bool usek = FROMK && fromk;
     const float add = usek ? ((src.sigma2 ? src.sigma2[b] : 0.f) + src.jitter) : 0.f;
     const float* Kb = usek ? src.K + (int64_t)b * src.bsk : nullptr;
+    if (LOWER && !src.square) {
+        {
+            const LowerMap lm = lower_map(threadIdx.x >> 6);
+#pragma unroll
+            for (int t = 0; t < 4; ++t) {
+                if (t == 1) continue;
+#pragma unroll
+                for (int q = 0; q < 16; ++q) {
+                    const int r = lm.row(t) * 32 + accrow(q, lane);
+                    const int c = lm.col(t) * 32 + (lane & 31);
+                    acc[t][q] = -input_elem(src, Kb, add, Ab, Np, usek, rowblk * TS + r, colblk * TS + c);
+                }
+            }
+        }
+        gemm_nt_128<2, CHASE, LOCALP>(Arows, Np, Brows, Np, (kb1 - kb0) * (TS / BK), acc, smem, ch, ch_ok);
+        const int tix = threadIdx.x, ln = lane;
+        const LowerMap lm = lower_map(tix >> 6);
+        if (to_image) {
+            __syncthreads();
+#pragma unroll
+            for (int t = 0; t < 4; ++t) {
+                if (t == 1) continue;
+#pragma unroll
+                for (int q = 0; q < 16; ++q) {
+                    const int r = lm.row(t) * 32 + accrow(q, ln);
+                    const int c = lm.col(t) * 32 + (ln & 31);
+                    smem[r * (TS + 1) + c] = (c <= r) ? -acc[t][q] : 0.f;
+                }
+            }
+#pragma unroll
+            for (int u = 0; u < 6; ++u) {
+                const int zi = u < 3 ? 0 : (u < 5 ? 1 : 2), zj = u < 3 ? u + 1 : (u < 5 ? u - 1 : 3);
+#pragma unroll
+                for (int it = 0; it < 32 * 32 / NT; ++it) {
+                    const int e = tix + it * NT;
+                    smem[(32 * zi + (e >> 5)) * (TS + 1) + 32 * zj + (e & 31)] = 0.f;
+                }
+            }
+            return;
+        }
+#pragma unroll
+        for (int t = 0; t < 4; ++t) {
+            if (t == 1) continue;
+#pragma unroll
+            for (int q = 0; q < 16; ++q) {
+                const int r = lm.row(t) * 32 + accrow(q, ln);
+                const int c = lm.col(t) * 32 + (ln & 31);
+                C[(int64_t)r * Np + c] = -acc[t][q];
+            }
+        }
+        return;
+    }
+    const int wave = threadIdx.x >> 6, wr = wave >> 1, wc = wave & 1;
 #pragma unroll
     for (int tm = 0; tm < 2; ++tm)
 #pragma unroll
@@ -74,6 +126,12 @@
                 const int c = wc * 64 + tn * 32 + (lane & 31);
                 C[(int64_t)r * Np + c] = -acc[tm * 2 + tn][q];
             }
+}
+template <bool FROMK, bool CHASE = false, bool LOCALP = false>
+__device__ __forceinline__ void update_diag(float* __restrict__ A, int Np, int k, int kb0, int kb1, bool fromk, int b,
+                                            const KSource& src, float* smem, bool to_image = false,
+                                            const Chase* ch = nullptr, bool* ch_ok = nullptr) {
+    update_body<FROMK, 0, CHASE, LOCALP, true>(A, Np, k, k, kb0, kb1, fromk, b, src, smem, to_image, ch, ch_ok);
 }
 
 constexpr int DT = TS + 1;
```

New measurement: 45.83 steps/s (1 step = MLL+grad over 64 series of N=4096) (median of 6 runs). About the same (+0.6%).
